# brendan-duncan/unity_webgpu_pathtracer

Hardware: AMD Instinct MI355X
Metric: Mrays/s at 1920x1080, 8 spp (higher is better)
Workload: dtype f32; 1 GPU; sponza: Sponza-class atrium (~250k tris, 24 textured Disney materials, 2 rect lights + sky), 1920x1080, 8 spp/pass, depth 4, progressive passes (CurrentSample = 8k); tris=250752, schedule=1, passes_in_flight=12, passes_per_launch_sequence=1

## Files before the change

### __graft_entry__.py

```python
import os
import subprocess
import sys

ROOT = os.path.dirname(os.path.abspath(__file__))
if ROOT not in sys.path:
    sys.path.insert(0, ROOT)


def build() -> None:
    subprocess.check_call(["make", "-C", os.path.join(ROOT, "unity_webgpu_pathtracer_amd", "csrc")])
    subprocess.check_call(["make", "-C", os.path.join(ROOT, "unity_webgpu_pathtracer_amd", "csrc"), "stress"])
    subprocess.check_call(["make", "-C", os.path.join(ROOT, "host")])
    subprocess.check_call(["make", "-C", os.path.join(ROOT, "oracle")])
    subprocess.check_call(["make", "-C", os.path.join(ROOT, "oracle"), "ref"])
    from unity_webgpu_pathtracer_amd import plugin
    plugin.load_library()


def smoke() -> None:
    import numpy as np
    from oracle import pyoracle
    from unity_webgpu_pathtracer_amd import scenes
    from unity_webgpu_pathtracer_amd.pathtracer import PathTracer

    for s, w, h in ((scenes.material_zoo(), 96, 64), (scenes.cornell_box(), 64, 64)):
        pt = PathTracer(s, device=0, width=w, height=h, samplesPerPass=2)
        p = pt.params(seed=0x12345678)
        pt.render_pass(p)
        gpu = pt.readback()
        b = pyoracle.buffers_from_bvhscene(pt._bvhScene)
        ref, _ = pyoracle.render(b, p)
        linf = float(np.abs(gpu - ref).max())
        print(f"[smoke] {s.name} {w}x{h} 2spp, schedule {pt.schedule()}: Linf vs oracle = {linf:.3e}, rays = {pt.stats().rays}")
        assert linf < 1e-4, linf
        pt.close()


if __name__ == "__main__":
    build()
    if len(sys.argv) > 1 and sys.argv[1] == "smoke":
        smoke()
```

### include/ptmi_plugin.h

```cpp
#ifndef PTMI_PLUGIN_H
#define PTMI_PLUGIN_H

#include <stdint.h>
#include "ptmi_layouts.h"

#ifdef __cplusplus
extern "C" {
#endif

#if defined(_WIN32)
#define PT_API __declspec(dllexport)
#else
#define PT_API __attribute__((visibility("default")))
#endif


PT_API int   BuildBVH(const PTFloat4* vertices, int triangleCount);
PT_API void  DestroyBVH(int index);
PT_API int   IsBVHReady(int index);
PT_API void* GetBVHPtr(int index);
PT_API void* GetBVH(int index);
PT_API int   GetCWBVHNodesSize(int index);
PT_API int   GetCWBVHTrisSize(int index);
PT_API int   GetCWBVHData(int index, PTFloat4** bvhNodes, PTFloat4** bvhTris);
// ... 88 lines not shown
} PTTimings;

#define PT_OK                 0
#define PT_ERR_INVALID_ARG   -1
#define PT_ERR_NO_DEVICE     -2
#define PT_ERR_HIP           -3
#define PT_ERR_NO_SCENE      -4
#define PT_ERR_UNSUPPORTED   -5

PT_API int PTCreate(int deviceIndex, PTContext** outCtx);
PT_API int PTDestroy(PTContext* ctx);

PT_API int PTSetScene(PTContext* ctx, const PTSceneDesc* scene);

PT_API int PTSetTileOwnership(PTContext* ctx, int rank, int worldSize);

PT_API int PTGetOwnedTileSlots(PTContext* ctx, const PTFrameParams* params, uint64_t* outFloat4Slots);
PT_API int PTPackOwnedTiles(PTContext* ctx, const PTFrameParams* params, const void* dFrame, void* dPacked);
PT_API int PTUnpackTiles(PTContext* ctx, const PTFrameParams* params, int rank, int worldSize, const void* dPacked, void* dFrame);

typedef struct PTGroup PTGroup;
PT_API int PTCreateMulti(const int* deviceIndices, int deviceCount, PTGroup** outGroup);
PT_API int PTGroupDestroy(PTGroup* group);
PT_API int PTGroupSize(PTGroup* group);
PT_API PTContext* PTGroupGetContext(PTGroup* group, int index);
PT_API int PTGroupSetScene(PTGroup* group, const PTSceneDesc* scene);
PT_API int PTGroupRenderPass(PTGroup* group, const PTFrameParams* params);
PT_API int PTGroupRenderPassBatch(PTGroup* group, const PTFrameParams* params, int count);
PT_API int PTGroupFlipFrames(PTGroup* group);
PT_API int PTGroupResetFrames(PTGroup* group);
PT_API int PTGroupSynchronize(PTGroup* group);
PT_API int PTGroupReadback(PTGroup* group, float* dstRGBA, uint64_t dstFloats);
PT_API void* PTGroupGetAssembledFrame(PTGroup* group);
PT_API int PTGroupGetStats(PTGroup* group, PTStats* out);
PT_API int PTGroupResetStats(PTGroup* group);

PT_API int PTRenderPass(PTContext* ctx, const PTFrameParams* params);
PT_API int PTFlipFrames(PTContext* ctx);
PT_API int PTResetFrames(PTContext* ctx);

PT_API int PTRenderPassTo(PTContext* ctx, const PTFrameParams* params, void* dOutput, const void* dAccumulated);

PT_API int PTRenderPassBatchTo(PTContext* ctx, const PTFrameParams* params, int count, void* dOutput, const void* dAccumulated);
PT_API int PTRenderPassBatch(PTContext* ctx, const PTFrameParams* params, int count);

PT_API int PTSynchronize(PTContext* ctx);
PT_API int PTReadback(PTContext* ctx, float* dstRGBA, uint64_t dstFloats);
PT_API void* PTGetFramePointer(PTContext* ctx, int which);
typedef struct PTPresentParams {
    uint32_t OutputWidth, OutputHeight;
    int32_t  Mode;
    int32_t  sRGB;
    float    Exposure, Brightness, Contrast, Saturation, Vignette;
} PTPresentParams;
PT_API int PTPresent(PTContext* ctx, const PTPresentParams* params, const void* dSrc, void* dDst);
PT_API int PTPresentToHost(PTContext* ctx, const PTPresentParams* params, float* dstRGBA, uint64_t dstFloats);

#define PT_MESH_HAS_32_BIT_INDICES 0x1u
#define PT_MESH_HAS_NORMALS        0x2u
#define PT_MESH_HAS_TANGENTS       0x4u
#define PT_MESH_HAS_UVS            0x8u
typedef struct PTMeshDesc {
    const void* vertexBuffer;  uint64_t vertexBufferBytes;
    const void* indexBuffer;   uint64_t indexBufferBytes;
    uint32_t VertexStride, PositionOffset, NormalOffset, TangentOffset, UVOffset;
    uint32_t MaterialIndex;
    uint32_t TriangleCount, OutputTriangleStart;
    float    LocalToWorld[16], WorldToLocal[16];
    uint32_t flags;            uint32_t _pad;
} PTMeshDesc;
PT_API int PTProcessMeshes(PTContext* ctx, const PTMeshDesc* meshes, uint32_t meshCount, uint32_t totalTriangles,
                           float* outVertexPositions, void* outTriangleAttributes);

typedef struct PTTextureDesc {
    const float* texels;  uint32_t width, height;  int32_t hasAlpha;  uint32_t _pad;
} PTTextureDesc;
PT_API int PTCopyTextureData(PTContext* ctx, const PTTextureDesc* textures, uint32_t count, uint32_t* outTextureData, uint64_t outUints);

PT_API void* PTGetStream(PTContext* ctx);

PT_API int PTSetStatsLevel(PTContext* ctx, int level);
PT_API int PTGetStats(PTContext* ctx, PTStats* out);
PT_API int PTResetStats(PTContext* ctx);

PT_API int PTSetProfiling(PTContext* ctx, int enabled);
PT_API int PTGetTimings(PTContext* ctx, PTTimings* out);
PT_API int PTResetTimings(PTContext* ctx);

PT_API int PTSetSchedule(PTContext* ctx, int schedule);
PT_API int PTGetSchedule(PTContext* ctx);
PT_API int PTSetWavefrontIterations(PTContext* ctx, int iterations);

PT_API int PTSetPassesInFlight(PTContext* ctx, int passes);
PT_API int PTGetPassesInFlight(PTContext* ctx);
PT_API int PTSetSubFrames(PTContext* ctx, int subFrames);

typedef struct PTRay {
    float    origin[3];
    float    direction[3];
    float    tmax;
    uint32_t reserved;
} PTRay;

typedef struct PTRayHit {
    float    t;
    float    u, v;
    uint32_t prim;
} PTRayHit;

typedef struct PTRaySurface {
    float    position[3]; float    t;
    float    normal[3];   int32_t  materialIndex;
    float    uv[2];       uint32_t instance;
                          uint32_t prim;
} PTRaySurface;

#ifdef __cplusplus
static_assert(sizeof(PTRay) == 32, "PTRay is 32 bytes");
static_assert(sizeof(PTRayHit) == 16, "PTRayHit is 16 bytes");
static_assert(sizeof(PTRaySurface) == 48, "PTRaySurface is 48 bytes");
#else
_Static_assert(sizeof(PTRay) == 32, "PTRay is 32 bytes");
_Static_assert(sizeof(PTRayHit) == 16, "PTRayHit is 16 bytes");
_Static_assert(sizeof(PTRaySurface) == 48, "PTRaySurface is 48 bytes");
#endif

#define PT_QUERY_CLOSEST  0u
#define PT_QUERY_ANY_HIT  1u
#define PT_QUERY_SURFACE  2u

PT_API int PTTraceRays(PTContext* ctx, const PTRay* dRays, uint64_t count, uint32_t flags,
                       PTRayHit* dHits, PTRaySurface* dSurface );
PT_API int PTTraceRaysHost(PTContext* ctx, const PTRay* rays, uint64_t count, uint32_t flags,
                           PTRayHit* hits, PTRaySurface* surface);

#define PT_DENOISE_DEMODULATE_ALBEDO 0x1u

typedef struct PTDenoiseParams {
    uint32_t structSize;
    int32_t  iterations;
    float    sigmaLuminance;
    float    sigmaNormal;
    float    sigmaDepth;
    uint32_t flags;
} PTDenoiseParams;

#ifdef __cplusplus
static_assert(sizeof(PTDenoiseParams) == 24, "PTDenoiseParams is 24 bytes");
#else
_Static_assert(sizeof(PTDenoiseParams) == 24, "PTDenoiseParams is 24 bytes");
#endif

PT_API int PTRenderGuides(PTContext* ctx, const PTFrameParams* params, int samplesPerPixel);
PT_API int PTDenoise(PTContext* ctx, const PTDenoiseParams* params, const void* dSrc, void* dDst);
PT_API int PTDenoiseToHost(PTContext* ctx, const PTDenoiseParams* params, float* dstRGBA, uint64_t dstFloats);
PT_API void* PTGetGuidePointer(PTContext* ctx, int which);

PT_API int PTUpdateInstances(PTContext* ctx, const PTBlasInstance* instances, uint32_t count);
PT_API int PTUpdateInstancesDevice(PTContext* ctx, const PTBlasInstance* dInstances, uint32_t count);
PT_API int PTUpdateLights(PTContext* ctx, const void* lights, uint32_t count);
PT_API int PTUpdateMaterials(PTContext* ctx, const void* materials, uint32_t count);
PT_API int PTReadTLAS(PTContext* ctx, void* dstNodes, uint64_t dstNodeBytes, uint32_t* dstIndices, uint64_t dstIndexCount,
                      uint32_t* outNodeCount);

typedef struct PTNoiseParams {
    uint32_t structSize;
// ... 483 lines not shown
```

### unity_webgpu_pathtracer_amd/abi.py

```python
import ctypes as C

import numpy as np

FLOAT4 = np.dtype([("x", "<f4"), ("y", "<f4"), ("z", "<f4"), ("w", "<f4")])

CWBVH_NODE = np.dtype([
    ("lo", "<f4", 3), ("ex", "u1"), ("ey", "u1"), ("ez", "u1"), ("imask", "u1"),
    ("childBaseIndex", "<u4"), ("triBaseIndex", "<u4"), ("meta", "u1", 8),
    ("qlox", "u1", 8), ("qloy", "u1", 8), ("qloz", "u1", 8),
    ("qhix", "u1", 8), ("qhiy", "u1", 8), ("qhiz", "u1", 8),
])
assert CWBVH_NODE.itemsize == 80

TRI_ATTR = np.dtype([
    ("normal0", "<f4", 3), ("pad0", "<f4"), ("normal1", "<f4", 3), ("pad1", "<f4"),
    ("normal2", "<f4", 3), ("pad2", "<f4"), ("tangent0", "<f4", 3), ("pad3", "<f4"),
    ("tangent1", "<f4", 3), ("pad4", "<f4"), ("tangent2", "<f4", 3), ("pad5", "<f4"),
    ("uv0", "<f4", 2), ("uv1", "<f4", 2), ("uv2", "<f4", 2), ("materialIndex", "<u4"), ("pad6", "<f4"),
])
assert TRI_ATTR.itemsize == 128

MATERIAL_FLOATS = 32
LIGHT_FLOATS = 16

# ... 22 lines not shown
PT_FEATURE_HAS_ENVIRONMENT_TEXTURE = 0x8

PT_OK = 0
PT_ERR_INVALID_ARG = -1
PT_ERR_NO_DEVICE = -2
PT_ERR_HIP = -3
PT_ERR_NO_SCENE = -4
PT_ERR_UNSUPPORTED = -5


class _Sized(C.Structure):
    def __init__(self, *args, **kw):
        super().__init__(*args, **kw)
        self.structSize = C.sizeof(type(self))


class PTSceneDesc(_Sized):
    _fields_ = [
        ("structSize", C.c_uint32), ("_pad3", C.c_uint32),
        ("bvhNodes", C.c_void_p), ("bvhNodesBytes", C.c_uint64),
        ("bvhTris", C.c_void_p), ("bvhTrisBytes", C.c_uint64),
        ("triAttrs", C.c_void_p), ("triAttrsBytes", C.c_uint64),
        ("materials", C.c_void_p), ("materialCount", C.c_uint32), ("_pad0", C.c_uint32),
        ("lights", C.c_void_p), ("lightCount", C.c_uint32), ("_pad1", C.c_uint32),
        ("textureData", C.c_void_p), ("textureDataUints", C.c_uint64),
        ("features", C.c_uint32), ("_pad2", C.c_uint32),
        ("tlasData", C.c_void_p), ("tlasDataFloats", C.c_uint64),
        ("tlasIndexOffset", C.c_uint32), ("instanceCount", C.c_uint32),
        ("gpuInstances", C.c_void_p),
        ("envTexture", C.c_void_p), ("envWidth", C.c_uint32), ("envHeight", C.c_uint32),
    ]


class PTFrameParams(_Sized):
    _fields_ = [
        ("structSize", C.c_uint32), ("_pad0", C.c_uint32),
        ("CamInvProj", C.c_float * 16),
        ("CamToWorld", C.c_float * 16),
        ("RngSeedRoot", C.c_uint32),
        ("MaxRayBounces", C.c_uint32),
        ("SamplesPerPass", C.c_int32),
        ("OutputWidth", C.c_uint32),
        ("OutputHeight", C.c_uint32),
        ("CurrentSample", C.c_uint32),
        ("EnvironmentMode", C.c_int32),
        ("EnvironmentIntensity", C.c_float),
        ("EnvironmentColor", C.c_float * 4),
        ("EnvironmentMapRotation", C.c_float),
        ("FocalLength", C.c_float),
        ("Aperture", C.c_float),
        ("UseFireflyFilter", C.c_int32),
        ("MaxFireflyLuminance", C.c_float),
        ("UseRussianRoulette", C.c_int32),
        ("DispatchGroupsX", C.c_uint32),
        ("DispatchGroupsY", C.c_uint32),
    ]

    def copy(self):
        other = PTFrameParams()
        C.memmove(C.byref(other), C.byref(self), C.sizeof(PTFrameParams))
        return other


class PTStats(C.Structure):
    _fields_ = [(n, C.c_uint64) for n in (
        "paths", "closestHitRays", "shadowRays", "nodeVisits", "triTests", "attrFetches",
        "materialFetches", "lightFetches", "texelFetches", "texDescriptorFetches",
        "pixelsWritten", "pixelsRead", "maxStackDepth", "stackOverflows", "tlasNodeVisits", "instanceVisits")]

    def as_dict(self):
        return {n: int(getattr(self, n)) for n, _ in self._fields_}

    @property
    def rays(self):
        return int(self.closestHitRays + self.shadowRays)

    def algorithmic_bytes(self):
        return int(80 * self.nodeVisits + 48 * self.triTests + 128 * self.attrFetches
                   + 128 * self.materialFetches + 64 * self.lightFetches + 4 * self.texelFetches
                   + 16 * self.texDescriptorFetches + 16 * (self.pixelsWritten + self.pixelsRead)
                   + 64 * self.tlasNodeVisits + 144 * self.instanceVisits)


class PTPresentParams(C.Structure):
    _fields_ = [("OutputWidth", C.c_uint32), ("OutputHeight", C.c_uint32), ("Mode", C.c_int32), ("sRGB", C.c_int32),
                ("Exposure", C.c_float), ("Brightness", C.c_float), ("Contrast", C.c_float), ("Saturation", C.c_float),
                ("Vignette", C.c_float)]


TONEMAP_NONE, TONEMAP_ACES, TONEMAP_FILMIC, TONEMAP_REINHARD, TONEMAP_LOTTES = range(5)


PT_MESH_HAS_32_BIT_INDICES, PT_MESH_HAS_NORMALS, PT_MESH_HAS_TANGENTS, PT_MESH_HAS_UVS = 0x1, 0x2, 0x4, 0x8


class PTMeshDesc(C.Structure):
    _fields_ = [("vertexBuffer", C.c_void_p), ("vertexBufferBytes", C.c_uint64),
                ("indexBuffer", C.c_void_p), ("indexBufferBytes", C.c_uint64),
                ("VertexStride", C.c_uint32), ("PositionOffset", C.c_uint32), ("NormalOffset", C.c_uint32),
                ("TangentOffset", C.c_uint32), ("UVOffset", C.c_uint32), ("MaterialIndex", C.c_uint32),
                ("TriangleCount", C.c_uint32), ("OutputTriangleStart", C.c_uint32),
                ("LocalToWorld", C.c_float * 16), ("WorldToLocal", C.c_float * 16),
                ("flags", C.c_uint32), ("_pad", C.c_uint32)]


class PTTextureDesc(C.Structure):
    _fields_ = [("texels", C.c_void_p), ("width", C.c_uint32), ("height", C.c_uint32), ("hasAlpha", C.c_int32), ("_pad", C.c_uint32)]


class PTTimings(C.Structure):
    _fields_ = [("passes", C.c_uint64), ("kernelMsTotal", C.c_double),
                ("kernelMsLast", C.c_double), ("kernelLaunches", C.c_uint64)]


PT_FAR_PLANE = 100000.0
PT_QUERY_CLOSEST = 0
PT_QUERY_ANY_HIT = 1
PT_QUERY_SURFACE = 2
PT_MISS = 0xFFFFFFFF


class PTRay(C.Structure):
    _fields_ = [("origin", C.c_float * 3), ("direction", C.c_float * 3), ("tmax", C.c_float), ("reserved", C.c_uint32)]


class PTRayHit(C.Structure):
    _fields_ = [("t", C.c_float), ("u", C.c_float), ("v", C.c_float), ("prim", C.c_uint32)]


class PTRaySurface(C.Structure):
    _fields_ = [("position", C.c_float * 3), ("t", C.c_float), ("normal", C.c_float * 3), ("materialIndex", C.c_int32),
                ("uv", C.c_float * 2), ("instance", C.c_uint32), ("prim", C.c_uint32)]


assert C.sizeof(PTRay) == 32 and C.sizeof(PTRayHit) == 16 and C.sizeof(PTRaySurface) == 48


PT_DENOISE_DEMODULATE_ALBEDO = 0x1


class PTDenoiseParams(C.Structure):
    _fields_ = [("structSize", C.c_uint32), ("iterations", C.c_int32), ("sigmaLuminance", C.c_float),
                ("sigmaNormal", C.c_float), ("sigmaDepth", C.c_float), ("flags", C.c_uint32)]


assert C.sizeof(PTDenoiseParams) == 24


def denoise_params(iterations: int = 5, sigma_luminance: float = 4.0, sigma_normal: float = 128.0, sigma_depth: float = 1.0,
                   demodulate: bool = True) -> PTDenoiseParams:
    return PTDenoiseParams(C.sizeof(PTDenoiseParams), iterations, sigma_luminance, sigma_normal, sigma_depth,
                           PT_DENOISE_DEMODULATE_ALBEDO if demodulate else 0)


class PTNoiseParams(C.Structure):
    _fields_ = [("structSize", C.c_uint32), ("relFloor", C.c_float), ("threshold", C.c_float), ("percentile", C.c_float)]


class PTNoiseStats(C.Structure):
    _fields_ = [("structSize", C.c_uint32), ("observations", C.c_uint32), ("samples", C.c_uint64), ("pixels", C.c_uint64),
                ("pixelsBelow", C.c_uint64), ("meanError", C.c_float), ("maxError", C.c_float), ("percentileError", C.c_float),
                ("_pad", C.c_uint32), ("histogram", C.c_uint32 * 256)]


assert C.sizeof(PTNoiseParams) == 16 and C.sizeof(PTNoiseStats) == 1072

# ... 277 lines not shown
```

### unity_webgpu_pathtracer_amd/csrc/plugin_exports.cpp

```cpp
#include <chrono>
#include <cstddef>
#include <deque>
#include <string>
#include <algorithm>
#include "bvh_builder.h"
#include "bvh_refit.h"
#include "bvh_quality.h"
#include "skin_rule.h"
#include "morph_rule.h"
#include "chart_rule.h"
#include "sh_rule.h"
#include "volume_rule.h"
#include "placement_rule.h"
#include "lmfilter_rule.h"
#include "adaptive_gather_rule.h"
#include "reflection_rule.h"
#include "ptmi_plugin.h"

namespace {
std::deque<ptbvh::Cwbvh*> g_bvhs;
std::deque<ptbvh::Tlas*> g_tlases;

template <class T> int add_slot(std::deque<T*>& table, T* obj)
{
    for (size_t i = 0; i < table.size(); ++i)
        if (table[i] == nullptr) { table[i] = obj; return (int)i; }
    table.push_back(obj);
    return (int)table.size() - 1;
}
template <class T> T* get_slot(std::deque<T*>& table, int index)
{
    return (index >= 0 && index < (int)table.size()) ? table[index] : nullptr;
}
template <class T> void free_slot(std::deque<T*>& table, int index)
{
    if (index >= 0 && index < (int)table.size() && table[index]) { delete table[index]; table[index] = nullptr; }
}
}

extern "C" {

PT_API int BuildBVH(const PTFloat4* vertices, int triangleCount)
{
    if (!vertices || triangleCount <= 0) return -1;
    ptbvh::Cwbvh* bvh = new ptbvh::Cwbvh();
    const auto t0 = std::chrono::steady_clock::now();
    if (!bvh->build(vertices, (uint32_t)triangleCount)) { delete bvh; return -1; }
    bvh->buildMs = std::chrono::duration<double, std::milli>(std::chrono::steady_clock::now() - t0).count();
    return add_slot(g_bvhs, bvh);
}

namespace { std::string g_buildError; }
PT_API int PTBuildBVHDevice(int deviceIndex, const PTFloat4* vertices, int triangleCount)
{
    if (!vertices || triangleCount <= 0) { g_buildError = "vertices == NULL or triangleCount <= 0"; return -1; }
    ptbvh::Cwbvh* bvh = new ptbvh::Cwbvh();
    if (!ptbvh::build_cwbvh_device(deviceIndex, vertices, (uint32_t)triangleCount, *bvh, &bvh->buildMs, g_buildError)) { delete bvh; return -1; }
    g_buildError.clear();
    return add_slot(g_bvhs, bvh);
}
PT_API const char* PTGetBVHBuildError(void) { return g_buildError.c_str(); }
PT_API double PTGetBVHBuildMs(int index)
{
    ptbvh::Cwbvh* b = get_slot(g_bvhs, index);
    return b ? b->buildMs : -1.0;
}
PT_API int PTRefitBVH(int index, const PTFloat4* vertices, int triangleCount)
{
    ptbvh::Cwbvh* b = get_slot(g_bvhs, index);
    if (!b) { g_buildError = "no such BVH handle"; return 0; }
    if (!vertices || triangleCount <= 0 || (uint32_t)triangleCount != b->triCount) { g_buildError = "vertices == NULL or triangleCount is not the handle's"; return 0; }
    if (!ptbvh::refit_cwbvh(b->nodeData.data(), b->usedBlocks / 5u, b->triData.data(), (uint64_t)b->triCount * 3u, 0, 0, vertices, b->triCount, g_buildError)) return 0;
    g_buildError.clear();
    return 1;
}
PT_API int PTRefitBVHArrays(PTFloat4* bvhNodes, uint64_t nodeBytes, PTFloat4* bvhTris, uint64_t triBytes, const PTFloat4* vertices, int triangleCount)
{
    if (!bvhNodes || !bvhTris || !vertices || triangleCount <= 0 || nodeBytes < 80 || nodeBytes % 80 || triBytes != (uint64_t)triangleCount * 48u) {
        g_buildError = "NULL array, nodeBytes not a multiple of 80 or triBytes != triangleCount * 48";
        return 0;
    }
    if (!ptbvh::refit_cwbvh(bvhNodes, nodeBytes / 80u, bvhTris, triBytes / 16u, 0, 0, vertices, (uint32_t)triangleCount, g_buildError)) return 0;
    g_buildError.clear();
    return 1;
}
PT_API int PTMeasureBVHArrays(const PTFloat4* bvhNodes, uint64_t nodeBytes, const PTFloat4* bvhTris, uint64_t triBytes, int triangleCount, PTGeometryQuality* out)
{
    if (!bvhNodes || !bvhTris || !out || triangleCount <= 0 || nodeBytes < 80 || nodeBytes % 80 || triBytes != (uint64_t)triangleCount * 48u) {
        g_buildError = "NULL array or result, nodeBytes not a multiple of 80 or triBytes != triangleCount * 48";
        return 0;
    }
    if (out->structSize < sizeof(PTGeometryQuality) || out->structSize > 4096u) {
        g_buildError = "PTGeometryQuality.structSize is not set (must be sizeof(PTGeometryQuality) of the host's header)";
        return 0;
    }
    ptbvh::Quality q;
    if (!ptbvh::measure_cwbvh(bvhNodes, nodeBytes / 80u, bvhTris, triBytes / 16u, (uint32_t)triangleCount, q, g_buildError)) return 0;
    out->nodeCapacity = q.nodeCapacity; out->nodeCount = q.nodeCount; out->triangleCount = q.triangleCount; out->levels = q.levels;
    out->reserved = 0;
// ... 96 lines not shown
    g_buildError.clear();
    return 1;
}
PT_API int PTProbeDepthProjectHost(const PTProbe* probes, uint64_t count, uint32_t firstSample, uint32_t samples, const float* distances,
                                   float maxDistance, PTProbeDepthMap* out)
{
    if (!ptvol::depth_project_host(probes, count, firstSample, samples, distances, maxDistance, out, g_buildError)) return 0;
    g_buildError.clear();
    return 1;
}
PT_API int PTProbeGridIrradianceHost(const PTProbeGrid* grid, const PTProbeCoeffs* sh, const PTProbeDepthMap* depth, const PTReceiver* queries,
                                     uint64_t count, PTIrradiance* out)
{
    if (!ptvol::grid_irradiance_host(grid, sh, depth, queries, count, out, g_buildError)) return 0;
    g_buildError.clear();
    return 1;
}
PT_API int PTProbePlaceStepHost(const PTProbe* probes, uint64_t count, uint32_t firstSample, uint32_t samples, const PTProbePlaceParams* params,
                                const PTRayHit* hits, const PTRaySurface* surfaces, int move, PTProbePlacement* inout, PTProbePlaceStats* stats)
{
    if (!ptplace::place_step_host(probes, count, firstSample, samples, params, hits, surfaces, move, inout, stats, g_buildError)) return 0;
    g_buildError.clear();
    return 1;
}
PT_API int PTProbeGridIrradiancePlacedHost(const PTProbeGrid* grid, const PTProbeCoeffs* sh, const PTProbeDepthMap* depth, const PTProbePlacement* placement,
                                           const PTReceiver* queries, uint64_t count, PTIrradiance* out)
{
    if (!ptplace::grid_irradiance_placed_host(grid, sh, depth, placement, queries, count, out, g_buildError)) return 0;
    g_buildError.clear();
    return 1;
}
PT_API int PTDenoiseLightmapHost(const PTLightmapDenoiseParams* params, const uint32_t* texels, const PTReceiver* recv, const PTIrradiance* irr, uint64_t count,
                                 uint32_t width, uint32_t height, PTIrradiance* out)
{
    if (!ptlmf::denoise_host(params, texels, recv, irr, count, width, height, out, g_buildError)) return 0;
    g_buildError.clear();
    return 1;
}
PT_API int PTSelectReceiversHost(const PTAdaptiveGather* adaptive, uint32_t n, const uint32_t* active, uint64_t activeCount, const PTIrradiance* acc,
                                 const PTReceiver* recv, uint64_t entryCount, uint32_t* outActive, PTReceiver* outRecv, uint64_t* survivors, uint64_t* stopped)
{
    if (!ptag::select_host(adaptive, n, active, activeCount, acc, recv, entryCount, outActive, outRecv, survivors, stopped, g_buildError)) return 0;
    g_buildError.clear();
    return 1;
}
PT_API int PTFoldIrradianceHost(const uint32_t* active, uint64_t activeCount, const PTIrradiance* fresh, uint32_t m, uint32_t n, uint64_t entryCount,
                                PTIrradiance* acc, uint32_t* counts)
{
    if (!ptag::fold_host(active, activeCount, fresh, m, n, entryCount, acc, counts, g_buildError)) return 0;
    g_buildError.clear();
    return 1;
}
PT_API int PTEqualiseIrradianceHost(const PTIrradiance* irr, const uint32_t* counts, uint64_t count, uint32_t samplesEq, PTIrradiance* out)
{
    if (!ptag::equalise_host(irr, counts, count, samplesEq, out, g_buildError)) return 0;
    g_buildError.clear();
    return 1;
}
PT_API int PTReflectionDirectionsHost(const PTProbe* probes, uint64_t count, uint32_t res, uint32_t firstSample, uint32_t samples, PTRadianceRay* rays)
{
    if (!ptrefl::directions_host(probes, count, res, firstSample, samples, rays, g_buildError)) return 0;
    g_buildError.clear();
    return 1;
}
PT_API int PTReflectionFoldHost(const PTRadiance* radiance, uint64_t count, uint32_t res, uint32_t samples, PTReflectionTexel* out)
{
    if (!ptrefl::fold_host(radiance, count, res, samples, out, g_buildError)) return 0;
    g_buildError.clear();
    return 1;
}
PT_API int PTReflectionPrefilterHost(const PTReflectionTexel* base, uint64_t count, uint32_t res, uint32_t levels, PTReflectionTexel* outMaps)
{
    if (!ptrefl::prefilter_host(base, count, res, levels, outMaps, g_buildError)) return 0;
    g_buildError.clear();
    return 1;
}
PT_API int PTReflectionLookupHost(const PTReflectionTexel* maps, uint64_t probeCount, uint32_t res, uint32_t levels, const PTProbe* probes,
                                  const PTReflectionBox* boxes, const PTReflectionQuery* queries, uint64_t count, PTReflectionTexel* out)
{
    if (!ptrefl::lookup_host(maps, probeCount, res, levels, probes, boxes, queries, count, out, g_buildError)) return 0;
    g_buildError.clear();
    return 1;
}
PT_API void DestroyBVH(int index) { free_slot(g_bvhs, index); }
PT_API int IsBVHReady(int index) { return get_slot(g_bvhs, index) != nullptr; }
PT_API void* GetBVH(int index) { return get_slot(g_bvhs, index); }
PT_API void* GetBVHPtr(int index) { return get_slot(g_bvhs, index); }
PT_API int GetCWBVHNodesSize(int index)
{
    ptbvh::Cwbvh* b = get_slot(g_bvhs, index);
    return b ? (int)(b->usedBlocks * 16u) : 0;
}
PT_API int GetCWBVHTrisSize(int index)
{
    ptbvh::Cwbvh* b = get_slot(g_bvhs, index);
    return b ? (int)(b->triCount * 3u * 16u) : 0;
}
PT_API int GetCWBVHData(int index, PTFloat4** bvhNodes, PTFloat4** bvhTris)
{
    ptbvh::Cwbvh* b = get_slot(g_bvhs, index);
    if (!b || !bvhNodes || !bvhTris || b->nodeData.empty() || b->triData.empty()) return 0;
    *bvhNodes = b->nodeData.data();
    *bvhTris = b->triData.data();
    return 1;
}

PT_API int BuildTLAS(const PTBlasInstance* instances, int instanceCount)
{
    if (!instances || instanceCount <= 0) return -1;
    ptbvh::Tlas* t = new ptbvh::Tlas();
    if (!t->build(instances, (uint32_t)instanceCount)) { delete t; return -1; }
    return add_slot(g_tlases, t);
}
PT_API void DestroyTLAS(int index) { free_slot(g_tlases, index); }
PT_API int IsTLASReady(int index) { return get_slot(g_tlases, index) != nullptr; }
PT_API int GetTLASNodesSize(int index)
{
    ptbvh::Tlas* t = get_slot(g_tlases, index);
    return t ? (int)(t->usedNodes * 64u) : 0;
}
PT_API int GetTLASData(int index, PTFloat4** tlasNodes, uint32_t** tlasIndices)
{
    ptbvh::Tlas* t = get_slot(g_tlases, index);
    if (!t || !tlasNodes || !tlasIndices || t->nodes.empty()) return 0;
    *tlasNodes = (PTFloat4*)t->nodes.data();
    *tlasIndices = t->indices.data();
    return 1;
}

}
```

### unity_webgpu_pathtracer_amd/csrc/pt_api_context.hip

```cpp
#include "pt_context.h"

#include <dlfcn.h>

#include <cstdlib>
#include <algorithm>
#include <array>

thread_local std::string g_lastError;

namespace {

uint32_t hw_queue_limit()
{
    const char* e = getenv("GPU_MAX_HW_QUEUES");
    const long q = e ? strtol(e, nullptr, 10) : 4;
    return q < 1 ? 1u : (q > 1024 ? 1024u : (uint32_t)q);
}

bool create_masked(Stream& s)
{
    int device = 0, cus = 0;
    if (hipGetDevice(&device) != hipSuccess || hipDeviceGetAttribute(&cus, hipDeviceAttributeMultiprocessorCount, device) != hipSuccess || cus <= 0) {
        (void)hipGetLastError();
        return false;
// ... 279 lines not shown
    if (envOn) {
        const size_t n = (size_t)s->envWidth * s->envHeight;
        cdf.resize(n);
        for (size_t i = 0; i < n; ++i) {
            const float* px = s->envTexture + 4 * i;
            cdfSum += 0.299f * px[0] + 0.587f * px[1] + 0.114f * px[2];
            cdf[i] = cdfSum;
        }
        if ((rc = upload(c, c->envTex, s->envTexture, n * 16))) return rc;
        if ((rc = upload(c, c->envCdf, cdf.data(), n * 4))) return rc;
    }
    if (lights) {
        if ((rc = c->lightConst.reserve((size_t)s->lightCount * 64))) return rc;
    }
    HIP_TRY(hipStreamSynchronize(c->stream));
    c->scene.nodes = (const uint4*)c->nodes.ptr;
    c->scene.tris = (const float4*)c->tris.ptr;
    c->scene.attrs = (const float4*)c->attrs.ptr;
    c->scene.materials = (const float4*)c->materials.ptr;
    c->scene.lights = lights ? (const float4*)c->lights.ptr : nullptr;
    c->scene.tex = textures ? (const uint32_t*)c->tex.ptr : nullptr;
    c->scene.lightCount = lights ? (int32_t)s->lightCount : 0;
    c->scene.materialCount = s->materialCount;
    c->scene.hasLights = lights ? 1u : 0u;
    c->scene.hasTextures = textures ? 1u : 0u;
    c->scene.tlas = tlasOn ? (const float*)c->tlas.ptr : nullptr;
    c->scene.instances = tlasOn ? (const float4*)c->instances.ptr : nullptr;
    c->scene.instByLeaf = tlasOn ? (const float4*)c->instByLeaf.ptr : nullptr;
    c->scene.tlasBfs = tlasOn ? (const float*)c->tlasBfs.ptr : nullptr;
    c->scene.tlasNodeCount = tlasOn ? (uint32_t)(bfs.size() / 16) : 0u;
    c->scene.tlasIndexOffset = tlasOn ? s->tlasIndexOffset : 0u;
    c->scene.hasTlas = tlasOn ? 1u : 0u;
    c->scene.envTex = envOn ? (const float4*)c->envTex.ptr : nullptr;
    c->scene.envCdf = envOn ? (const float*)c->envCdf.ptr : nullptr;
    c->scene.envW = envOn ? (int32_t)s->envWidth : 0;
    c->scene.envH = envOn ? (int32_t)s->envHeight : 0;
    c->scene.envCdfSum = cdfSum;
    c->scene.hasEnvTex = envOn ? 1u : 0u;
    c->scene.lightConst = lights ? (const float4*)c->lightConst.ptr : nullptr;
    c->update.instanceCount = tlasOn ? s->instanceCount : 0u;
    c->update.sceneLightCount = lights ? s->lightCount : 0u;
    c->update.origTlasNodes = tlasOn ? s->tlasIndexOffset / 16u : 0u;
    std::vector<uint32_t>& valid = c->update.validTextures;
    valid.clear();
    if (textures) {
        const float* mats = (const float*)s->materials;
        for (uint32_t m = 0; m < s->materialCount; ++m)
            for (int k : kTextureSlots) {
                uint64_t t = 0;
                if (texture_slot(mats[(size_t)m * 32 + k], s->textureData, s->textureDataUints, t) == 0) valid.push_back((uint32_t)t);
            }
        std::sort(valid.begin(), valid.end());
        valid.erase(std::unique(valid.begin(), valid.end()), valid.end());
    }
    if (lights) {
        HIP_TRY(pt_launch_derive_lights(c->scene, (float4*)c->lightConst.ptr, c->stream));
        HIP_TRY(hipStreamSynchronize(c->stream));
    }
    c->hasScene = true;
    return PT_OK;
}

extern "C" {

PT_API int PTCreate(int deviceIndex, PTContext** outCtx)
{
    if (!outCtx) return fail(PT_ERR_INVALID_ARG, "outCtx == NULL");
    *outCtx = nullptr;
    int count = 0;
    hipError_t e = hipGetDeviceCount(&count);
    if (e != hipSuccess || count <= 0)
        return fail(PT_ERR_NO_DEVICE, std::string("no HIP device available (") + (e != hipSuccess ? hipGetErrorString(e) : "device count 0") +
                                          "); this library has no CPU fallback");
    if (deviceIndex < 0 || deviceIndex >= count) return fail(PT_ERR_INVALID_ARG, "deviceIndex out of range");
    HIP_TRY(hipSetDevice(deviceIndex));
    PTContext* c = new PTContext();
    c->device = deviceIndex;
    hipError_t se = hipStreamCreateWithFlags(&c->stream.h, hipStreamNonBlocking);
    if (se != hipSuccess) { delete c; return fail(PT_ERR_HIP, std::string("hipStreamCreate: ") + hipGetErrorString(se)); }
    if (hw_queue_limit() < 16u) {
        if (int rc = create_set_stream(0u, c->sets[0].stream, &c->ownQueues)) { delete c; return rc; }
    }
    c->numSets = default_passes_in_flight(c->ownQueues);
    se = hipMalloc(&c->dStats.ptr, 16 * sizeof(unsigned long long));
    if (se != hipSuccess) { delete c; return fail(PT_ERR_HIP, std::string("hipMalloc: ") + hipGetErrorString(se)); }
    hipMemsetAsync(c->dStats.ptr, 0, 16 * sizeof(unsigned long long), c->stream);
    *outCtx = c;
    return PT_OK;
}

PT_API int PTDestroy(PTContext* c)
{
    if (!c) return PT_OK;
    hipSetDevice(c->device);
    hipStreamSynchronize(c->stream);
    if (c->update.stream) hipStreamSynchronize(c->update.stream);
    for (auto& set : c->sets) if (set.stream) hipStreamSynchronize(set.stream);
    delete c;
    return PT_OK;
}

PT_API int PTSetScene(PTContext* c, const PTSceneDesc* hostScene) { return set_scene(c, hostScene, true); }

PT_API int PTSetTileOwnership(PTContext* c, int rank, int worldSize)
{
    if (!c || worldSize < 1 || rank < 0 || rank >= worldSize) return fail(PT_ERR_INVALID_ARG, "bad rank/worldSize");
    c->rank = rank;
    c->world = worldSize;
    return PT_OK;
}

PT_API int PTSynchronize(PTContext* c)
{
    if (!c) return fail(PT_ERR_INVALID_ARG, "ctx == NULL");
    HIP_TRY(hipSetDevice(c->device));
    HIP_TRY(hipStreamSynchronize(c->stream));
    return PT_OK;
}

PT_API void* PTGetStream(PTContext* c) { return c ? (void*)c->stream : nullptr; }

PT_API int PTSetStatsLevel(PTContext* c, int level)
{
    if (!c) return fail(PT_ERR_INVALID_ARG, "ctx == NULL");
    c->statsLevel = level > 0 ? 1 : 0;
    return PT_OK;
}

PT_API int PTGetStats(PTContext* c, PTStats* out)
{
    if (!c || !out) return fail(PT_ERR_INVALID_ARG, "ctx/out == NULL");
    HIP_TRY(hipSetDevice(c->device));
    unsigned long long h[16];
    HIP_TRY(hipMemcpyAsync(h, c->dStats.ptr, sizeof(h), hipMemcpyDeviceToHost, c->stream));
    HIP_TRY(hipStreamSynchronize(c->stream));
    static_assert(sizeof(PTStats) == 16 * 8, "PTStats is 16 counters");
    memcpy(out, h, sizeof(PTStats));
    return PT_OK;
}

PT_API int PTResetStats(PTContext* c)
{
    if (!c) return fail(PT_ERR_INVALID_ARG, "ctx == NULL");
    HIP_TRY(hipSetDevice(c->device));
    HIP_TRY(hipMemsetAsync(c->dStats.ptr, 0, 16 * sizeof(unsigned long long), c->stream));
    return PT_OK;
}

PT_API int PTSetProfiling(PTContext* c, int enabled)
{
    if (!c) return fail(PT_ERR_INVALID_ARG, "ctx == NULL");
    c->profiling = enabled != 0;
    return PT_OK;
}

PT_API int PTGetTimings(PTContext* c, PTTimings* out)
{
    if (!c || !out) return fail(PT_ERR_INVALID_ARG, "ctx/out == NULL");
    HIP_TRY(hipSetDevice(c->device));
    int rc = drain_events(c);
    if (rc) return rc;
    *out = c->timings;
    return PT_OK;
}

PT_API int PTResetTimings(PTContext* c)
{
    if (!c) return fail(PT_ERR_INVALID_ARG, "ctx == NULL");
    int rc = drain_events(c);
    if (rc) return rc;
    c->timings = PTTimings{};
    return PT_OK;
}

PT_API int PTGetSchedule(PTContext* c)
{
    if (!c) return fail(PT_ERR_INVALID_ARG, "ctx == NULL");
    return effective_schedule(c);
}

PT_API int PTSetSchedule(PTContext* c, int schedule)
{
    if (!c) return fail(PT_ERR_INVALID_ARG, "ctx == NULL");
    if (schedule < -1 || schedule > 4)
        return fail(PT_ERR_UNSUPPORTED, "unknown schedule (0 = megakernel, 1 = wavefront + refill trace, 2 = wavefront, one ray per lane, 3 = wavefront + persistent dynamic-chunk trace, 4 = fused persistent wavefront)");
    c->schedule = schedule;
    return PT_OK;
}

PT_API int PTSetPassesInFlight(PTContext* c, int passes)
{
    if (!c || passes < 0 || passes > PT_WF_SETS) return fail(PT_ERR_INVALID_ARG, "ctx == NULL or passes outside 0.." + std::to_string(PT_WF_SETS));
    HIP_TRY(hipSetDevice(c->device));
    for (auto& set : c->sets) if (set.stream) HIP_TRY(hipStreamSynchronize(set.stream));
    c->numSets = passes == 0 ? default_passes_in_flight(c->ownQueues) : (uint32_t)passes;
    c->nextSet = 0u;
    for (uint32_t k = c->numSets; k < (uint32_t)PT_WF_SETS; ++k) {
        c->sets[k].arena.release();
        c->sets[k].wf = PTWfBuffers{};
    }
    return PT_OK;
}

PT_API int PTSetSubFrames(PTContext* c, int subFrames)
{
    if (!c || subFrames < 1 || subFrames > PT_WF_SETS) return fail(PT_ERR_INVALID_ARG, "ctx == NULL or subFrames outside 1.." + std::to_string(PT_WF_SETS));
    c->subFrames = (uint32_t)subFrames;
    return PT_OK;
}

PT_API int PTGetPassesInFlight(PTContext* c) { return c ? (int)c->numSets : fail(PT_ERR_INVALID_ARG, "ctx == NULL"); }

PT_API int PTSetWavefrontIterations(PTContext* c, int iterations)
{
    if (!c || iterations < 0) return fail(PT_ERR_INVALID_ARG, "ctx == NULL or iterations < 0");
    c->wfIterations = (uint32_t)iterations;
    return PT_OK;
}

PT_API const char* PTGetLastError(void) { return g_lastError.c_str(); }
PT_API int PTGetVersion(void) { return (0 << 16) | 2; }

}
// ... 1 lines not shown
```

### unity_webgpu_pathtracer_amd/csrc/pt_api_render.hip

```cpp
#include "pt_context.h"

int ensure_frames(PTContext* c, uint32_t w, uint32_t h)
{
    if (c->frames.w == w && c->frames.h == h) return PT_OK;
    int rc = c->frames.resize(w, h, {sizeof(float4), sizeof(float4)}, nullptr);
    if (rc) return rc;
    for (int i = 0; i < 2; i++) HIP_TRY(hipMemsetAsync(c->frames.f4(i), 0, c->frames.buf[i].used, c->stream));
    c->cur = 0;
    return PT_OK;
}

int ensure_wavefront(PTContext* c, PTContext::WfSet& set, uint32_t numSlots, uint32_t maxIterations)
{
    int rc;
    if ((rc = create_set_stream((uint32_t)(&set - c->sets), set.stream)) || (rc = create(set.callEv)) || (rc = create(set.done))) return rc;
    const bool needTlas = c->scene.hasTlas != 0u;
    if (set.wf.flags && set.wf.numSlots == numSlots && set.wf.maxIterations >= maxIterations && (!needTlas || set.wf.tlasSpill)) return PT_OK;
    if (c->residentWaves == 0u) {
        hipDeviceProp_t prop;
        HIP_TRY(hipGetDeviceProperties(&prop, c->device));
        c->residentWaves = (uint32_t)prop.multiProcessorCount * 4u * 8u;
    }
    if ((rc = set.arena.reserve(pt_wf_arena_bytes(numSlots, c->residentWaves, needTlas, maxIterations), set.stream))) {
        set.wf = PTWfBuffers{};
        return rc;
    }
    set.wf = pt_wf_arena_carve(set.arena.ptr, numSlots, c->residentWaves, needTlas, maxIterations);
    HIP_TRY(hipMemsetAsync(set.wf.statRows, 0, (size_t)set.wf.numStatRows * 16 * 8, set.stream));
    return PT_OK;
}

int wavefront_limits(const PTFrameParams& p, uint32_t& maxIterations)
{
    const uint32_t spp = p.SamplesPerPass > 1 ? (uint32_t)p.SamplesPerPass : 1u;
    const uint32_t bounces = p.MaxRayBounces > 1u ? p.MaxRayBounces : 1u;
    if (spp > 4095u || bounces > 8191u) return fail(PT_ERR_UNSUPPORTED, "wavefront schedules pack SamplesPerPass <= 4095 and MaxRayBounces <= 8191");
    const uint64_t maxIt = (uint64_t)spp * (bounces + 2u) + 4u;
    maxIterations = (uint32_t)(maxIt > 65536u ? 65536u : maxIt);
    return PT_OK;
}

PTContext::WfSet& next_wavefront_set(PTContext* c, uint32_t* index)
{
    if (c->nextSet >= c->numSets) c->nextSet = 0u;
    const uint32_t k = c->nextSet;
    c->nextSet = (k + 1u) % c->numSets;
    if (index) *index = k;
    return c->sets[k];
}

int enqueue_wavefront(PTContext* c, PTContext::WfSet& set, PTWfLaunch& L, hipEvent_t profStart, hipEvent_t profStop, uint32_t& launches)
{
    L.scene = &c->scene;
    L.buffers = &set.wf;
    L.counters = (unsigned long long*)c->dStats.ptr;
    L.fullStats = c->statsLevel > 0;
    L.stream = set.stream;
    L.schedule = effective_schedule(c);
    L.iterationsOverride = c->wfIterations;
    if (c->update.pending) HIP_TRY(hipStreamWaitEvent(set.stream, c->update.done, 0));
    if (profStart) HIP_TRY(hipEventRecord(profStart, set.stream));
    uint32_t n = 0;
    HIP_TRY(pt_launch_wavefront(L, &n));
    launches += n;
    if (profStop) HIP_TRY(hipEventRecord(profStop, set.stream));
    HIP_TRY(hipEventRecord(set.done, set.stream));
    return PT_OK;
}

int enqueue_list_chunks(PTContext* c, const PTFrameParams& p, uint64_t count, uint64_t perChunk, uint32_t slotsPerEntry, const char* rangeName,
                        ListChunkFill fill, void* fillArg)
{
    RoctxRange range(rangeName);
    int rc;
    uint32_t maxIterations;
    if ((rc = wavefront_limits(p, maxIterations))) return rc;
    if (count == 0) return PT_OK;
    HIP_TRY(hipSetDevice(c->device));
    uint32_t used = 0u;
    static_assert(PT_WF_SETS <= 32, "one bit per state set");
    for (uint64_t first = 0; first < count; first += perChunk) {
        const uint32_t n = (uint32_t)(count - first < perChunk ? count - first : perChunk);
        EventPair ep;
        if (c->profiling && (rc = take_event_pair(c, ep))) return rc;
        uint32_t k;
        PTContext::WfSet& set = next_wavefront_set(c, &k);
        used |= 1u << k;
        const uint32_t numSlots = (n * slotsPerEntry + 255u) & ~255u;
        if ((rc = ensure_wavefront(c, set, numSlots, maxIterations))) return rc;
        set.wf.slotsPerPass = numSlots;
        PTWfLaunch L = {};
        L.params = &p;
        fill(fillArg, first, n, L);
        HIP_TRY(hipEventRecord(set.callEv, c->stream));
        HIP_TRY(hipStreamWaitEvent(set.stream, set.callEv, 0));
        uint32_t launches = 0;
        if ((rc = enqueue_wavefront(c, set, L, c->profiling ? ep.start.h : nullptr, c->profiling ? ep.stop.h : nullptr, launches))) return rc;
        if (c->profiling) {
            ep.launches = launches;
            c->pending.push_back(std::move(ep));
        }
    }
    for (uint32_t k = 0; k < c->numSets; ++k)
        if (used & (1u << k)) HIP_TRY(hipStreamWaitEvent(c->stream, c->sets[k].done, 0));
    return PT_OK;
}

namespace {

int render_to(PTContext* c, const PTFrameParams& params, float4* dOut, const float4* dAcc, const PTBatch* hostBatch = nullptr)
{
    RoctxRange range("PT pass (enqueue)");
    const PTFrameParams* p = &params;
    int rc;
    PTBatch batch = {};
    if (hostBatch) batch = *hostBatch;
    else { batch.count = 1u; batch.seedRoot[0] = p->RngSeedRoot; batch.currentSample[0] = p->CurrentSample; }
    if (!c->hasScene) return fail(PT_ERR_NO_SCENE, "PTSetScene has not been called");
    if (!dOut) return fail(PT_ERR_INVALID_ARG, "output buffer == NULL");
    if (p->CurrentSample > 0 && !dAcc) return fail(PT_ERR_INVALID_ARG, "CurrentSample > 0 needs an accumulated frame");
    HIP_TRY(hipSetDevice(c->device));

    const PTTileMap tm = pt_make_tile_map(*p, c->rank, c->world);

    EventPair ep;
    if (c->profiling && (rc = take_event_pair(c, ep))) return rc;
    uint32_t launches = 0;
    const int schedule = effective_schedule(c);
    switch (schedule) {
    case 1:
    case 2:
    case 3:
    case 4: {
        uint32_t maxIterations;
        if ((rc = wavefront_limits(*p, maxIterations))) return rc;
        uint32_t S = c->subFrames < 1u ? 1u : c->subFrames;
        if (S > c->numSets) S = c->numSets;
        const bool zeroOnce = c->world > 1 && S > 1u;
// ... 194 lines not shown
```

### unity_webgpu_pathtracer_amd/csrc/pt_launch.h

```cpp
#pragma once
#include <hip/hip_runtime.h>
#include "pt_device.h"

struct PTTileMap {
    uint32_t rank, world;
    uint32_t blocksX, blocksY;
    uint32_t coverW, coverH;
};

__host__ __device__ inline uint32_t pt_num_slots(const PTTileMap& tm)
{
    const uint32_t bpr = (tm.blocksX + tm.world - 1u) / tm.world;
    return bpr * tm.blocksY * 256u;
}
__host__ __device__ inline bool pt_slot_to_pixel(const PTTileMap& tm, uint32_t slot, uint32_t& px, uint32_t& py)
{
    const uint32_t bpr = (tm.blocksX + tm.world - 1u) / tm.world;
    const uint32_t block = slot >> 8, tid = slot & 255u;
    const uint32_t by = block / bpr, k = block % bpr;
    const uint32_t first = (uint32_t)(((int)tm.rank - (int)(by % tm.world) + (int)tm.world) % (int)tm.world);
    const uint32_t bx = first + k * tm.world;
    const uint32_t wave = tid >> 6, lane = tid & 63u;
    px = bx * 16u + (wave & 1u) * 8u + (lane & 7u);
    py = by * 16u + (wave >> 1) * 8u + (lane >> 3);
// ... 25 lines not shown
                                  float4* dTriangleAttributes, hipStream_t stream);
hipError_t pt_launch_copy_texture(const float4* dTexture, uint32_t width, uint32_t height, uint32_t dataOffset, uint32_t descriptorOffset,
                                  int hasAlpha, uint32_t* dTextureData, hipStream_t stream);
hipError_t pt_launch_present(const PTPresentParams& Q, const float4* src, float4* dst, hipStream_t stream);

#define PT_QUERY_KERNELS 12
inline int pt_query_kernel_index(bool tlas, uint32_t mode, bool stats) { return ((tlas ? 3 : 0) + (int)mode) * 2 + (stats ? 1 : 0); }
hipError_t pt_query_grid_caps(int device, uint32_t caps[PT_QUERY_KERNELS]);
size_t pt_query_slab_bytes_per_wave();
hipError_t pt_launch_query(const DScene& S, const float4* rays, uint32_t count, uint32_t mode, bool stats, float4* hits,
                           float4* surface, uint2* slab, uint32_t gridCap, unsigned long long* gstats, hipStream_t stream);

hipError_t pt_guide_grid_caps(int device, uint32_t caps[2]);
size_t pt_guide_slab_bytes_per_wave();
hipError_t pt_launch_guides(const DScene& S, const PTFrameParams& P, uint32_t n, float4* albedo, float4* normalDepth, uint2* slab,
                            uint32_t gridCap, hipStream_t stream);
struct PTDenoiseArgs {
    uint32_t width, height;
    float sigmaL, sigmaN, sigmaZ;
    uint32_t flags;
};
struct PTDenoiseVariance {
    const float4* plane0;
    const float4* plane1;
    float invDof;
    const float* blockInvDof = nullptr;
};
hipError_t pt_launch_denoise(const PTDenoiseArgs& A, int iterations, const float4* src, float4* dst, const float4* albedo,
                             const float4* normalDepth, float4* state0, float4* state1, float2* gradz,
                             const PTDenoiseVariance* variance, hipStream_t stream);

hipError_t pt_launch_moments_accumulate(uint32_t pixels, float f, const float4* out, const float4* acc, float4* plane0,
                                        float4* plane1, hipStream_t stream);
hipError_t pt_launch_moments_accumulate_blocks(uint32_t entries, const uint2* table, uint32_t width, uint32_t height, const float4* out,
                                               const float4* acc, float4* plane0, float4* plane1, hipStream_t stream);
enum : uint32_t { PT_NOISE_MAX = 256, PT_NOISE_BELOW, PT_NOISE_SUM, PT_NOISE_WORDS };
struct PTNoiseArgs {
    uint32_t width, height;
    uint32_t rank, world;
    float invDof, relFloor, threshold;
};
hipError_t pt_launch_noise(const PTNoiseArgs& A, const float4* frame, const float4* plane0, uint32_t* stats, float* blockSums,
                           float* tiles, hipStream_t stream, const float* blockInvDof = nullptr);

enum : uint32_t { PT_F4_RAY0 = 0, PT_F4_RAY1 = 2, PT_F4_RAY2 = 4, PT_F4_RAD = 6, PT_F4_THR, PT_F4_COLOR, PT_F4_ENVC, PT_F4_LIGHTC,
                  PT_F4_PTHR, PT_F4_HIT, PT_F4_HIT2, PT_F4_PIXSUM, PT_F4_COUNT };
#ifndef PT_WF_LDS_STACK
#define PT_WF_LDS_STACK 8
#endif
#ifndef PT_WF_TLAS_WG_WAVES
#define PT_WF_TLAS_WG_WAVES 1u
#endif
#ifndef PT_WF_TLAS_CACHE_NODES
#define PT_WF_TLAS_CACHE_NODES 400u
#endif
#ifndef PT_WF_TLAS_CHUNK
#define PT_WF_TLAS_CHUNK 64u
#endif
#ifndef PT_WF_TLAS_BLAS_LDS_STACK
#define PT_WF_TLAS_BLAS_LDS_STACK (PT_WF_LDS_STACK < 4 ? PT_WF_LDS_STACK : 4)
#endif
#define PT_WF_SPILL_ROW_ENTRIES (PT_BVH_STACK_SIZE - (PT_WF_TLAS_BLAS_LDS_STACK < PT_WF_LDS_STACK ? PT_WF_TLAS_BLAS_LDS_STACK : PT_WF_LDS_STACK))
struct PTWfBuffers {
    uint32_t* flags;
    uint32_t* rng;
    float4* ray[3];
    float4 *rad, *thr, *color;
    float4 *envC, *lightC, *pthr;
    float4* hit;
    float4* hit2;
    float4* pixsum;
    float4* f4base;
    uint32_t f4stride;
    uint8_t* occl;
    uint2* stackSpill;
    uint32_t* tlasSpill;
    uint4* susp;
    uint32_t* suspCount;
    uint32_t* chunkHeads;
    unsigned long long* statRows;
    uint32_t numSlots, numStatRows, maxIterations;
    uint32_t slotsPerPass;
    uint32_t residentWaves;
};

size_t pt_wf_arena_bytes(uint32_t numSlots, uint32_t residentWaves, bool needTlas, uint32_t maxIterations);
PTWfBuffers pt_wf_arena_carve(void* base, uint32_t numSlots, uint32_t residentWaves, bool needTlas, uint32_t maxIterations);

#ifndef PT_WF_WIDE_DIV
#define PT_WF_WIDE_DIV 4u
#endif
inline bool pt_wf_wide_ranges(uint32_t numSlots, uint32_t residentWaves) { return (numSlots / 128u) >= residentWaves / PT_WF_WIDE_DIV; }
inline uint32_t pt_wf_max_trace_waves(uint32_t numSlots, uint32_t residentWaves)
{
    const uint32_t narrow = (numSlots + 63u) / 64u;
    if (!pt_wf_wide_ranges(numSlots, residentWaves)) return narrow;
    const uint32_t wide = (numSlots + 127u) / 128u, persist = residentWaves < narrow ? residentWaves : narrow;
    return wide > persist ? wide : persist;
}

#define PT_MAX_BATCH 8
struct PTBatch {
    uint32_t count;
    uint32_t seedRoot[PT_MAX_BATCH];
    uint32_t currentSample[PT_MAX_BATCH];
};
__host__ __device__ inline void pt_batch_pick(const PTBatch& b, uint32_t j, uint32_t& seedRoot, uint32_t& currentSample)
{
    seedRoot = b.seedRoot[0]; currentSample = b.currentSample[0];
#pragma unroll
    for (uint32_t k = 1; k < PT_MAX_BATCH; ++k) if (j == k) { seedRoot = b.seedRoot[k]; currentSample = b.currentSample[k]; }
}

struct PTListMap {
    uint32_t frameBlocksX;
    uint32_t coverW, coverH;
    const uint2* table;
};
__host__ __device__ inline bool pt_list_slot_to_pixel(uint32_t frameBlocksX, uint32_t coverW, uint32_t coverH, uint32_t blockId, uint32_t tid,
                                                      uint32_t& px, uint32_t& py)
{
    const uint32_t by = blockId / frameBlocksX, bx = blockId - by * frameBlocksX;
    const uint32_t wave = tid >> 6, lane = tid & 63u;
    px = bx * 16u + (wave & 1u) * 8u + (lane & 7u);
    py = by * 16u + (wave >> 1) * 8u + (lane >> 3);
    return px < coverW && py < coverH;
}

struct PTRayMap {
    const PTRadianceRay* rays;
    uint32_t count;
};
#define PT_RADIANCE_CHUNK (1u << 21)
hipError_t pt_launch_camera_rays(const PTFrameParams& P, const uint32_t* indices, uint32_t count, PTRadianceRay* rays, hipStream_t stream);

struct PTGatherMap {
    const PTReceiver* recv;
    uint32_t entries, samples;
    uint32_t firstSample;
};
hipError_t pt_launch_gather_init(const DScene& S, const PTFrameParams& P, const PTGatherMap& gm, const PTWfBuffers& B, bool fullStats, hipStream_t stream);
hipError_t pt_launch_gather_resolve(const PTGatherMap& gm, const PTWfBuffers& B, PTIrradiance* out, hipStream_t stream);
hipError_t pt_launch_gather_rays(const DScene& S, const PTFrameParams& P, const PTGatherMap& gm, PTRadianceRay* rays, hipStream_t stream);

struct PTProbeMap {
    const PTProbe* probes;
    uint32_t entries, samples;
    uint32_t firstSample;
    uint32_t lightCount;
    const float4* deltaRays;
    const float4* deltaLi;
    const float4* deltaHits;
};
hipError_t pt_launch_probe_init(const PTProbeMap& pm, const PTWfBuffers& B, hipStream_t stream);
hipError_t pt_launch_probe_resolve(const PTProbeMap& pm, const PTWfBuffers& B, PTProbeCoeffs* out, hipStream_t stream);
hipError_t pt_launch_probe_rays(const PTProbeMap& pm, PTRadianceRay* rays, hipStream_t stream);
hipError_t pt_launch_probe_delta_rays(const DScene& S, const PTProbe* probes, uint32_t entries, float4* rays, float4* li, hipStream_t stream);
hipError_t pt_launch_probe_irradiance(const PTProbeCoeffs* sh, uint64_t probeCount, const PTProbeQuery* queries, uint32_t count, PTIrradiance* out,
                                      hipStream_t stream);
hipError_t pt_launch_probe_depth_rays(const PTProbe* probes, uint32_t entries, uint32_t samples, uint32_t firstSample, float maxDistance, float4* rays,
                                      hipStream_t stream);
hipError_t pt_launch_probe_depth_resolve(const PTProbe* probes, uint32_t entries, uint32_t samples, uint32_t firstSample, float maxDistance,
                                         const float4* hits, PTProbeDepthMap* out, hipStream_t stream);
hipError_t pt_launch_probe_grid_irradiance(const PTProbeGrid& grid, const PTProbeCoeffs* sh, const PTProbeDepthMap* depth, const PTReceiver* queries,
                                           uint32_t count, PTIrradiance* out, hipStream_t stream);
hipError_t pt_launch_probe_place_rays(const PTProbe* probes, uint32_t entries, uint32_t samples, uint32_t firstSample, const PTProbePlaceParams& params,
                                      const PTProbePlacement* placement, float4* rays, hipStream_t stream);
hipError_t pt_launch_probe_place_step(const PTProbe* probes, uint32_t entries, uint32_t samples, uint32_t firstSample, const PTProbePlaceParams& params,
                                      const float4* hits, const float4* surfaces, bool move, PTProbePlacement* placement, PTProbePlaceStats* stats,
                                      hipStream_t stream);
hipError_t pt_launch_probe_grid_irradiance_placed(const PTProbeGrid& grid, const PTProbeCoeffs* sh, const PTProbeDepthMap* depth, const PTProbePlacement* placement,
                                                  const PTReceiver* queries, uint32_t count, PTIrradiance* out, hipStream_t stream);
hipError_t pt_launch_refl_rays(const PTProbe* probes, uint64_t firstTexel, uint32_t texels, uint32_t res, uint32_t firstSample, uint32_t samples,
                               PTRadianceRay* rays, hipStream_t stream);
hipError_t pt_launch_refl_fold(const PTRadiance* radiance, uint32_t texels, uint32_t samples, PTReflectionTexel* out, hipStream_t stream);
hipError_t pt_launch_refl_prefilter(const PTReflectionTexel* base, uint32_t probes, uint32_t res, uint32_t levels, PTReflectionTexel* out, hipStream_t stream);
hipError_t pt_launch_refl_lookup(const PTReflectionTexel* maps, uint64_t probeCount, uint32_t res, uint32_t levels, const PTProbe* probes,
                                 const PTReflectionBox* boxes, const PTReflectionQuery* queries, uint32_t count, PTReflectionTexel* out, hipStream_t stream);
#ifndef PT_WF_FUSED_GROUPS
#define PT_WF_FUSED_GROUPS 2u
#endif
#ifndef PT_WF_SUSPEND
#define PT_WF_SUSPEND 16u
#endif
#ifndef PT_WF_SETS
#define PT_WF_SETS 12
#endif

enum PTWfMapKind : uint32_t { PT_WF_MAP_TILES, PT_WF_MAP_LIST, PT_WF_MAP_RAYS, PT_WF_MAP_GATHER, PT_WF_MAP_PROBE };
struct PTWfLaunch {
    const DScene* scene;
    const PTFrameParams* params;
    PTBatch batch;
    PTWfMapKind mapKind;
    union {
        PTTileMap tiles;
        PTListMap list;
        PTRayMap rays;
        PTGatherMap gather;
        PTProbeMap probe;
    };
    const float4* accumulated;
    void* output;
    const PTWfBuffers* buffers;
    unsigned long long* counters;
    bool fullStats;
    hipStream_t stream;
    hipEvent_t orderAfter;
    bool zeroOutputFirst;
    int schedule;
    uint32_t iterationsOverride;
};
hipError_t pt_launch_wavefront(const PTWfLaunch& L, uint32_t* launchesOut);
```

### unity_webgpu_pathtracer_amd/csrc/pt_wavefront.hip

```cpp
#include "pt_device.h"
#include "pt_launch.h"
#include "pt_wf_state.h"
#include <type_traits>

namespace {

#define PT_WF_CHUNK 64u

PT_DEV float4* f4_array(const PTWfBuffers& B, uint32_t k) { return B.f4base + (size_t)k * B.f4stride; }
PT_DEV void fetch_ray(const PTWfBuffers& B, uint32_t slot, uint32_t kind, v3& o, v3& d)
{
    const float4* rec = f4_array(B, 2u * kind) + 2u * (size_t)slot;
    o = xyz(rec[0]);
    d = xyz(rec[1]);
}


PT_DEV uint32_t pixel_slot_of(const PTWfBuffers& B, uint32_t slot, uint32_t& pass)
{
    pass = 0u;
    if (slot >= B.slotsPerPass) { pass = slot / B.slotsPerPass; slot -= pass * B.slotsPerPass; }
    return slot;
}

PT_DEV bool wf_pixel(const PTTileMap& tm, const PTWfBuffers& B, uint32_t slot, uint32_t wgSlot, uint32_t& px, uint32_t& py, uint32_t& pass, uint32_t& base)
{
    base = 0u;
    return pt_slot_to_pixel(tm, pixel_slot_of(B, slot, pass), px, py);
}
PT_DEV bool wf_pixel(const PTListMap& lm, const PTWfBuffers& B, uint32_t slot, uint32_t wgSlot, uint32_t& px, uint32_t& py, uint32_t& pass, uint32_t& base)
{
    pass = wgSlot / B.slotsPerPass;
    const uint2 entry = lm.table[(wgSlot - pass * B.slotsPerPass) >> 8];
    base = entry.y;
    return pt_list_slot_to_pixel(lm.frameBlocksX, lm.coverW, lm.coverH, entry.x, slot & 255u, px, py);
}
template <class MAP> constexpr bool kListMap = std::is_same<MAP, PTListMap>::value;

PT_DEV bool wf_pixel(const PTRayMap& rm, const PTWfBuffers& B, uint32_t slot, uint32_t wgSlot, uint32_t& px, uint32_t& py, uint32_t& pass, uint32_t& base)
{
    px = 0u; py = 0u; pass = 0u; base = 0u;
    return slot < rm.count;
}
template <class MAP> constexpr bool kRayMap = std::is_same<MAP, PTRayMap>::value;
struct RaySample {
    const PTRadianceRay* rays; uint32_t slot;
    PT_DEV void operator()(const PTFrameParams&, uint32_t, uint32_t, PathRegs& r, Counters& cn) const { start_ray(r, cn); }
    PT_DEV void start_ray(PathRegs& r, Counters& cn) const
    {
        const float4* e = (const float4*)(rays + slot);
        const float4 a = e[0], b = e[1];
        cn.paths++;
        r.scatterPdf = 0.0f;
        r.maxRoughness = 0.0f;
        r.ro = mk3(a.x, a.y, a.z);
        r.rd = mk3(a.w, b.x, b.y);
        r.state = PS_TRACE;
    }
};
PT_DEV void ray_path_init(const PTRayMap& rm, uint32_t slot, PathRegs& r, Counters& cn)
{
    r.rng = rm.rays[slot].rng;
    r.sampleIdx = 0u;
    r.color = mk3(0.0f);
    r.env.valid = 0u; r.light.valid = 0u;
    r.env.dir = mk3(0.0f); r.light.dir = mk3(0.0f);
    r.env.contribution = mk3(0.0f); r.light.contribution = mk3(0.0f);
    r.neeOrigin = mk3(0.0f); r.pendThroughput = mk3(0.0f);
    r.hasPending = false; r.green = false;
    path_reset_sample(r);
    RaySample{rm.rays, slot}.start_ray(r, cn);
}

template <class MAP = PTTileMap>
__global__ __launch_bounds__(256) void pt_wf_init(PTFrameParams P, PTBatch batch, MAP tm, PTWfBuffers B)
{
    const uint32_t slot = blockIdx.x * 256u + threadIdx.x;
    if (blockIdx.x == 0u && threadIdx.x < PT_WF_SHARDS) B.chunkHeads[threadIdx.x * 32u] = 0u;
    if (slot >= B.numSlots) return;
    uint32_t px, py, pass, base;
    Counters cn = {};
    if (!wf_pixel(tm, B, slot, blockIdx.x * 256u, px, py, pass, base)) B.flags[slot] = PS_DONE;
    else {
        PathRegs r;
        if constexpr (kRayMap<MAP>) ray_path_init(tm, slot, r, cn);
        else {
            uint32_t seedRoot, currentSample;
            pt_batch_pick(batch, pass, seedRoot, currentSample);
            if (kListMap<MAP>) currentSample = base + pass * (P.SamplesPerPass > 1 ? (uint32_t)P.SamplesPerPass : 1u);
            path_init(P, seedRoot, currentSample, px, py, py * P.OutputWidth + px, r, cn);
        }
        store_path(B, slot, r, false);
    }
    flush_counters<false>(cn, B.statRows, blockIdx.x * 4u + (threadIdx.x >> 6), threadIdx.x & 63u);
}

#ifndef PT_WF_TRACE_MIN_WAVES
#define PT_WF_TRACE_MIN_WAVES 8
#endif

template <bool STATS, bool TLAS>
__global__ __launch_bounds__(256, 4) void pt_wf_trace(DScene S, PTWfBuffers B, uint32_t iteration)
{
    __shared__ uint2 s_stack[PT_LDS_STACK][256];
    const uint32_t nb = B.numSlots >> 8;
    const uint32_t vb = blockIdx.x;
    const uint32_t kind = vb / nb;
    const uint32_t slot = (vb % nb) * 256u + threadIdx.x;
    const uint32_t f = B.flags[slot];
    bool valid;
    if (kind == 0u) valid = fl_state(f) == PS_TRACE;
    else if (kind == 1u) valid = fl_pending(f) && fl_env(f) != 0u;
    else valid = fl_pending(f) && fl_light(f) != 0u;
    Counters cn = {};
    if (valid) {
        v3 o, d;
        fetch_ray(B, slot, kind, o, d);
        TravStack st;
        st.lds = PT_LDS_U2(&s_stack[0][threadIdx.x]);
        st.stride = 256u;
        HitRecord h;
        h.h.t = PT_FAR_PLANE; h.h.u = 0.0f; h.h.v = 0.0f; h.h.triIndex = 0u;
        h.pos = mk3(0.0f); h.inst = 0u;
        bool occluded;
        if (TLAS) occluded = traverse_tlas<STATS>(S, o, d, kind != 0u, h, st, cn);
        else { traverse_cwbvh<STATS>(S, o, d, kind != 0u, h.h, st, cn); occluded = h.h.t < PT_FAR_PLANE; }
        if (kind == 0u) {
            B.hit[slot] = make_float4(h.h.t, h.h.u, h.h.v, pt_asfloat(h.h.triIndex));
            if (TLAS) B.hit2[slot] = make_float4(h.pos.x, h.pos.y, h.pos.z, pt_asfloat(h.inst));
            cn.closestRays++;
        } else { B.occl[(size_t)(kind - 1u) * B.numSlots + slot] = occluded ? 1 : 0; cn.shadowRays++; }
    }
    flush_counters<STATS>(cn, B.statRows, (B.numSlots >> 6) + vb * 4u + (threadIdx.x >> 6), threadIdx.x & 63u);
}

#ifndef PT_WF_RANGE
#define PT_WF_RANGE 128u
#endif
#define PT_WF_STAT_ROW_SETS 4u
static_assert(PT_WF_RANGE >= 64u && (PT_WF_RANGE & (PT_WF_RANGE - 1u)) == 0u && PT_WF_STAT_ROW_SETS >= 3u,
              "one counter row per trace wave: the main trace launch uses rows numSlots/64 + wave, the tail launch rows 2 x numSlots/64 + wave");
#ifndef PT_WF_REFILL
#define PT_WF_REFILL 16u
#endif
#ifndef PT_WF_TRI_PARK
#define PT_WF_TRI_PARK 4u
#endif

typedef volatile __attribute__((address_space(3))) uint32_t* pt_lds_u32;
typedef volatile __attribute__((address_space(3))) uint16_t* pt_lds_u16;
PT_DEV uint32_t rank_below(unsigned long long m)
{
    return __builtin_amdgcn_mbcnt_hi((uint32_t)(m >> 32), __builtin_amdgcn_mbcnt_lo((uint32_t)m, 0u));
}

PT_DEV void store_miss(const PTWfBuffers& B, uint32_t slot)
{
    float far = PT_FAR_PLANE;
    asm volatile("" : "+v"(far), "+v"(slot));
    f4_array(B, PT_F4_HIT)[slot] = make_float4(far, 0.0f, 0.0f, 0.0f);
}
PT_DEV void store_hit(const PTWfBuffers& B, uint32_t slot, const TraceHit& hit)
// ... 428 lines not shown
    if ((threadIdx.x & 63u) == 0u) {
        for (uint32_t t = 0; t < PT_WF_SHARDS; ++t) {
            const uint32_t sh = (shard + t) & (PT_WF_SHARDS - 1u);
            const uint32_t inShard = (numChunks + PT_WF_SHARDS - 1u - sh) / PT_WF_SHARDS;
            if (inShard == 0u) continue;
            const uint32_t k = atomicAdd(&heads[sh * 32u], 1u);
            if (k < inShard) { result = k * PT_WF_SHARDS + sh; break; }
        }
    }
    result = __shfl(result, 0, 64);
    chunk = result;
    return result != 0xFFFFFFFFu;
}

template <bool STATS>
__global__ __launch_bounds__(64, PT_WF_TRACE_MIN_WAVES) void pt_wf_trace_persist(DScene S, PTWfBuffers B, uint32_t iteration)
{
    __shared__ uint2 s_stack[PT_WF_LDS_STACK][64];
    __shared__ uint32_t s_xchg[64];
    const uint32_t lane = threadIdx.x;
    const uint32_t numChunks = (B.numSlots + PT_WF_CHUNK - 1u) / PT_WF_CHUNK;
    const uint32_t shard = blockIdx.x & (PT_WF_SHARDS - 1u);
    const uint32_t nItems = 3u * PT_WF_CHUNK;
    pt_lds_u32 xchg = (pt_lds_u32)&s_xchg[0];

    Counters cn = {};
    TravStackT<PT_WF_LDS_STACK, true> st;
    st.lds = PT_LDS_U2(&s_stack[0][lane]);
    st.stride = 64u;
    st.gbase = B.stackSpill;
    __shared__ uint32_t s_gw;
    if (lane == 0u) s_gw = blockIdx.x;
    st.gwave = PT_LDS_WORD(s_gw);
    RayState rs;
    rs.sp = 0u; rs.anyHit = false; rs.overflow = false;
    bool have = false;
    uint32_t mySlot = 0u, myKind = 0u;
    uint32_t cursor = nItems, slotBase = 0u;
    bool more = true;

    while (true) {
        uint32_t nIdle = (uint32_t)__popcll(__ballot(!have));
        while (nIdle >= PT_WF_REFILL || nIdle == 64u) {
            if (cursor >= nItems) {
                uint32_t chunk;
                if (!more || !next_chunk(B.chunkHeads, numChunks, shard, chunk)) { more = false; break; }
                slotBase = chunk * PT_WF_CHUNK;
                cursor = 0u;
            }
            const uint32_t item = cursor + lane;
            const uint32_t kind = item / PT_WF_CHUNK;
            const uint32_t slot = slotBase + (item & (PT_WF_CHUNK - 1u));
            bool valid = item < nItems && slot < B.numSlots;
            if (valid) valid = ray_exists(B.flags[slot], kind);
            const Compaction c = compact_candidates(xchg, !have, nIdle, valid, item);
            if (!have && c.rankI < c.take) {
                const uint32_t it = xchg[c.rankI];
                myKind = it / PT_WF_CHUNK;
                mySlot = slotBase + (it & (PT_WF_CHUNK - 1u));
                have = start_ray(B, mySlot, myKind, rs, cn);
            }
            __builtin_amdgcn_wave_barrier();
            cursor += c.consumed;
            nIdle = (uint32_t)__popcll(__ballot(!have));
        }
        if (nIdle == 64u) break;
        const uint32_t stopAt = more ? PT_WF_REFILL : 64u;
        do {
            if (have) {
                const float tBefore = rs.hit.t;
                const bool fin = ray_step<STATS>(S, rs, st, cn);
                if (myKind == 0u && rs.hit.t < tBefore) f4_array(B, PT_F4_HIT)[mySlot] = make_float4(rs.hit.t, rs.hit.u, rs.hit.v, pt_asfloat(rs.hit.triIndex));
                if (fin) {
                    store_result(B, mySlot, myKind, rs.hit.t < PT_FAR_PLANE, rs.hit, true);
                    have = false;
                }
            }
            nIdle = (uint32_t)__popcll(__ballot(!have));
        } while (nIdle < stopAt);
    }
    flush_counters<STATS>(cn, B.statRows, (B.numSlots >> 6) + blockIdx.x, lane);
}

#ifndef PT_WF_SHADE_MIN_WAVES
#define PT_WF_SHADE_MIN_WAVES 3
#endif

PT_DEV void load_path(const PTWfBuffers& B, uint32_t slot, uint32_t f, PathRegs& r)
{
    r.state = fl_state(f);
    r.hasPending = fl_pending(f);
    r.env.valid = fl_env(f);
    r.light.valid = fl_light(f);
    r.green = (f >> 6) & 1u;
    r.sampleIdx = (f >> 7) & 0xFFFu;
    r.depth = f >> 19;
    r.rng = B.rng[slot];
    float4 q;
    q = B.ray[0][2u * slot]; r.ro = xyz(q); r.scatterPdf = q.w;
    q = B.ray[0][2u * slot + 1u]; r.rd = xyz(q); r.maxRoughness = q.w;
    r.radiance = xyz(B.rad[slot]);
    r.throughput = xyz(B.thr[slot]);
    r.color = xyz(B.color[slot]);
    r.env.dir = mk3(0.0f); r.light.dir = mk3(0.0f); r.neeOrigin = mk3(0.0f);
    r.env.contribution = mk3(0.0f); r.light.contribution = mk3(0.0f); r.pendThroughput = mk3(0.0f);
    if (r.hasPending) {
        r.env.contribution = xyz(B.envC[slot]);
        r.light.contribution = xyz(B.lightC[slot]);
        r.pendThroughput = xyz(B.pthr[slot]);
    }
}

template <bool STATS, bool PIXSUM = false, class MAP = PTTileMap>
PT_DEV bool shade_slot(const DScene& S, const PTFrameParams& P, const MAP& tm, const PTWfBuffers& B, uint32_t slot, uint32_t pixelSlot,
                       uint32_t f, Counters& cn, uint32_t wgSlot = 0u)
{
    uint32_t px, py, pass, base;
    wf_pixel(tm, B, pixelSlot, wgSlot, px, py, pass, base);
    uint32_t rng = B.rng[slot];
    float4 qro = B.ray[0][2u * slot], qrd = B.ray[0][2u * slot + 1u], qrad = B.rad[slot], qthr = B.thr[slot], qcol = B.color[slot];
    float4 qenvC = B.envC[slot], qlightC = B.lightC[slot], qpthr = B.pthr[slot], qhit = B.hit[slot];
    uint32_t o0 = B.occl[slot], o1 = B.occl[(size_t)B.numSlots + slot];
    float4 qhit2 = make_float4(0.0f, 0.0f, 0.0f, 0.0f);
    if (S.hasTlas) qhit2 = B.hit2[slot];
    asm volatile("" : "+v"(rng), "+v"(qro.x), "+v"(qrd.x), "+v"(qrad.x), "+v"(qthr.x), "+v"(qcol.x), "+v"(qenvC.x), "+v"(qlightC.x), "+v"(qpthr.x),
                      "+v"(qhit.x), "+v"(o0), "+v"(o1), "+v"(qhit2.x));
    PathRegs r;
    r.state = fl_state(f);
    r.hasPending = fl_pending(f);
    r.env.valid = fl_env(f);
    r.light.valid = fl_light(f);
    r.green = (f >> 6) & 1u;
    r.sampleIdx = (f >> 7) & 0xFFFu;
    r.depth = f >> 19;
    r.rng = rng;
    r.ro = xyz(qro); r.scatterPdf = qro.w;
    r.rd = xyz(qrd); r.maxRoughness = qrd.w;
    r.radiance = xyz(qrad);
    r.throughput = xyz(qthr);
    r.color = xyz(qcol);
    r.env.dir = mk3(0.0f); r.light.dir = mk3(0.0f); r.neeOrigin = mk3(0.0f);
    r.env.contribution = r.hasPending ? xyz(qenvC) : mk3(0.0f);
    r.light.contribution = r.hasPending ? xyz(qlightC) : mk3(0.0f);
    r.pendThroughput = r.hasPending ? xyz(qpthr) : mk3(0.0f);
    const bool occEnv = r.hasPending && o0 != 0u, occLight = r.hasPending && o1 != 0u;
    HitRecord ch;
    ch.h.t = PT_FAR_PLANE; ch.h.u = 0.0f; ch.h.v = 0.0f; ch.h.triIndex = 0u;
    ch.pos = mk3(0.0f); ch.inst = 0u;
    if (r.state == PS_TRACE) {
        ch.h.t = qhit.x; ch.h.u = qhit.y; ch.h.v = qhit.z; ch.h.triIndex = pt_asuint(qhit.w);
        if (S.hasTlas) { ch.pos = xyz(qhit2); ch.inst = pt_asuint(qhit2.w); }
    }
    struct Sink {
        const PTWfBuffers& B; uint32_t slot;
        PT_DEV void operator()(PathRegs& q) const {
            uint32_t s2 = slot;
            asm volatile("" : "+v"(s2));
            B.ray[1][2u * s2] = f4(q.neeOrigin, 0.0f);
            B.ray[1][2u * s2 + 1u] = f4(q.env.dir, 0.0f);
            B.ray[2][2u * s2] = f4(q.neeOrigin, 0.0f);
            B.ray[2][2u * s2 + 1u] = f4(q.light.dir, 0.0f);
            B.envC[s2] = f4(q.env.contribution, 0.0f);
            B.lightC[s2] = f4(q.light.contribution, 0.0f);
            B.pthr[s2] = f4(q.pendThroughput, 0.0f);
        }
    };
    if constexpr (kRayMap<MAP>)
        path_step<STATS, false, Sink, RaySample, true>(S, P, r, ch, occEnv, occLight, 0u, 0u, 0u, nullptr, nullptr, cn, Sink{B, slot}, RaySample{tm.rays, pixelSlot});
    else
        path_step<STATS, false, Sink, CameraSample, true>(S, P, r, ch, occEnv, occLight, px, py, py * P.OutputWidth + px, nullptr, nullptr, cn, Sink{B, slot});
    uint32_t storeSlot = slot;
    asm volatile("" : "+v"(storeSlot));
    store_path(B, storeSlot, r, false);
    if (PIXSUM && r.state == PS_DONE) {
        uint32_t ps = pixelSlot;
        asm volatile("" : "+v"(ps));
        B.pixsum[ps] = f4(r.color, 0.0f);
    }
    return r.state != PS_DONE;
}

#ifndef PT_WF_SHADE_BLOCK
#define PT_WF_SHADE_BLOCK 64u
#endif
template <bool STATS, class MAP = PTTileMap>
__global__ __launch_bounds__(PT_WF_SHADE_BLOCK, PT_WF_SHADE_MIN_WAVES) void pt_wf_shade(DScene S, PTFrameParams P, MAP tm, PTWfBuffers B,
                                                                         uint32_t iteration)
{
    const uint32_t vb = blockIdx.x;
    const uint32_t slot = vb * PT_WF_SHADE_BLOCK + threadIdx.x;
    if (vb == 0u && threadIdx.x < PT_WF_SHARDS) B.chunkHeads[threadIdx.x * 32u] = 0u;
    const uint32_t f = B.flags[slot];
    Counters cn = {};
    if (fl_state(f) != PS_DONE) shade_slot<STATS, false, MAP>(S, P, tm, B, slot, slot, f, cn, vb * PT_WF_SHADE_BLOCK);
    flush_counters<STATS>(cn, B.statRows, vb * (PT_WF_SHADE_BLOCK / 64u) + (threadIdx.x >> 6), threadIdx.x & 63u);
}

#ifndef PT_WF_FUSED_WAVES
#define PT_WF_FUSED_WAVES 4
#endif

#define PT_WF_NO_PIXEL 0xFFFFFFFFu

template <bool STATS>
PT_DEV void counters_to_lds(const Counters& cn, pt_lds_u32 tot, uint32_t lane)
{
    uint32_t vals[PT_NUM_COUNTERS];
    counters_to_array(cn, vals);
#pragma unroll
    for (int i = 0; i < PT_NUM_COUNTERS; ++i) {
        if (!STATS && (i >= 3 && i <= 9)) continue;
        if (!STATS && i >= 12) continue;
        if (i == 12) {
            const uint32_t m = wave_max_u32(vals[i]);
            if (lane == 0u && m > tot[i]) tot[i] = m;
        } else {
            const uint32_t v = wave_sum_u32(vals[i]);
            if (lane == 0u && v) tot[i] += v;
        }
    }
}

template <bool STATS>
__global__ __launch_bounds__(64, PT_WF_FUSED_WAVES) void pt_wf_fused(DScene S, PTFrameParams P, PTBatch batch, PTTileMap tm, PTWfBuffers B)
{
    constexpr uint32_t K = PT_WF_FUSED_GROUPS;
    constexpr uint32_t kSusp = PT_WF_SUSPEND ? PT_WF_SUSPEND : 1u;
    static_assert((K & (K - 1u)) == 0u && K >= 1u && K <= 16u, "context groups per wave: a power of two");
    __shared__ uint2 s_stack[PT_WF_LDS_STACK][64];
    __shared__ uint32_t s_xchg[64];
    __shared__ uint32_t s_pix[K][64];
    __shared__ uint32_t s_pend[2][K][2];
    __shared__ uint4 s_susp[kSusp][PT_WF_SUSP_ROWS];
    __shared__ uint32_t s_cnt[PT_NUM_COUNTERS];
    __shared__ uint32_t s_gw;
    const uint32_t lane = threadIdx.x;
    const uint32_t ctxBase = blockIdx.x * (K * 64u);
    pt_lds_u32 xchg = (pt_lds_u32)&s_xchg[0];
    pt_lds_u32 pix = (pt_lds_u32)&s_pix[0][0];
    pt_lds_u32 cnt = (pt_lds_u32)&s_cnt[0];
#pragma unroll
    for (uint32_t k = 0; k < K; ++k) {
        s_pix[k][lane] = PT_WF_NO_PIXEL;
        B.flags[ctxBase + k * 64u + lane] = PS_DONE;
    }
    if (lane < PT_NUM_COUNTERS) s_cnt[lane] = 0u;
    if (lane < 4u * K) (&s_pend[0][0][0])[lane] = 0u;
    if (lane == 0u) s_gw = blockIdx.x;
    __builtin_amdgcn_wave_barrier();
    uint32_t nSusp = 0u, pb = 0u;
    bool more = true;

    while (true) {
        bool any = false;
#pragma unroll 1
        for (uint32_t k = 0; k < K; ++k) {
            const uint32_t ctx = ctxBase + k * 64u + lane;
            uint32_t mine = pix[k * 64u + lane];
            const unsigned long long E = __ballot(mine == PT_WF_NO_PIXEL);
            if (more && E != 0ull) {
                const uint32_t n = (uint32_t)__popcll(E);
                uint32_t base = 0u;
                if (lane == 0u) base = atomicAdd(&B.chunkHeads[0], n);
                base = (uint32_t)__builtin_amdgcn_readfirstlane((int)base);
                if (base + n >= B.numSlots) more = false;
                Counters cn = {};
                if (mine == PT_WF_NO_PIXEL) {
// ... 49 lines not shown

            while (true) {
                uint32_t nIdle = (uint32_t)__popcll(__ballot(!have));
                while (cursor < nItems && (nIdle >= PT_WF_REFILL || nIdle == 64u)) {
                    const uint32_t item = cursor + lane;
                    const uint32_t kind = item / (64u * K);
                    const uint32_t local = item & (64u * K - 1u);
                    bool valid = item < nItems;
                    if (valid) {
                        const uint32_t pw = s_pend[po][local >> 6][(local >> 5) & 1u];
                        valid = !((pw >> (local & 31u)) & 1u) && ray_exists(B.flags[ctxBase + local], kind);
                    }
                    const Compaction c = compact_candidates(xchg, !have, nIdle, valid, (kind << 30) | local);
                    if (!have && c.rankI < c.take) {
                        myRef = xchg[c.rankI];
                        have = start_ray(B, ctxBase + (myRef & 0x3FFFFFFFu), myRef >> 30, rs, cn);
                    }
                    __builtin_amdgcn_wave_barrier();
                    if (c.take > 0u) startedNew = true;
                    cursor += c.consumed;
                    nIdle = (uint32_t)__popcll(__ballot(!have));
                }
                if (nIdle == 64u) break;
                const bool exhausted = cursor >= nItems;
                const bool mayPark = PT_WF_SUSPEND > 0u && exhausted && startedNew;
                const uint32_t stopAt = !exhausted ? PT_WF_REFILL : (mayPark ? 64u - PT_WF_SUSPEND : 64u);
                while (nIdle < stopAt) {
                    if (wave_step<STATS>(S, have, rs, st, cn)) {
                        store_result(B, ctxBase + (myRef & 0x3FFFFFFFu), myRef >> 30, rs.hit.t < PT_FAR_PLANE, rs.hit, false);
                        have = false;
                    }
                    nIdle = (uint32_t)__popcll(__ballot(!have));
                }
                if (mayPark && nIdle < 64u) {
                    have = finish_slab_rays<STATS>(S, B, have, ctxBase + (myRef & 0x3FFFFFFFu), myRef >> 30, rs, st, cn);
                    const unsigned long long act = __ballot(have);
                    if (have) {
                        const uint32_t kind = myRef >> 30, local = myRef & 0x3FFFFFFFu;
                        if (kind == 0u && rs.hit.t < PT_FAR_PLANE) store_hit(B, ctxBase + local, rs.hit);
                        suspend_ray(s_susp[rank_below(act)], myRef, rs, st);
                        atomicOr(&s_pend[pn][local >> 6][(local >> 5) & 1u], 1u << (local & 31u));
                        have = false;
                    }
                    nSusp = (uint32_t)__popcll(act);
                    break;
                }
            }
            pb = pn;
            counters_to_lds<STATS>(cn, cnt, lane);
        }
        __builtin_amdgcn_fence(__ATOMIC_RELEASE, "workgroup");
        __builtin_amdgcn_fence(__ATOMIC_ACQUIRE, "workgroup");
        __builtin_amdgcn_wave_barrier();

#pragma unroll 1
        for (uint32_t k = 0; k < K; ++k) {
            const uint32_t ctx = ctxBase + k * 64u + lane;
            const uint32_t mine = pix[k * 64u + lane];
            const uint32_t pw = s_pend[pb][k][lane >> 5];
            const bool parked = (pw >> (lane & 31u)) & 1u;
            Counters cn = {};
            if (mine != PT_WF_NO_PIXEL && !parked) {
                const uint32_t f = B.flags[ctx];
                if (!shade_slot<STATS, true>(S, P, tm, B, ctx, mine, f, cn)) pix[k * 64u + lane] = PT_WF_NO_PIXEL;
            }
            counters_to_lds<STATS>(cn, cnt, lane);
        }
        __builtin_amdgcn_fence(__ATOMIC_RELEASE, "workgroup");
        __builtin_amdgcn_fence(__ATOMIC_ACQUIRE, "workgroup");
        __builtin_amdgcn_wave_barrier();
    }
    __builtin_amdgcn_wave_barrier();
    if (lane < PT_NUM_COUNTERS) {
        unsigned long long* p = B.statRows + (size_t)blockIdx.x * 16u + lane;
        const unsigned long long v = cnt[lane];
        if (lane == 12u) { if (v > *p) *p = v; } else if (v) *p += v;
    }
}

template <bool STATS, bool TLAS, class MAP = PTTileMap>
__global__ __launch_bounds__(256, 2) void pt_wf_cleanup(DScene S, PTFrameParams P, MAP tm, PTWfBuffers B)
{
    __shared__ uint2 s_stack[PT_LDS_STACK][256];
    Counters cn = {};
    for (uint32_t blk = blockIdx.x; blk < (B.numSlots >> 8); blk += gridDim.x) {
    const uint32_t slot = blk * 256u + threadIdx.x;
    const uint32_t f = B.flags[slot];
    if (__any(fl_state(f) != PS_DONE)) {
        if (fl_state(f) != PS_DONE) {
            uint32_t px, py, pass, base;
            wf_pixel(tm, B, slot, blk * 256u, px, py, pass, base);
            PathRegs r;
            load_path(B, slot, f, r);
            if (r.hasPending) {
                r.neeOrigin = xyz(B.ray[1][2u * slot]);
                r.env.dir = xyz(B.ray[1][2u * slot + 1u]);
                r.light.dir = xyz(B.ray[2][2u * slot + 1u]);
            }
            TravStack st;
            st.lds = PT_LDS_U2(&s_stack[0][threadIdx.x]);
            st.stride = 256u;
            while (r.state != PS_DONE) {
                HitRecord ch;
                ch.h.t = PT_FAR_PLANE; ch.h.u = 0.0f; ch.h.v = 0.0f; ch.h.triIndex = 0u;
                ch.pos = mk3(0.0f); ch.inst = 0u;
                bool occEnv = false, occLight = false;
                if (r.hasPending && r.env.valid != 0u) {
                    HitRecord h = ch;
                    if (TLAS) occEnv = traverse_tlas<STATS>(S, r.neeOrigin, r.env.dir, true, h, st, cn);
                    else { traverse_cwbvh<STATS>(S, r.neeOrigin, r.env.dir, true, h.h, st, cn); occEnv = h.h.t < PT_FAR_PLANE; }
                    cn.shadowRays++;
                }
                if (r.hasPending && r.light.valid != 0u) {
                    HitRecord h = ch;
                    if (TLAS) occLight = traverse_tlas<STATS>(S, r.neeOrigin, r.light.dir, true, h, st, cn);
                    else { traverse_cwbvh<STATS>(S, r.neeOrigin, r.light.dir, true, h.h, st, cn); occLight = h.h.t < PT_FAR_PLANE; }
                    cn.shadowRays++;
                }
                if (r.state == PS_TRACE) {
                    if (TLAS) traverse_tlas<STATS>(S, r.ro, r.rd, false, ch, st, cn);
                    else traverse_cwbvh<STATS>(S, r.ro, r.rd, false, ch.h, st, cn);
                    cn.closestRays++;
                }
                if constexpr (kRayMap<MAP>)
                    path_step<STATS, false, NoNeeSink, RaySample, true>(S, P, r, ch, occEnv, occLight, 0u, 0u, 0u, nullptr, nullptr, cn, NoNeeSink(), RaySample{tm.rays, slot});
                else
                    path_step<STATS, false, NoNeeSink, CameraSample, true>(S, P, r, ch, occEnv, occLight, px, py, py * P.OutputWidth + px, nullptr, nullptr, cn);
            }
            B.flags[slot] = pack_flags(r);
            B.color[slot] = f4(r.color, 0.0f);
            if constexpr (kRayMap<MAP>) B.rng[slot] = r.rng;
        }
    }
    }
    flush_counters<STATS>(cn, B.statRows, blockIdx.x * 4u + (threadIdx.x >> 6), threadIdx.x & 63u);
}

template <class MAP = PTTileMap>
__global__ __launch_bounds__(256) void pt_wf_resolve(PTFrameParams P, PTBatch batch, MAP tm, PTWfBuffers B, const float4* __restrict__ sums,
                                                     const float4* __restrict__ accumulated, float4* __restrict__ output)
{
    const uint32_t slot = blockIdx.x * 256u + threadIdx.x;
    uint32_t px, py, pass, base;
    Counters cn = {};
    if (slot < B.slotsPerPass && wf_pixel(tm, B, slot, blockIdx.x * 256u, px, py, pass, base)) {
        const uint32_t pixelIndex = py * P.OutputWidth + px;
        const uint32_t numSamples = P.SamplesPerPass > 1 ? (uint32_t)P.SamplesPerPass : 1u;
        const float fSamples = (float)numSamples;
        v3 acc = mk3(0.0f);
        for (uint32_t j = 0; j < batch.count; ++j) {
            uint32_t seedRoot, currentSample;
            pt_batch_pick(batch, j, seedRoot, currentSample);
            if (kListMap<MAP>) currentSample = base + j * numSamples;
            const v3 color = xyz(sums[(size_t)j * B.slotsPerPass + slot]);
            if (currentSample > 0u) {
                if (j == 0u) {
                    const float4 a = accumulated[pixelIndex];
                    acc = mk3(a.x, a.y, a.z);
                }
                cn.pixelsRead++;
                const float cs = (float)currentSample;
                acc = (color + acc * cs) / (cs + fSamples);
            } else {
                acc = color / fSamples;
            }
            cn.pixelsWritten++;
        }
        output[pixelIndex] = make_float4(acc.x, acc.y, acc.z, 1.0f);
    }
    flush_counters<false>(cn, B.statRows, blockIdx.x * 4u + (threadIdx.x >> 6), threadIdx.x & 63u);
}

__global__ __launch_bounds__(256) void pt_wf_resolve_rays(PTFrameParams P, PTRayMap rm, PTWfBuffers B, PTRadiance* __restrict__ out)
{
    const uint32_t slot = blockIdx.x * 256u + threadIdx.x;
    if (slot >= rm.count) return;
    const uint32_t numSamples = P.SamplesPerPass > 1 ? (uint32_t)P.SamplesPerPass : 1u;
    const float fSamples = (float)numSamples;
    const v3 acc = xyz(B.color[slot]) / fSamples;
    ((float4*)out)[slot] = make_float4(acc.x, acc.y, acc.z, pt_asfloat(B.rng[slot]));
}

__global__ __launch_bounds__(256) void pt_wf_fold_rows(unsigned long long* rows, uint32_t numRows, unsigned long long* gstats)
{
    unsigned long long acc[PT_NUM_COUNTERS] = {};
    for (uint32_t r = blockIdx.x * 256u + threadIdx.x; r < numRows; r += gridDim.x * 256u) {
        unsigned long long* p = rows + (size_t)r * 16u;
#pragma unroll
        for (int i = 0; i < PT_NUM_COUNTERS; ++i) {
            unsigned long long v = p[i];
            if (i == 12) acc[i] = v > acc[i] ? v : acc[i]; else acc[i] += v;
            p[i] = 0ull;
        }
    }
    const uint32_t lane = threadIdx.x & 63u;
#pragma unroll
    for (int i = 0; i < PT_NUM_COUNTERS; ++i) {
        unsigned long long v = acc[i];
        for (int off = 32; off > 0; off >>= 1) {
            unsigned long long o = __shfl_xor(v, off, 64);
            if (i == 12) v = o > v ? o : v; else v += o;
        }
        if (lane == 0 && v) { if (i == 12) atomicMax(&gstats[i], v); else atomicAdd(&gstats[i], v); }
    }
}

size_t pt_wf_arena_layout(char* base, uint32_t numSlots, uint32_t residentWaves, bool needTlas, uint32_t maxIterations, PTWfBuffers& B)
{
    const size_t n = numSlots;
    const uint32_t numRows = PT_WF_STAT_ROW_SETS * (numSlots >> 6);
    auto align = [](size_t x) { return (x + 255) & ~(size_t)255; };
    const size_t traceWaves = pt_wf_max_trace_waves(numSlots, residentWaves);
    const size_t spillBytes = traceWaves * 64u * (size_t)(needTlas ? PT_WF_SPILL_ROW_ENTRIES : PT_BVH_STACK_SIZE - PT_WF_LDS_STACK) * sizeof(uint2);
    const size_t suspBytes = traceWaves * (size_t)(PT_WF_SUSPEND ? PT_WF_SUSPEND : 1u) * PT_WF_SUSP_RECORD_ROWS * sizeof(uint4);
    const size_t tlasSpillBytes = needTlas ? traceWaves * 64u * (size_t)PT_BVH_STACK_SIZE * sizeof(uint32_t) : 0;
    size_t total = 0;
    auto carve = [&](size_t bytes) { char* q = base ? base + total : nullptr; total += align(bytes); return q; };
    B.flags = (uint32_t*)carve(n * 4);
    B.rng = (uint32_t*)carve(n * 4);
    float4* dummy = nullptr;
    float4** arrs[PT_F4_COUNT] = {&B.ray[0], &dummy, &B.ray[1], &dummy, &B.ray[2], &dummy, &B.rad, &B.thr, &B.color, &B.envC, &B.lightC, &B.pthr, &B.hit, &B.hit2, &B.pixsum};
    for (auto a : arrs) *a = (float4*)carve(n * 16);
    B.f4base = B.ray[0];
    B.f4stride = (uint32_t)(align(n * 16) / 16);
    B.occl = (uint8_t*)carve(n * 2);
    B.statRows = (unsigned long long*)carve((size_t)numRows * 16 * 8);
    B.chunkHeads = (uint32_t*)carve(PT_WF_SHARDS * 32 * 4);
    B.stackSpill = (uint2*)carve(spillBytes);
    B.susp = (uint4*)carve(suspBytes);
    B.suspCount = (uint32_t*)carve(traceWaves * 4);
    B.tlasSpill = needTlas ? (uint32_t*)carve(tlasSpillBytes) : nullptr;
    B.residentWaves = residentWaves;
    B.numSlots = numSlots;
    B.numStatRows = numRows;
    B.maxIterations = maxIterations;
    return total;
}

}

namespace {

enum class Trace { Refill, RefillTlas, Lane, Persist, Fused };
Trace pick_trace(int schedule, bool tlas)
{
    if (tlas) return schedule == 1 || schedule == 4 ? Trace::RefillTlas : Trace::Lane;
    return schedule == 1 ? Trace::Refill : schedule == 2 ? Trace::Lane : schedule == 3 ? Trace::Persist : Trace::Fused;
}

template <class F> void with_flag(bool flag, F&& f) { if (flag) f(std::true_type{}); else f(std::false_type{}); }
#define PT_FLAG(x) (decltype(x)::value)

template <class MAP, bool UNIT_A>
hipError_t launch_sequence(const PTWfLaunch& L, const MAP& tm, uint32_t* launchesOut)
{
    constexpr bool kList = kListMap<MAP>, kRays = kRayMap<MAP>;
    const DScene& S = *L.scene;
    const PTFrameParams& P = *L.params;
    const PTBatch& batch = L.batch;
    const PTWfBuffers& B = *L.buffers;
    const bool fullStats = L.fullStats;
    const hipStream_t stream = L.stream;
    float4* const output = (float4*)L.output;
    const uint32_t nb = B.numSlots >> 8, nbPass = B.slotsPerPass >> 8;
    uint32_t launches = 0;
    hipError_t e;
    const bool tlas = S.hasTlas != 0u;
    const Trace trace = pick_trace(L.schedule, tlas);
    if (UNIT_A != (trace == Trace::Refill)) return hipErrorInvalidValue;
    if (trace == Trace::Fused) {
        if constexpr (!UNIT_A && !kList && !kRays) {
            if ((e = hipMemsetAsync(B.chunkHeads, 0, sizeof(uint32_t), stream)) != hipSuccess) return e;
            const uint32_t maxWaves = B.numSlots / (64u * PT_WF_FUSED_GROUPS);
            uint32_t waves = B.residentWaves / 8u * (uint32_t)PT_WF_FUSED_WAVES;
            if (waves > maxWaves) waves = maxWaves;
            if (waves == 0u) waves = 1u;
            with_flag(fullStats, [&](auto stats) {
                hipLaunchKernelGGL(pt_wf_fused<PT_FLAG(stats)>, dim3(waves), dim3(64), 0, stream, S, P, batch, tm, B);
            });
            if ((e = hipGetLastError()) != hipSuccess) return e;
            if (L.orderAfter && (e = hipStreamWaitEvent(stream, L.orderAfter, 0)) != hipSuccess) return e;
            if (L.zeroOutputFirst &&
                (e = hipMemsetAsync(output, 0, (size_t)P.OutputWidth * P.OutputHeight * sizeof(float4), stream)) != hipSuccess) return e;
            hipLaunchKernelGGL(pt_wf_resolve<PTTileMap>, dim3(nbPass), dim3(256), 0, stream, P, batch, tm, B, (const float4*)B.pixsum, L.accumulated, output);
            hipLaunchKernelGGL(pt_wf_fold_rows, dim3(256), dim3(256), 0, stream, B.statRows, B.numStatRows, L.counters);
            if (launchesOut) *launchesOut = 3u;
            return hipGetLastError();
        } else {
            return hipErrorNotSupported;
        }
    }
    const bool gather = kRays && L.mapKind == PT_WF_MAP_GATHER;
    const bool probe = kRays && L.mapKind == PT_WF_MAP_PROBE;
    if (gather) { if ((e = pt_launch_gather_init(S, P, L.gather, B, fullStats, stream)) != hipSuccess) return e; }
    else if (probe) { if ((e = pt_launch_probe_init(L.probe, B, stream)) != hipSuccess) return e; }
    else hipLaunchKernelGGL(pt_wf_init<MAP>, dim3(nb), dim3(256), 0, stream, P, batch, tm, B);
    launches++;
    const uint32_t spp = P.SamplesPerPass > 1 ? (uint32_t)P.SamplesPerPass : 1u;
    const uint32_t bounces = P.MaxRayBounces > 1u ? P.MaxRayBounces : 1u;
    uint32_t iterations = L.iterationsOverride ? L.iterationsOverride : spp * (bounces + 2u) + 4u;
    if (iterations > B.maxIterations) iterations = B.maxIterations;
    for (uint32_t it = 0; it < iterations; ++it) {
        if constexpr (UNIT_A) {
            const bool wide = PT_WF_RANGE >= 128u && pt_wf_wide_ranges(B.numSlots, B.residentWaves);
            const uint32_t blocks = wide ? (B.numSlots + 127u) / 128u : (B.numSlots + 63u) / 64u;
            auto refill = [&](auto tail, uint32_t grid) {
                with_flag(fullStats, [&](auto stats) { with_flag(wide, [&](auto w) {
                    hipLaunchKernelGGL((pt_wf_trace_refill<PT_FLAG(stats), PT_FLAG(tail), PT_FLAG(w) ? 128u : 64u>), dim3(grid), dim3(64), 0, stream, S, B, it);
                }); });
                launches++;
            };
            refill(std::false_type{}, blocks);
            if (PT_WF_SUSPEND > 0u) refill(std::true_type{}, (blocks + PT_WF_TAIL_GROUP - 1u) / PT_WF_TAIL_GROUP);
        } else {
            if (trace == Trace::Persist) {
                const uint32_t numChunks = (B.numSlots + PT_WF_CHUNK - 1u) / PT_WF_CHUNK;
                uint32_t waves = B.residentWaves;
                if (waves > numChunks) waves = numChunks;
                with_flag(fullStats, [&](auto stats) {
                    hipLaunchKernelGGL(pt_wf_trace_persist<PT_FLAG(stats)>, dim3(waves), dim3(64), 0, stream, S, B, it);
                });
            } else if (trace == Trace::RefillTlas) {
                const uint32_t refillBlocks = (B.numSlots + PT_WF_RANGE - 1u) / PT_WF_RANGE;
                const bool shared = PT_WF_TLAS_WG_WAVES > 1u && S.tlasNodeCount <= 0xFFFFu;
                with_flag(fullStats, [&](auto stats) { with_flag(shared, [&](auto sh) {
                    constexpr uint32_t WAVES = PT_FLAG(sh) ? PT_WF_TLAS_WG_WAVES : 1u;
                    hipLaunchKernelGGL((pt_wf_trace_refill_tlas<PT_FLAG(stats), WAVES>), dim3((refillBlocks + WAVES - 1u) / WAVES), dim3(64u * WAVES), 0, stream, S, B, it);
                }); });
            } else {
                with_flag(fullStats, [&](auto stats) { with_flag(tlas, [&](auto tl) {
                    hipLaunchKernelGGL((pt_wf_trace<PT_FLAG(stats), PT_FLAG(tl)>), dim3(nb * 3u), dim3(256), 0, stream, S, B, it);
                }); });
            }
            launches++;
        }
        with_flag(fullStats, [&](auto stats) {
            hipLaunchKernelGGL((pt_wf_shade<PT_FLAG(stats), MAP>), dim3(B.numSlots / PT_WF_SHADE_BLOCK), dim3(PT_WF_SHADE_BLOCK), 0, stream, S, P, tm, B, it);
        });
        launches++;
    }
    const uint32_t cleanupBlocks = nb < 1024u ? nb : 1024u;
    with_flag(fullStats, [&](auto stats) { with_flag(!UNIT_A && tlas, [&](auto tl) {
        constexpr bool TLAS = !UNIT_A && PT_FLAG(tl);
        hipLaunchKernelGGL((pt_wf_cleanup<PT_FLAG(stats), TLAS, MAP>), dim3(cleanupBlocks), dim3(256), 0, stream, S, P, tm, B);
    }); });
    if (L.orderAfter && (e = hipStreamWaitEvent(stream, L.orderAfter, 0)) != hipSuccess) return e;
    if (L.zeroOutputFirst &&
        (e = hipMemsetAsync(output, 0, (size_t)P.OutputWidth * P.OutputHeight * sizeof(float4), stream)) != hipSuccess) return e;
    if constexpr (kRays) {
        if (gather) { if ((e = pt_launch_gather_resolve(L.gather, B, (PTIrradiance*)L.output, stream)) != hipSuccess) return e; }
        else if (probe) { if ((e = pt_launch_probe_resolve(L.probe, B, (PTProbeCoeffs*)L.output, stream)) != hipSuccess) return e; }
        else hipLaunchKernelGGL(pt_wf_resolve_rays, dim3(nbPass), dim3(256), 0, stream, P, tm, B, (PTRadiance*)L.output);
    } else if constexpr (kList) {
        if (L.accumulated &&
            (e = hipMemcpyAsync(output, L.accumulated, (size_t)P.OutputWidth * P.OutputHeight * sizeof(float4), hipMemcpyDeviceToDevice, stream)) != hipSuccess) return e;
    }
    if constexpr (!kRays)
        hipLaunchKernelGGL(pt_wf_resolve<MAP>, dim3(nbPass), dim3(256), 0, stream, P, batch, tm, B, (const float4*)B.color, L.accumulated, output);
    hipLaunchKernelGGL(pt_wf_fold_rows, dim3(256), dim3(256), 0, stream, B.statRows, B.numStatRows, L.counters);
    launches += 3;
    if (launchesOut) *launchesOut = launches;
    return hipGetLastError();
}
#undef PT_FLAG

template <bool UNIT_A>
hipError_t launch_mapped(const PTWfLaunch& L, uint32_t* launchesOut)
{
    PTWfLaunch M = L;
    switch (L.mapKind) {
    case PT_WF_MAP_TILES:
        return launch_sequence<PTTileMap, UNIT_A>(M, M.tiles, launchesOut);
    case PT_WF_MAP_LIST:
        M.zeroOutputFirst = false;
        return launch_sequence<PTListMap, UNIT_A>(M, M.list, launchesOut);
    case PT_WF_MAP_RAYS:
        M.batch = PTBatch{};
        M.batch.count = 1u;
        M.accumulated = nullptr;
        M.orderAfter = nullptr;
        M.zeroOutputFirst = false;
        return launch_sequence<PTRayMap, UNIT_A>(M, M.rays, launchesOut);
    case PT_WF_MAP_GATHER:
    case PT_WF_MAP_PROBE: {
        const PTRayMap slots = {nullptr, L.mapKind == PT_WF_MAP_PROBE ? L.probe.entries * L.probe.samples : L.gather.entries * L.gather.samples};
        PTFrameParams P1 = *L.params;
        P1.SamplesPerPass = 1;
        M.params = &P1;
        M.batch = PTBatch{};
        M.batch.count = 1u;
        M.accumulated = nullptr;
        M.orderAfter = nullptr;
        M.zeroOutputFirst = false;
        return launch_sequence<PTRayMap, UNIT_A>(M, slots, launchesOut);
    }
    }
    return hipErrorInvalidValue;
}
}

#ifdef PT_WF_TU_B
size_t pt_wf_arena_bytes(uint32_t numSlots, uint32_t residentWaves, bool needTlas, uint32_t maxIterations)
{
    PTWfBuffers B = {};
    return pt_wf_arena_layout(nullptr, numSlots, residentWaves, needTlas, maxIterations, B);
}
PTWfBuffers pt_wf_arena_carve(void* base, uint32_t numSlots, uint32_t residentWaves, bool needTlas, uint32_t maxIterations)
{
    PTWfBuffers B = {};
    pt_wf_arena_layout((char*)base, numSlots, residentWaves, needTlas, maxIterations, B);
    return B;
}
hipError_t pt_wf_launch_unit_a(const PTWfLaunch& L, uint32_t* launchesOut);
hipError_t pt_launch_wavefront(const PTWfLaunch& L, uint32_t* launchesOut)
{
    if (L.schedule < 1 || L.schedule > 4) return hipErrorInvalidValue;
    if (L.schedule == 4 && L.mapKind != PT_WF_MAP_TILES) return hipErrorNotSupported;
    if (L.schedule == 1 && L.scene->hasTlas == 0u) return pt_wf_launch_unit_a(L, launchesOut);
    return launch_mapped<false>(L, launchesOut);
}
#else
hipError_t pt_wf_launch_unit_a(const PTWfLaunch& L, uint32_t* launchesOut) { return launch_mapped<true>(L, launchesOut); }
#endif
```

### unity_webgpu_pathtracer_amd/pathtracer.py

```python
import contextlib
import ctypes as C

import numpy as np

from . import abi, plugin
from .scenes import Scene, frame_params


class BVHScene:

    def __init__(self, scene: Scene, build_device: int = None, node_capacity=None):
        self.scene = scene
        self.build_device = build_device
        self.node_capacity = node_capacity
        self.build_ms = {}
        self.tlas_data = None
        self.tlas_index_offset = 0
        self.gpu_instances = None
        if scene.use_tlas:
            self._build_two_level(scene)
        else:
            self.bvh_nodes, self.bvh_tris = plugin.build_cwbvh(scene.vertices, device=build_device, timing=self.build_ms)
            self.bvh_nodes = self._padded(self.bvh_nodes, 0)
            self.blas_spans = [(0, self.bvh_nodes.nbytes // 80, 0, self.bvh_tris.nbytes // 48)]
# ... 141 lines not shown
        self.ctx = ctx
        self.device = device
        self._bvhScene = BVHScene(scene, build_device=build_device, node_capacity=node_capacity)
        self._builtCost = {}
        self._bvhScene.PrepareShader(self.ctx)
        if world_size > 1:
            plugin.check(self.lib.PTSetTileOwnership(self.ctx, rank, world_size))
        self.rank, self.world_size = rank, world_size
        if schedule is not None:
            self.set_schedule(schedule)

    def Reset(self):
        self._currentSample = 0
        plugin.check(self.lib.PTResetFrames(self.ctx))

    def params(self, seed: int) -> abi.PTFrameParams:
        groups = (0, 0)
        if self.reference_dispatch:
            groups = (self.width // 8, self.height // 8)
        return frame_params(self.scene, self.width, self.height, spp=self.samplesPerPass,
                            current_sample=self._currentSample, seed=seed, max_bounces=self.maxRayBounces,
                            russian_roulette=self.useRussianRoulette, firefly=self.fireflyFilter,
                            max_firefly_luminance=self.maxFireflyLuminance, dispatch_groups=groups)

    def OnRenderImage(self, seed: int):
        if self._currentSample < self.maxSamples:
            p = self.params(seed)
            plugin.check(self.lib.PTRenderPass(self.ctx, C.byref(p)))
            if self.track_noise:
                plugin.check(self.lib.PTAccumulateMoments(self.ctx, C.byref(p), 1))
        if self._currentSample < self.maxSamples:
            self._currentSample += max(1, self.samplesPerPass)
        if self._currentSample < self.maxSamples:
            plugin.check(self.lib.PTFlipFrames(self.ctx))
            self._flipped = True
        else:
            self._flipped = False

    def render_pass(self, p: abi.PTFrameParams):
        plugin.check(self.lib.PTRenderPass(self.ctx, C.byref(p)))

    def render_pass_to(self, p: abi.PTFrameParams, d_output: int, d_accumulated: int = 0):
        plugin.check(self.lib.PTRenderPassTo(self.ctx, C.byref(p), C.c_void_p(d_output), C.c_void_p(d_accumulated or None)))

    def render_batch_to(self, params, d_output: int, d_accumulated: int = 0):
        arr = (abi.PTFrameParams * len(params))(*params)
        plugin.check(self.lib.PTRenderPassBatchTo(self.ctx, arr, len(params), C.c_void_p(d_output), C.c_void_p(d_accumulated or None)))

    def flip(self):
        plugin.check(self.lib.PTFlipFrames(self.ctx))

    def synchronize(self):
        plugin.check(self.lib.PTSynchronize(self.ctx))

    def readback(self, last_output: bool = True) -> np.ndarray:
        out = np.empty((self.height, self.width, 4), dtype=np.float32)
        flipped = last_output and getattr(self, "_flipped", False)
        if flipped:
            plugin.check(self.lib.PTFlipFrames(self.ctx))
        try:
            plugin.check(self.lib.PTReadback(self.ctx, out.ctypes.data_as(C.c_void_p), out.size))
        finally:
            if flipped:
                plugin.check(self.lib.PTFlipFrames(self.ctx))
        return out

    def frame_pointer(self, which: int = -1) -> int:
        return self.lib.PTGetFramePointer(self.ctx, which)

    def stream(self) -> int:
        return self.lib.PTGetStream(self.ctx)

    def set_stats_level(self, level: int):
        plugin.check(self.lib.PTSetStatsLevel(self.ctx, level))

    def stats(self) -> abi.PTStats:
        st = abi.PTStats()
        plugin.check(self.lib.PTGetStats(self.ctx, C.byref(st)))
        return st

    def reset_stats(self):
        plugin.check(self.lib.PTResetStats(self.ctx))

    def set_profiling(self, on: bool):
        plugin.check(self.lib.PTSetProfiling(self.ctx, 1 if on else 0))

    def timings(self) -> abi.PTTimings:
        t = abi.PTTimings()
        plugin.check(self.lib.PTGetTimings(self.ctx, C.byref(t)))
        return t

    def reset_timings(self):
        plugin.check(self.lib.PTResetTimings(self.ctx))

    def present_params(self) -> abi.PTPresentParams:
        q = abi.PTPresentParams()
        q.OutputWidth, q.OutputHeight = self.width, self.height
        q.Mode, q.sRGB = int(self.tonemapMode), 1 if self.sRGB else 0
        q.Exposure, q.Brightness, q.Contrast, q.Saturation, q.Vignette = (self.exposure, self.brightness, self.contrast,
                                                                          self.saturation, self.vignette)
        return q

    def present(self, q: abi.PTPresentParams = None) -> np.ndarray:
        q = q or self.present_params()
        out = np.empty((q.OutputHeight, q.OutputWidth, 4), dtype=np.float32)
        plugin.check(self.lib.PTPresentToHost(self.ctx, C.byref(q), out.ctypes.data_as(C.c_void_p), out.size))
        return out

    def present_to(self, q: abi.PTPresentParams, d_src: int, d_dst: int):
        plugin.check(self.lib.PTPresent(self.ctx, C.byref(q), C.c_void_p(d_src) if d_src else None, C.c_void_p(d_dst)))

    def set_schedule(self, schedule: int):
        plugin.check(self.lib.PTSetSchedule(self.ctx, schedule))

    def schedule(self) -> int:
        rc = self.lib.PTGetSchedule(self.ctx)
        if rc < 0:
            plugin.check(rc)
        return rc

    def set_wavefront_iterations(self, n: int):
        plugin.check(self.lib.PTSetWavefrontIterations(self.ctx, n))

    def set_passes_in_flight(self, n: int):
        plugin.check(self.lib.PTSetPassesInFlight(self.ctx, n))

    def set_sub_frames(self, n: int):
        plugin.check(self.lib.PTSetSubFrames(self.ctx, n))

    def passes_in_flight(self) -> int:
        return self.lib.PTGetPassesInFlight(self.ctx)

    @contextlib.contextmanager
    def _ordered(self, dev):
        import torch
        cur = torch.cuda.current_stream(dev)
        ext = torch.cuda.ExternalStream(self.stream(), device=dev)
        ext.wait_stream(cur)
        yield
        cur.wait_stream(ext)

    @staticmethod
    def _seed_bits(seeds, n, dev):
        import torch
        if seeds is None:
            return torch.arange(n, dtype=torch.int32, device=dev)
        sd = torch.as_tensor(seeds, device=dev).reshape(n).to(torch.int64).bitwise_and(0xFFFFFFFF)
        return torch.where(sd >= 2 ** 31, sd - 2 ** 32, sd).to(torch.int32)

    def _sample_rays(self, fn, rows, p, first_sample, spp):
        import torch
        as_numpy = isinstance(rows, np.ndarray)
        dev = torch.device(f"cuda:{self.device}")
        d_rows = torch.from_numpy(rows).to(dev) if as_numpy else rows
        n = rows.shape[0]
        rays = torch.empty((n * max(spp, 0), 8), dtype=torch.float32, device=dev)
        with self._ordered(dev):
            plugin.check(fn(self.ctx, C.byref(p), d_rows.data_ptr(), n, first_sample & 0xFFFFFFFF, spp, rays.data_ptr()))
        return rays.cpu().numpy() if as_numpy else rays

    def trace_rays(self, rays, any_hit: bool = False, surface: bool = False):
        if any_hit and surface:
            raise ValueError("surface records need closest-hit queries")
        flags = (abi.PT_QUERY_ANY_HIT if any_hit else abi.PT_QUERY_CLOSEST) | (abi.PT_QUERY_SURFACE if surface else 0)
        if isinstance(rays, np.ndarray):
            r = np.ascontiguousarray(rays, dtype=np.float32)
# ... 983 lines not shown
```

### unity_webgpu_pathtracer_amd/plugin.py

```python
import ctypes as C
import os
import subprocess

import numpy as np

from . import abi

_HERE = os.path.dirname(os.path.abspath(__file__))
LIB_NAME = "libunity-webgpu-pathtracer-plugin.so"
LIB_PATH = os.environ.get("PT_PLUGIN") or os.path.join(_HERE, "lib", LIB_NAME)

vp, i32, u32p = C.c_void_p, C.c_int, C.POINTER(C.c_uint32)
sig = {
    "BuildBVH": (i32, [vp, i32]), "DestroyBVH": (None, [i32]), "IsBVHReady": (i32, [i32]),
    "GetBVHPtr": (vp, [i32]), "GetBVH": (vp, [i32]),
    "GetCWBVHNodesSize": (i32, [i32]), "GetCWBVHTrisSize": (i32, [i32]),
    "GetCWBVHData": (i32, [i32, C.POINTER(vp), C.POINTER(vp)]),
    "PTBuildBVHDevice": (i32, [i32, vp, i32]), "PTGetBVHBuildError": (C.c_char_p, []), "PTGetBVHBuildMs": (C.c_double, [i32]),
    "PTRefitBVH": (i32, [i32, vp, i32]), "PTRefitBVHArrays": (i32, [vp, C.c_uint64, vp, C.c_uint64, vp, i32]),
    "BuildTLAS": (i32, [vp, i32]), "DestroyTLAS": (None, [i32]), "IsTLASReady": (i32, [i32]),
    "GetTLASNodesSize": (i32, [i32]), "GetTLASData": (i32, [i32, C.POINTER(vp), C.POINTER(vp)]),
    "PTCreate": (i32, [i32, C.POINTER(vp)]), "PTDestroy": (i32, [vp]),
    "PTSetScene": (i32, [vp, C.POINTER(abi.PTSceneDesc)]),
    "PTSetTileOwnership": (i32, [vp, i32, i32]),
    "PTRenderPass": (i32, [vp, C.POINTER(abi.PTFrameParams)]),
    "PTFlipFrames": (i32, [vp]), "PTResetFrames": (i32, [vp]),
    "PTRenderPassTo": (i32, [vp, C.POINTER(abi.PTFrameParams), vp, vp]),
    "PTRenderPassBatchTo": (i32, [vp, C.POINTER(abi.PTFrameParams), i32, vp, vp]),
    "PTRenderPassBatch": (i32, [vp, C.POINTER(abi.PTFrameParams), i32]),
    "PTGroupRenderPassBatch": (i32, [vp, C.POINTER(abi.PTFrameParams), i32]),
    "PTSynchronize": (i32, [vp]), "PTReadback": (i32, [vp, vp, C.c_uint64]),
    "PTGetFramePointer": (vp, [vp, i32]), "PTGetStream": (vp, [vp]),
    "PTSetStatsLevel": (i32, [vp, i32]), "PTGetStats": (i32, [vp, C.POINTER(abi.PTStats)]), "PTResetStats": (i32, [vp]),
    "PTSetProfiling": (i32, [vp, i32]), "PTGetTimings": (i32, [vp, C.POINTER(abi.PTTimings)]), "PTResetTimings": (i32, [vp]),
    "PTProcessMeshes": (i32, [vp, C.POINTER(abi.PTMeshDesc), C.c_uint32, C.c_uint32, vp, vp]),
    "PTCopyTextureData": (i32, [vp, C.POINTER(abi.PTTextureDesc), C.c_uint32, vp, C.c_uint64]),
    "PTPresent": (i32, [vp, C.POINTER(abi.PTPresentParams), vp, vp]),
    "PTPresentToHost": (i32, [vp, C.POINTER(abi.PTPresentParams), vp, C.c_uint64]),
    "PTSetSchedule": (i32, [vp, i32]), "PTGetSchedule": (i32, [vp]), "PTSetWavefrontIterations": (i32, [vp, i32]),
    "PTSetPassesInFlight": (i32, [vp, i32]), "PTGetPassesInFlight": (i32, [vp]), "PTSetSubFrames": (i32, [vp, i32]),
    "PTGetOwnedTileSlots": (i32, [vp, C.POINTER(abi.PTFrameParams), C.POINTER(C.c_uint64)]),
    "PTPackOwnedTiles": (i32, [vp, C.POINTER(abi.PTFrameParams), vp, vp]),
    "PTUnpackTiles": (i32, [vp, C.POINTER(abi.PTFrameParams), i32, i32, vp, vp]),
    "PTCreateMulti": (i32, [C.POINTER(i32), i32, C.POINTER(vp)]), "PTGroupDestroy": (i32, [vp]), "PTGroupSize": (i32, [vp]),
    "PTGroupGetContext": (vp, [vp, i32]), "PTGroupSetScene": (i32, [vp, C.POINTER(abi.PTSceneDesc)]),
    "PTGroupRenderPass": (i32, [vp, C.POINTER(abi.PTFrameParams)]), "PTGroupFlipFrames": (i32, [vp]), "PTGroupResetFrames": (i32, [vp]),
    "PTGroupSynchronize": (i32, [vp]), "PTGroupReadback": (i32, [vp, vp, C.c_uint64]), "PTGroupGetAssembledFrame": (vp, [vp]),
    "PTGroupGetStats": (i32, [vp, C.POINTER(abi.PTStats)]), "PTGroupResetStats": (i32, [vp]),
    "PTTraceRays": (i32, [vp, vp, C.c_uint64, C.c_uint32, vp, vp]),
    "PTTraceRaysHost": (i32, [vp, vp, C.c_uint64, C.c_uint32, vp, vp]),
    "PTRenderGuides": (i32, [vp, C.POINTER(abi.PTFrameParams), i32]),
    "PTDenoise": (i32, [vp, C.POINTER(abi.PTDenoiseParams), vp, vp]),
    "PTDenoiseToHost": (i32, [vp, C.POINTER(abi.PTDenoiseParams), vp, C.c_uint64]),
    "PTGetGuidePointer": (vp, [vp, i32]),
    "PTUpdateInstances": (i32, [vp, vp, C.c_uint32]), "PTUpdateInstancesDevice": (i32, [vp, vp, C.c_uint32]),
    "PTUpdateLights": (i32, [vp, vp, C.c_uint32]), "PTUpdateMaterials": (i32, [vp, vp, C.c_uint32]),
    "PTReadTLAS": (i32, [vp, vp, C.c_uint64, vp, C.c_uint64, u32p]),
    "PTAccumulateMoments": (i32, [vp, C.POINTER(abi.PTFrameParams), i32]),
    "PTAccumulateMomentsTo": (i32, [vp, C.POINTER(abi.PTFrameParams), i32, vp, vp]),
    "PTGetMomentsInfo": (i32, [vp, u32p, C.POINTER(C.c_uint64), u32p, u32p]),
    "PTGetMomentsPointer": (vp, [vp, i32]),
    "PTMeasureNoise": (i32, [vp, C.POINTER(abi.PTNoiseParams), vp, C.POINTER(abi.PTNoiseStats)]),
    "PTGetNoiseTilePointer": (vp, [vp]),
    "PTDenoiseMoments": (i32, [vp, C.POINTER(abi.PTDenoiseParams), vp, vp]),
    "PTDenoiseMomentsToHost": (i32, [vp, C.POINTER(abi.PTDenoiseParams), vp, C.c_uint64]),
    "PTAdaptiveBegin": (i32, [vp, C.POINTER(abi.PTFrameParams), C.c_uint32]), "PTAdaptiveEnd": (i32, [vp]),
    "PTSetActiveBlocks": (i32, [vp, u32p, C.c_uint32, u32p]),
    "PTSelectActiveBlocks": (i32, [vp, C.POINTER(abi.PTAdaptiveSelect), u32p]),
    "PTGetActiveBlocks": (i32, [vp, u32p, C.c_uint32, u32p]), "PTGetBlockSamples": (i32, [vp, u32p, C.c_uint64]),
    "PTRenderPassActive": (i32, [vp, C.POINTER(abi.PTFrameParams), i32]),
    "PTRenderPassActiveTo": (i32, [vp, C.POINTER(abi.PTFrameParams), i32, vp, vp]),
    "PTAccumulateMomentsActive": (i32, [vp, C.POINTER(abi.PTFrameParams), i32]),
    "PTAccumulateMomentsActiveTo": (i32, [vp, C.POINTER(abi.PTFrameParams), i32, vp, vp]),
    "PTCameraRays": (i32, [vp, C.POINTER(abi.PTFrameParams), vp, C.c_uint64, vp]),
    "PTTraceRadiance": (i32, [vp, C.POINTER(abi.PTFrameParams), vp, C.c_uint64, vp]),
    "PTTraceRadianceHost": (i32, [vp, C.POINTER(abi.PTFrameParams), vp, C.c_uint64, vp]),
    "PTUpdateGeometry": (i32, [vp, C.c_int32, C.c_int32, C.c_int32, vp, i32, vp]),
    "PTUpdateGeometryDevice": (i32, [vp, C.c_int32, C.c_int32, C.c_int32, vp, i32, vp]),
    "PTReadGeometry": (i32, [vp, vp, C.c_uint64, vp, C.c_uint64, vp, C.c_uint64]),
    "PTRebuildGeometry": (i32, [vp, C.c_int32, C.c_int32, C.c_int32, vp, i32, vp]),
    "PTRebuildGeometryDevice": (i32, [vp, C.c_int32, C.c_int32, C.c_int32, vp, i32, vp]),
    "PTMeasureGeometry": (i32, [vp, C.c_int32, C.c_int32, C.c_int32, C.POINTER(abi.PTGeometryQuality)]),
    "PTMeasureBVHArrays": (i32, [vp, C.c_uint64, vp, C.c_uint64, i32, C.POINTER(abi.PTGeometryQuality)]),
    "PTSetSkin": (i32, [vp, C.c_int32, C.c_int32, C.c_int32, i32, C.POINTER(abi.PTSkinDesc)]),
    "PTSkinGeometry": (i32, [vp, C.c_int32, C.c_int32, C.c_int32, vp, C.c_uint32, C.c_uint32, C.POINTER(C.c_float)]),
    "PTSkinGeometryDevice": (i32, [vp, C.c_int32, C.c_int32, C.c_int32, vp, C.c_uint32, C.c_uint32, C.POINTER(C.c_float)]),
    "PTSkinVerticesHost": (i32, [C.POINTER(abi.PTSkinDesc), i32, vp, vp, vp, C.POINTER(C.c_float)]),
    "PTSetMorph": (i32, [vp, C.c_int32, C.c_int32, C.c_int32, i32, C.POINTER(abi.PTMorphDesc)]),
    "PTMorphGeometry": (i32, [vp, C.c_int32, C.c_int32, C.c_int32, vp, C.c_uint32, vp, C.c_uint32, C.c_uint32, C.POINTER(C.c_float)]),
    "PTMorphGeometryDevice": (i32, [vp, C.c_int32, C.c_int32, C.c_int32, vp, C.c_uint32, vp, C.c_uint32, C.c_uint32, C.POINTER(C.c_float)]),
    "PTMorphVerticesHost": (i32, [C.POINTER(abi.PTMorphDesc), C.POINTER(abi.PTSkinDesc), i32, vp, vp, vp, vp, C.POINTER(C.c_float)]),
    "PTMorphLayoutHost": (C.c_uint64, [vp, vp, C.c_uint32, vp, vp, vp]),
    "PTGatherIrradiance": (i32, [vp, C.POINTER(abi.PTFrameParams), vp, C.c_uint64, C.c_uint32, C.c_uint32, vp]),
    "PTGatherIrradianceHost": (i32, [vp, C.POINTER(abi.PTFrameParams), vp, C.c_uint64, C.c_uint32, C.c_uint32, vp]),
    "PTGatherRays": (i32, [vp, C.POINTER(abi.PTFrameParams), vp, C.c_uint64, C.c_uint32, C.c_uint32, vp]),
    "PTRasterizeChart": (i32, [vp, C.POINTER(abi.PTChartDesc), vp, vp, vp, C.c_uint64, C.POINTER(C.c_uint64)]),
    "PTRasterizeChartHost": (i32, [C.POINTER(abi.PTChartDesc), vp, vp, vp, vp, vp, vp, vp, C.c_uint64, C.POINTER(C.c_uint64)]),
    "PTResolveLightmap": (i32, [vp, vp, vp, C.c_uint64, C.c_uint32, C.c_uint32, C.c_uint32, vp]),
    "PTResolveLightmapHost": (i32, [vp, vp, C.c_uint64, C.c_uint32, C.c_uint32, C.c_uint32, vp]),
    "PTProbeSH": (i32, [vp, C.POINTER(abi.PTFrameParams), vp, C.c_uint64, C.c_uint32, C.c_uint32, C.c_uint32, vp]),
    "PTProbeSHHost": (i32, [vp, C.POINTER(abi.PTFrameParams), vp, C.c_uint64, C.c_uint32, C.c_uint32, C.c_uint32, vp]),
    "PTProbeRays": (i32, [vp, C.POINTER(abi.PTFrameParams), vp, C.c_uint64, C.c_uint32, C.c_uint32, vp]),
    "PTProbeIrradiance": (i32, [vp, vp, C.c_uint64, vp, C.c_uint64, vp]),
    "PTProbeDirectionsHost": (i32, [vp, C.c_uint64, C.c_uint32, C.c_uint32, vp]),
    "PTProbeProjectHost": (i32, [vp, vp, C.c_uint64, C.c_uint32, vp]),
    "PTProbeIrradianceHost": (i32, [vp, C.c_uint64, vp, C.c_uint64, vp]),
    "PTProbeDepth": (i32, [vp, vp, C.c_uint64, C.c_uint32, C.c_uint32, C.c_float, vp]),
    "PTProbeDepthHost": (i32, [vp, vp, C.c_uint64, C.c_uint32, C.c_uint32, C.c_float, vp]),
    "PTProbeGridIrradiance": (i32, [vp, C.POINTER(abi.PTProbeGrid), vp, vp, vp, C.c_uint64, vp]),
    "PTProbeDepthProjectHost": (i32, [vp, C.c_uint64, C.c_uint32, C.c_uint32, vp, C.c_float, vp]),
    "PTProbeGridIrradianceHost": (i32, [C.POINTER(abi.PTProbeGrid), vp, vp, vp, C.c_uint64, vp]),
    "PTDenoiseLightmap": (i32, [vp, C.POINTER(abi.PTLightmapDenoiseParams), vp, vp, vp, C.c_uint64, C.c_uint32, C.c_uint32, vp]),
    "PTDenoiseLightmapHost": (i32, [C.POINTER(abi.PTLightmapDenoiseParams), vp, vp, vp, C.c_uint64, C.c_uint32, C.c_uint32, vp]),
    "PTProbePlace": (i32, [vp, vp, C.c_uint64, C.c_uint32, C.c_uint32, C.POINTER(abi.PTProbePlaceParams), C.c_uint32, vp, vp]),
    "PTProbePlaceHost": (i32, [vp, vp, C.c_uint64, C.c_uint32, C.c_uint32, C.POINTER(abi.PTProbePlaceParams), C.c_uint32, vp, vp]),
    "PTProbeGridIrradiancePlaced": (i32, [vp, C.POINTER(abi.PTProbeGrid), vp, vp, vp, vp, C.c_uint64, vp]),
# ... 647 lines not shown
```

Before: 5689 Mrays/s.

## Compact live wavefront path slots mid-sequence to shrink later kernel grids

Adds a stream-compaction pass for the wavefront path tracer. At selected iterations it counts live slots per block, scans them, and copies live path state (ray, radiance, throughput, rng, pixel index) into a temp arena and back, packed densely at the front. It also adds shade and cleanup variants that read the pixel via an indirection array. The aim is to cut idle lanes and reduce grid extent once many paths have terminated. The cost is four extra small kernels and about 204 bytes of state copied per live slot at each repack, plus the indirection loads.

```diff
diff --git a/__graft_entry__.py b/__graft_entry__.py
--- a/__graft_entry__.py
+++ b/__graft_entry__.py
@@ -10,6 +10,7 @@
 def build() -> None:
     subprocess.check_call(["make", "-C", os.path.join(ROOT, "unity_webgpu_pathtracer_amd", "csrc")])
     subprocess.check_call(["make", "-C", os.path.join(ROOT, "unity_webgpu_pathtracer_amd", "csrc"), "stress"])
+    subprocess.check_call(["make", "-C", os.path.join(ROOT, "unity_webgpu_pathtracer_amd", "csrc"), "stress-repack"])
     subprocess.check_call(["make", "-C", os.path.join(ROOT, "host")])
     subprocess.check_call(["make", "-C", os.path.join(ROOT, "oracle")])
     subprocess.check_call(["make", "-C", os.path.join(ROOT, "oracle"), "ref"])
diff --git a/include/ptmi_plugin.h b/include/ptmi_plugin.h
--- a/include/ptmi_plugin.h
+++ b/include/ptmi_plugin.h
@@ -194,6 +194,15 @@
 PT_API int PTSetStatsLevel(PTContext* ctx, int level);
 PT_API int PTGetStats(PTContext* ctx, PTStats* out);
 PT_API int PTResetStats(PTContext* ctx);
+typedef struct PTRepackStats {
+    uint64_t sequences;
+    uint64_t candidates;
+    uint64_t repacks;
+    uint64_t slotsMoved;
+} PTRepackStats;
+PT_API int PTGetRepackStats(PTContext* ctx, PTRepackStats* out);
+PT_API int PTRepackPlanHost(const uint32_t* flags, uint32_t numSlots, uint32_t capacity, uint32_t fillNum, uint32_t fillDen,
+                            uint32_t* outPlan, uint32_t* outDest);
 
 PT_API int PTSetProfiling(PTContext* ctx, int enabled);
 PT_API int PTGetTimings(PTContext* ctx, PTTimings* out);
diff --git a/unity_webgpu_pathtracer_amd/abi.py b/unity_webgpu_pathtracer_amd/abi.py
--- a/unity_webgpu_pathtracer_amd/abi.py
+++ b/unity_webgpu_pathtracer_amd/abi.py
@@ -128,6 +128,13 @@
                    + 64 * self.tlasNodeVisits + 144 * self.instanceVisits)
 
 
+class PTRepackStats(C.Structure):
+    _fields_ = [(n, C.c_uint64) for n in ("sequences", "candidates", "repacks", "slotsMoved")]
+
+    def as_dict(self):
+        return {n: int(getattr(self, n)) for n, _ in self._fields_}
+
+
 class PTPresentParams(C.Structure):
     _fields_ = [("OutputWidth", C.c_uint32), ("OutputHeight", C.c_uint32), ("Mode", C.c_int32), ("sRGB", C.c_int32),
                 ("Exposure", C.c_float), ("Brightness", C.c_float), ("Contrast", C.c_float), ("Saturation", C.c_float),
diff --git a/unity_webgpu_pathtracer_amd/csrc/plugin_exports.cpp b/unity_webgpu_pathtracer_amd/csrc/plugin_exports.cpp
--- a/unity_webgpu_pathtracer_amd/csrc/plugin_exports.cpp
+++ b/unity_webgpu_pathtracer_amd/csrc/plugin_exports.cpp
@@ -15,6 +15,7 @@
 #include "lmfilter_rule.h"
 #include "adaptive_gather_rule.h"
 #include "reflection_rule.h"
+#include "repack_rule.h"
 #include "ptmi_plugin.h"
 
 namespace {
@@ -277,6 +278,17 @@
     g_buildError.clear();
     return 1;
 }
+PT_API int PTRepackPlanHost(const uint32_t* flags, uint32_t numSlots, uint32_t capacity, uint32_t fillNum, uint32_t fillDen, uint32_t* outPlan, uint32_t* outDest)
+{
+    ptrepack::Plan plan;
+    if (!flags || !outPlan || !ptrepack::plan_host(flags, numSlots, capacity, fillNum, fillDen, plan, outDest, nullptr)) {
+        g_buildError = "NULL flags or plan, numSlots not a multiple of 256, or fillDen == 0";
+        return 0;
+    }
+    outPlan[0] = plan.go; outPlan[1] = plan.live; outPlan[2] = plan.extent;
+    g_buildError.clear();
+    return 1;
+}
 PT_API void DestroyBVH(int index) { free_slot(g_bvhs, index); }
 PT_API int IsBVHReady(int index) { return get_slot(g_bvhs, index) != nullptr; }
 PT_API void* GetBVH(int index) { return get_slot(g_bvhs, index); }
diff --git a/unity_webgpu_pathtracer_amd/csrc/pt_api_context.hip b/unity_webgpu_pathtracer_amd/csrc/pt_api_context.hip
--- a/unity_webgpu_pathtracer_amd/csrc/pt_api_context.hip
+++ b/unity_webgpu_pathtracer_amd/csrc/pt_api_context.hip
@@ -385,9 +385,9 @@
         if (int rc = create_set_stream(0u, c->sets[0].stream, &c->ownQueues)) { delete c; return rc; }
     }
     c->numSets = default_passes_in_flight(c->ownQueues);
-    se = hipMalloc(&c->dStats.ptr, 16 * sizeof(unsigned long long));
+    se = hipMalloc(&c->dStats.ptr, (16 + 4) * sizeof(unsigned long long));
     if (se != hipSuccess) { delete c; return fail(PT_ERR_HIP, std::string("hipMalloc: ") + hipGetErrorString(se)); }
-    hipMemsetAsync(c->dStats.ptr, 0, 16 * sizeof(unsigned long long), c->stream);
+    hipMemsetAsync(c->dStats.ptr, 0, (16 + 4) * sizeof(unsigned long long), c->stream);
     *outCtx = c;
     return PT_OK;
 }
@@ -442,6 +442,18 @@
     return PT_OK;
 }
 
+PT_API int PTGetRepackStats(PTContext* c, PTRepackStats* out)
+{
+    if (!c || !out) return fail(PT_ERR_INVALID_ARG, "ctx/out == NULL");
+    HIP_TRY(hipSetDevice(c->device));
+    unsigned long long h[4];
+    HIP_TRY(hipMemcpyAsync(h, (unsigned long long*)c->dStats.ptr + 16, sizeof(h), hipMemcpyDeviceToHost, c->stream));
+    HIP_TRY(hipStreamSynchronize(c->stream));
+    static_assert(sizeof(PTRepackStats) == 4 * 8, "PTRepackStats is 4 counters");
+    memcpy(out, h, sizeof(PTRepackStats));
+    return PT_OK;
+}
+
 PT_API int PTResetStats(PTContext* c)
 {
     if (!c) return fail(PT_ERR_INVALID_ARG, "ctx == NULL");
diff --git a/unity_webgpu_pathtracer_amd/csrc/pt_api_render.hip b/unity_webgpu_pathtracer_amd/csrc/pt_api_render.hip
--- a/unity_webgpu_pathtracer_amd/csrc/pt_api_render.hip
+++ b/unity_webgpu_pathtracer_amd/csrc/pt_api_render.hip
@@ -54,6 +54,7 @@
     L.scene = &c->scene;
     L.buffers = &set.wf;
     L.counters = (unsigned long long*)c->dStats.ptr;
+    L.repackStats = L.counters + 16;
     L.fullStats = c->statsLevel > 0;
     L.stream = set.stream;
     L.schedule = effective_schedule(c);
diff --git a/unity_webgpu_pathtracer_amd/csrc/pt_launch.h b/unity_webgpu_pathtracer_amd/csrc/pt_launch.h
--- a/unity_webgpu_pathtracer_amd/csrc/pt_launch.h
+++ b/unity_webgpu_pathtracer_amd/csrc/pt_launch.h
@@ -131,7 +131,13 @@
     uint32_t numSlots, numStatRows, maxIterations;
     uint32_t slotsPerPass;
     uint32_t residentWaves;
-};
+    uint32_t* pixelOf;
+    uint32_t* rpPrefix;
+    uint32_t* rpCtl;
+    char* rpTemp;
+    uint32_t rpCapacity;
+};
+#define PT_WF_REPACK_SLOT_BYTES 204u
 
 size_t pt_wf_arena_bytes(uint32_t numSlots, uint32_t residentWaves, bool needTlas, uint32_t maxIterations);
 PTWfBuffers pt_wf_arena_carve(void* base, uint32_t numSlots, uint32_t residentWaves, bool needTlas, uint32_t maxIterations);
@@ -232,6 +238,49 @@
 #ifndef PT_WF_SUSPEND
 #define PT_WF_SUSPEND 16u
 #endif
+#ifndef PT_WF_REPACK_MIN_ITERATIONS
+#define PT_WF_REPACK_MIN_ITERATIONS 12u
+#endif
+#ifndef PT_WF_REPACK_FIRST_SPP
+#define PT_WF_REPACK_FIRST_SPP 2u
+#endif
+#ifndef PT_WF_REPACK_FIRST_ADD
+#define PT_WF_REPACK_FIRST_ADD 0u
+#endif
+#ifndef PT_WF_REPACK_STRIDE
+#define PT_WF_REPACK_STRIDE 2u
+#endif
+#ifndef PT_WF_REPACK_MAX_CANDIDATES
+#define PT_WF_REPACK_MAX_CANDIDATES 5u
+#endif
+#ifndef PT_WF_REPACK_MIN_LEFT
+#define PT_WF_REPACK_MIN_LEFT 4u
+#endif
+#ifndef PT_WF_REPACK_FILL_NUM
+#define PT_WF_REPACK_FILL_NUM 3u
+#endif
+#ifndef PT_WF_REPACK_FILL_DEN
+#define PT_WF_REPACK_FILL_DEN 4u
+#endif
+inline bool pt_wf_repack_slots(uint32_t numSlots, uint32_t residentWaves)
+{
+#ifdef PT_WF_REPACK_MIN_SLOTS
+    return numSlots >= PT_WF_REPACK_MIN_SLOTS;
+#else
+    return pt_wf_wide_ranges(numSlots, residentWaves);
+#endif
+}
+inline bool pt_wf_repack_candidate(uint32_t it, uint32_t iterations, uint32_t spp)
+{
+    const uint32_t first = PT_WF_REPACK_FIRST_SPP * spp + PT_WF_REPACK_FIRST_ADD;
+    if (it < first || it + PT_WF_REPACK_MIN_LEFT >= iterations) return false;
+    return (it - first) % PT_WF_REPACK_STRIDE == 0u && (it - first) / PT_WF_REPACK_STRIDE < PT_WF_REPACK_MAX_CANDIDATES;
+}
+hipError_t pt_launch_repack(const PTWfBuffers& B, uint32_t fillNum, uint32_t fillDen, bool firstOfSequence, unsigned long long* stats, hipStream_t stream);
+hipError_t pt_launch_repack_shade(const DScene& S, const PTFrameParams& P, const PTTileMap& tm, const PTWfBuffers& B, bool fullStats, uint32_t iteration,
+                                  hipStream_t stream);
+hipError_t pt_launch_repack_cleanup(const DScene& S, const PTFrameParams& P, const PTTileMap& tm, const PTWfBuffers& B, bool fullStats, uint32_t blocks,
+                                    hipStream_t stream);
 #ifndef PT_WF_SETS
 #define PT_WF_SETS 12
 #endif
@@ -259,5 +308,6 @@
     bool zeroOutputFirst;
     int schedule;
     uint32_t iterationsOverride;
+    unsigned long long* repackStats;
 };
 hipError_t pt_launch_wavefront(const PTWfLaunch& L, uint32_t* launchesOut);
diff --git a/unity_webgpu_pathtracer_amd/csrc/pt_repack.hip b/unity_webgpu_pathtracer_amd/csrc/pt_repack.hip
--- /dev/null
+++ b/unity_webgpu_pathtracer_amd/csrc/pt_repack.hip
@@ -0,0 +1,176 @@
+#include "pt_device.h"
+#include "pt_launch.h"
+#include "pt_wf_state.h"
+#include "pt_wf_shade.h"
+#include "repack_rule.h"
+
+namespace {
+
+PT_DEV uint32_t rank_below(unsigned long long m)
+{
+    return __builtin_amdgcn_mbcnt_hi((uint32_t)(m >> 32), __builtin_amdgcn_mbcnt_lo((uint32_t)m, 0u));
+}
+
+static_assert(PT_REPACK_STATE_DONE == PS_DONE && PT_REPACK_BLOCK == 256u, "repack_rule.h restates the state code and the block");
+
+PT_DEV uint32_t* rp_u32(const PTWfBuffers& B, uint32_t k) { return (uint32_t*)((float4*)B.rpTemp + (size_t)PT_F4_HIT * B.rpCapacity) + (size_t)k * B.rpCapacity; }
+static_assert(PT_F4_HIT == 12u && PT_F4_HIT * 16u + 3u * 4u == PT_WF_REPACK_SLOT_BYTES, "the moved state is the twelve float4 planes before PT_F4_HIT and three words");
+
+PT_DEV uint32_t rp_rank_in_block(bool live, uint32_t* s_wave, uint32_t& blockLive)
+{
+    const unsigned long long m = __ballot(live);
+    const uint32_t w = threadIdx.x >> 6;
+    if ((threadIdx.x & 63u) == 0u) s_wave[w] = (uint32_t)__popcll(m);
+    __syncthreads();
+    uint32_t before = 0u;
+    for (uint32_t i = 0; i < 4u; ++i) if (i < w) before += s_wave[i];
+    blockLive = s_wave[0] + s_wave[1] + s_wave[2] + s_wave[3];
+    return before + rank_below(m);
+}
+
+__global__ __launch_bounds__(256) void pt_wf_repack_count(PTWfBuffers B)
+{
+    __shared__ uint32_t s_wave[4];
+    const uint32_t slot = blockIdx.x * 256u + threadIdx.x;
+    uint32_t blockLive;
+    rp_rank_in_block(ptrepack::slot_live(B.flags[slot]), s_wave, blockLive);
+    if (threadIdx.x == 0u) B.rpPrefix[blockIdx.x] = blockLive;
+}
+
+__global__ __launch_bounds__(1024) void pt_wf_repack_scan(PTWfBuffers B, uint32_t fillNum, uint32_t fillDen, uint32_t firstOfSequence, unsigned long long* stats)
+{
+    __shared__ uint32_t s_sum[16], s_hi[16];
+    const uint32_t nb = B.numSlots >> 8, t = threadIdx.x, lane = t & 63u, w = t >> 6;
+    const uint32_t per = (nb + 1023u) / 1024u;
+    const uint32_t b0 = t * per, b1 = b0 + per < nb ? b0 + per : nb;
+    uint32_t sum = 0u, hi = 0u;
+    for (uint32_t b = b0; b < b1; ++b) { const uint32_t c = B.rpPrefix[b]; sum += c; if (c) hi = b + 1u; }
+    uint32_t incl = sum;
+#pragma unroll
+    for (uint32_t off = 1u; off < 64u; off <<= 1) { const uint32_t o = (uint32_t)__shfl_up((int)incl, off, 64); if (lane >= off) incl += o; }
+    uint32_t whi = hi;
+#pragma unroll
+    for (uint32_t off = 32u; off > 0u; off >>= 1) { const uint32_t o = (uint32_t)__shfl_xor((int)whi, (int)off, 64); whi = o > whi ? o : whi; }
+    if (lane == 63u) s_sum[w] = incl;
+    if (lane == 0u) s_hi[w] = whi;
+    __syncthreads();
+    uint32_t before = 0u, L = 0u, top = 0u;
+    for (uint32_t i = 0; i < 16u; ++i) { if (i < w) before += s_sum[i]; L += s_sum[i]; top = s_hi[i] > top ? s_hi[i] : top; }
+    uint32_t running = before + incl - sum;
+    for (uint32_t b = b0; b < b1; ++b) { const uint32_t c = B.rpPrefix[b]; B.rpPrefix[b] = running; running += c; }
+    if (t == 0u) {
+        const uint32_t E = ptrepack::extent_of(top != 0u, top - 1u);
+        const bool go = ptrepack::decide(L, E, B.rpCapacity, fillNum, fillDen);
+        B.rpCtl[ptrepack::PT_REPACK_GO] = go ? 1u : 0u;
+        B.rpCtl[ptrepack::PT_REPACK_LIVE] = L;
+        B.rpCtl[ptrepack::PT_REPACK_EXTENT] = E;
+        if (stats) {
+            if (firstOfSequence) atomicAdd(stats + ptrepack::PT_REPACK_STAT_SEQUENCES, 1ull);
+            atomicAdd(stats + ptrepack::PT_REPACK_STAT_CANDIDATES, 1ull);
+            if (go) { atomicAdd(stats + ptrepack::PT_REPACK_STAT_REPACKS, 1ull); atomicAdd(stats + ptrepack::PT_REPACK_STAT_MOVED, (unsigned long long)L); }
+        }
+    }
+}
+
+struct RpLayout { float4* f4; size_t stride; uint32_t *flags, *rng, *pixelOf; };
+PT_DEV RpLayout rp_set_layout(const PTWfBuffers& B) { return RpLayout{B.f4base, B.f4stride, B.flags, B.rng, B.pixelOf}; }
+PT_DEV RpLayout rp_temp_layout(const PTWfBuffers& B) { return RpLayout{(float4*)B.rpTemp, B.rpCapacity, rp_u32(B, 0u), rp_u32(B, 1u), rp_u32(B, 2u)}; }
+PT_DEV void rp_copy(const RpLayout& s, size_t si, const RpLayout& d, size_t di, uint32_t flagsWord)
+{
+    const float4* s0 = s.f4 + PT_F4_RAY0 * s.stride + 2u * si;
+    const float4* s1 = s.f4 + PT_F4_RAY1 * s.stride + 2u * si;
+    const float4* s2 = s.f4 + PT_F4_RAY2 * s.stride + 2u * si;
+    const float4 a0 = s0[0], a1 = s0[1], b0 = s1[0], b1 = s1[1], c0 = s2[0], c1 = s2[1];
+    const float4 rad = s.f4[PT_F4_RAD * s.stride + si], thr = s.f4[PT_F4_THR * s.stride + si], col = s.f4[PT_F4_COLOR * s.stride + si];
+    const float4 envC = s.f4[PT_F4_ENVC * s.stride + si], lightC = s.f4[PT_F4_LIGHTC * s.stride + si], pthr = s.f4[PT_F4_PTHR * s.stride + si];
+    const uint32_t rng = s.rng[si], pix = s.pixelOf[si];
+    float4* d0 = d.f4 + PT_F4_RAY0 * d.stride + 2u * di;
+    float4* d1 = d.f4 + PT_F4_RAY1 * d.stride + 2u * di;
+    float4* d2 = d.f4 + PT_F4_RAY2 * d.stride + 2u * di;
+    d0[0] = a0; d0[1] = a1; d1[0] = b0; d1[1] = b1; d2[0] = c0; d2[1] = c1;
+    d.f4[PT_F4_RAD * d.stride + di] = rad; d.f4[PT_F4_THR * d.stride + di] = thr; d.f4[PT_F4_COLOR * d.stride + di] = col;
+    d.f4[PT_F4_ENVC * d.stride + di] = envC; d.f4[PT_F4_LIGHTC * d.stride + di] = lightC; d.f4[PT_F4_PTHR * d.stride + di] = pthr;
+    d.flags[di] = flagsWord; d.rng[di] = rng; d.pixelOf[di] = pix;
+}
+
+__global__ __launch_bounds__(256) void pt_wf_repack_out(PTWfBuffers B)
+{
+    __shared__ uint32_t s_wave[4];
+    if (B.rpCtl[ptrepack::PT_REPACK_GO] == 0u) return;
+    const uint32_t slot = blockIdx.x * 256u + threadIdx.x;
+    if (slot >= B.rpCtl[ptrepack::PT_REPACK_EXTENT]) return;
+    const uint32_t f = B.flags[slot];
+    const bool live = ptrepack::slot_live(f);
+    uint32_t blockLive;
+    const uint32_t rank = rp_rank_in_block(live, s_wave, blockLive);
+    if (!live) return;
+    const uint32_t d = ptrepack::destination(B.rpPrefix[blockIdx.x], rank);
+    if (d >= B.rpCapacity) return;
+    rp_copy(rp_set_layout(B), slot, rp_temp_layout(B), d, f);
+}
+
+__global__ __launch_bounds__(256) void pt_wf_repack_back(PTWfBuffers B)
+{
+    if (B.rpCtl[ptrepack::PT_REPACK_GO] == 0u) return;
+    const uint32_t slot = blockIdx.x * 256u + threadIdx.x;
+    const ptrepack::After w = ptrepack::after_move(slot, B.rpCtl[ptrepack::PT_REPACK_LIVE], B.rpCtl[ptrepack::PT_REPACK_EXTENT]);
+    if (w == ptrepack::After::Done) B.flags[slot] = PS_DONE;
+    if (w != ptrepack::After::Live) return;
+    const RpLayout T = rp_temp_layout(B);
+    rp_copy(T, slot, rp_set_layout(B), slot, T.flags[slot]);
+}
+
+template <bool STATS>
+__global__ __launch_bounds__(PT_WF_SHADE_BLOCK, PT_WF_SHADE_MIN_WAVES) void pt_wf_shade_repack(DScene S, PTFrameParams P, PTTileMap tm, PTWfBuffers B,
+                                                                                uint32_t iteration)
+{
+    const uint32_t vb = blockIdx.x;
+    const uint32_t slot = vb * PT_WF_SHADE_BLOCK + threadIdx.x;
+    if (vb == 0u && threadIdx.x < PT_WF_SHARDS) B.chunkHeads[threadIdx.x * 32u] = 0u;
+    const uint32_t f = B.flags[slot];
+    Counters cn = {};
+    if (fl_state(f) != PS_DONE) shade_slot<STATS, true, PTTileMap>(S, P, tm, B, slot, B.pixelOf[slot], f, cn, vb * PT_WF_SHADE_BLOCK);
+    flush_counters<STATS>(cn, B.statRows, vb * (PT_WF_SHADE_BLOCK / 64u) + (threadIdx.x >> 6), threadIdx.x & 63u);
+}
+
+template <bool STATS, bool TLAS>
+__global__ __launch_bounds__(256, 2) void pt_wf_cleanup_repack(DScene S, PTFrameParams P, PTTileMap tm, PTWfBuffers B)
+{
+    __shared__ uint2 s_stack[PT_LDS_STACK][256];
+    cleanup_slots<STATS, TLAS, true, PTTileMap>(S, P, tm, B, s_stack);
+}
+
+}
+
+hipError_t pt_launch_repack(const PTWfBuffers& B, uint32_t fillNum, uint32_t fillDen, bool firstOfSequence, unsigned long long* stats, hipStream_t stream)
+{
+    const uint32_t nb = B.numSlots >> 8;
+    hipLaunchKernelGGL(pt_wf_repack_count, dim3(nb), dim3(256), 0, stream, B);
+    hipLaunchKernelGGL(pt_wf_repack_scan, dim3(1), dim3(1024), 0, stream, B, fillNum, fillDen, firstOfSequence ? 1u : 0u, stats);
+    hipLaunchKernelGGL(pt_wf_repack_out, dim3(nb), dim3(256), 0, stream, B);
+    hipLaunchKernelGGL(pt_wf_repack_back, dim3(nb), dim3(256), 0, stream, B);
+    return hipGetLastError();
+}
+
+hipError_t pt_launch_repack_shade(const DScene& S, const PTFrameParams& P, const PTTileMap& tm, const PTWfBuffers& B, bool fullStats, uint32_t iteration,
+                                  hipStream_t stream)
+{
+    const dim3 grid(B.numSlots / PT_WF_SHADE_BLOCK), block(PT_WF_SHADE_BLOCK);
+    if (fullStats) hipLaunchKernelGGL(pt_wf_shade_repack<true>, grid, block, 0, stream, S, P, tm, B, iteration);
+    else hipLaunchKernelGGL(pt_wf_shade_repack<false>, grid, block, 0, stream, S, P, tm, B, iteration);
+    return hipGetLastError();
+}
+
+hipError_t pt_launch_repack_cleanup(const DScene& S, const PTFrameParams& P, const PTTileMap& tm, const PTWfBuffers& B, bool fullStats, uint32_t blocks,
+                                    hipStream_t stream)
+{
+    const bool tlas = S.hasTlas != 0u;
+    if (fullStats) {
+        if (tlas) hipLaunchKernelGGL((pt_wf_cleanup_repack<true, true>), dim3(blocks), dim3(256), 0, stream, S, P, tm, B);
+        else hipLaunchKernelGGL((pt_wf_cleanup_repack<true, false>), dim3(blocks), dim3(256), 0, stream, S, P, tm, B);
+    } else {
+        if (tlas) hipLaunchKernelGGL((pt_wf_cleanup_repack<false, true>), dim3(blocks), dim3(256), 0, stream, S, P, tm, B);
+        else hipLaunchKernelGGL((pt_wf_cleanup_repack<false, false>), dim3(blocks), dim3(256), 0, stream, S, P, tm, B);
+    }
+    return hipGetLastError();
+}
diff --git a/unity_webgpu_pathtracer_amd/csrc/pt_wavefront.hip b/unity_webgpu_pathtracer_amd/csrc/pt_wavefront.hip
--- a/unity_webgpu_pathtracer_amd/csrc/pt_wavefront.hip
+++ b/unity_webgpu_pathtracer_amd/csrc/pt_wavefront.hip
@@ -1,76 +1,13 @@
 #include "pt_device.h"
 #include "pt_launch.h"
 #include "pt_wf_state.h"
+#include "pt_wf_shade.h"
+#include "repack_rule.h"
 #include <type_traits>
 
 namespace {
 
 #define PT_WF_CHUNK 64u
-
-PT_DEV float4* f4_array(const PTWfBuffers& B, uint32_t k) { return B.f4base + (size_t)k * B.f4stride; }
-PT_DEV void fetch_ray(const PTWfBuffers& B, uint32_t slot, uint32_t kind, v3& o, v3& d)
-{
-    const float4* rec = f4_array(B, 2u * kind) + 2u * (size_t)slot;
-    o = xyz(rec[0]);
-    d = xyz(rec[1]);
-}
-
-
-PT_DEV uint32_t pixel_slot_of(const PTWfBuffers& B, uint32_t slot, uint32_t& pass)
-{
-    pass = 0u;
-    if (slot >= B.slotsPerPass) { pass = slot / B.slotsPerPass; slot -= pass * B.slotsPerPass; }
-    return slot;
-}
-
-PT_DEV bool wf_pixel(const PTTileMap& tm, const PTWfBuffers& B, uint32_t slot, uint32_t wgSlot, uint32_t& px, uint32_t& py, uint32_t& pass, uint32_t& base)
-{
-    base = 0u;
-    return pt_slot_to_pixel(tm, pixel_slot_of(B, slot, pass), px, py);
-}
-PT_DEV bool wf_pixel(const PTListMap& lm, const PTWfBuffers& B, uint32_t slot, uint32_t wgSlot, uint32_t& px, uint32_t& py, uint32_t& pass, uint32_t& base)
-{
-    pass = wgSlot / B.slotsPerPass;
-    const uint2 entry = lm.table[(wgSlot - pass * B.slotsPerPass) >> 8];
-    base = entry.y;
-    return pt_list_slot_to_pixel(lm.frameBlocksX, lm.coverW, lm.coverH, entry.x, slot & 255u, px, py);
-}
-template <class MAP> constexpr bool kListMap = std::is_same<MAP, PTListMap>::value;
-
-PT_DEV bool wf_pixel(const PTRayMap& rm, const PTWfBuffers& B, uint32_t slot, uint32_t wgSlot, uint32_t& px, uint32_t& py, uint32_t& pass, uint32_t& base)
-{
-    px = 0u; py = 0u; pass = 0u; base = 0u;
-    return slot < rm.count;
-}
-template <class MAP> constexpr bool kRayMap = std::is_same<MAP, PTRayMap>::value;
-struct RaySample {
-    const PTRadianceRay* rays; uint32_t slot;
-    PT_DEV void operator()(const PTFrameParams&, uint32_t, uint32_t, PathRegs& r, Counters& cn) const { start_ray(r, cn); }
-    PT_DEV void start_ray(PathRegs& r, Counters& cn) const
-    {
-        const float4* e = (const float4*)(rays + slot);
-        const float4 a = e[0], b = e[1];
-        cn.paths++;
-        r.scatterPdf = 0.0f;
-        r.maxRoughness = 0.0f;
-        r.ro = mk3(a.x, a.y, a.z);
-        r.rd = mk3(a.w, b.x, b.y);
-        r.state = PS_TRACE;
-    }
-};
-PT_DEV void ray_path_init(const PTRayMap& rm, uint32_t slot, PathRegs& r, Counters& cn)
-{
-    r.rng = rm.rays[slot].rng;
-    r.sampleIdx = 0u;
-    r.color = mk3(0.0f);
-    r.env.valid = 0u; r.light.valid = 0u;
-    r.env.dir = mk3(0.0f); r.light.dir = mk3(0.0f);
-    r.env.contribution = mk3(0.0f); r.light.contribution = mk3(0.0f);
-    r.neeOrigin = mk3(0.0f); r.pendThroughput = mk3(0.0f);
-    r.hasPending = false; r.green = false;
-    path_reset_sample(r);
-    RaySample{rm.rays, slot}.start_ray(r, cn);
-}
 
 template <class MAP = PTTileMap>
 __global__ __launch_bounds__(256) void pt_wf_init(PTFrameParams P, PTBatch batch, MAP tm, PTWfBuffers B)
@@ -78,6 +15,7 @@
     const uint32_t slot = blockIdx.x * 256u + threadIdx.x;
     if (blockIdx.x == 0u && threadIdx.x < PT_WF_SHARDS) B.chunkHeads[threadIdx.x * 32u] = 0u;
     if (slot >= B.numSlots) return;
+    if constexpr (!kListMap<MAP> && !kRayMap<MAP>) B.pixelOf[slot] = slot;
     uint32_t px, py, pass, base;
     Counters cn = {};
     if (!wf_pixel(tm, B, slot, blockIdx.x * 256u, px, py, pass, base)) B.flags[slot] = PS_DONE;
@@ -672,107 +610,6 @@
     flush_counters<STATS>(cn, B.statRows, (B.numSlots >> 6) + blockIdx.x, lane);
 }
 
-#ifndef PT_WF_SHADE_MIN_WAVES
-#define PT_WF_SHADE_MIN_WAVES 3
-#endif
-
-PT_DEV void load_path(const PTWfBuffers& B, uint32_t slot, uint32_t f, PathRegs& r)
-{
-    r.state = fl_state(f);
-    r.hasPending = fl_pending(f);
-    r.env.valid = fl_env(f);
-    r.light.valid = fl_light(f);
-    r.green = (f >> 6) & 1u;
-    r.sampleIdx = (f >> 7) & 0xFFFu;
-    r.depth = f >> 19;
-    r.rng = B.rng[slot];
-    float4 q;
-    q = B.ray[0][2u * slot]; r.ro = xyz(q); r.scatterPdf = q.w;
-    q = B.ray[0][2u * slot + 1u]; r.rd = xyz(q); r.maxRoughness = q.w;
-    r.radiance = xyz(B.rad[slot]);
-    r.throughput = xyz(B.thr[slot]);
-    r.color = xyz(B.color[slot]);
-    r.env.dir = mk3(0.0f); r.light.dir = mk3(0.0f); r.neeOrigin = mk3(0.0f);
-    r.env.contribution = mk3(0.0f); r.light.contribution = mk3(0.0f); r.pendThroughput = mk3(0.0f);
-    if (r.hasPending) {
-        r.env.contribution = xyz(B.envC[slot]);
-        r.light.contribution = xyz(B.lightC[slot]);
-        r.pendThroughput = xyz(B.pthr[slot]);
-    }
-}
-
-template <bool STATS, bool PIXSUM = false, class MAP = PTTileMap>
-PT_DEV bool shade_slot(const DScene& S, const PTFrameParams& P, const MAP& tm, const PTWfBuffers& B, uint32_t slot, uint32_t pixelSlot,
-                       uint32_t f, Counters& cn, uint32_t wgSlot = 0u)
-{
-    uint32_t px, py, pass, base;
-    wf_pixel(tm, B, pixelSlot, wgSlot, px, py, pass, base);
-    uint32_t rng = B.rng[slot];
-    float4 qro = B.ray[0][2u * slot], qrd = B.ray[0][2u * slot + 1u], qrad = B.rad[slot], qthr = B.thr[slot], qcol = B.color[slot];
-    float4 qenvC = B.envC[slot], qlightC = B.lightC[slot], qpthr = B.pthr[slot], qhit = B.hit[slot];
-    uint32_t o0 = B.occl[slot], o1 = B.occl[(size_t)B.numSlots + slot];
-    float4 qhit2 = make_float4(0.0f, 0.0f, 0.0f, 0.0f);
-    if (S.hasTlas) qhit2 = B.hit2[slot];
-    asm volatile("" : "+v"(rng), "+v"(qro.x), "+v"(qrd.x), "+v"(qrad.x), "+v"(qthr.x), "+v"(qcol.x), "+v"(qenvC.x), "+v"(qlightC.x), "+v"(qpthr.x),
-                      "+v"(qhit.x), "+v"(o0), "+v"(o1), "+v"(qhit2.x));
-    PathRegs r;
-    r.state = fl_state(f);
-    r.hasPending = fl_pending(f);
-    r.env.valid = fl_env(f);
-    r.light.valid = fl_light(f);
-    r.green = (f >> 6) & 1u;
-    r.sampleIdx = (f >> 7) & 0xFFFu;
-    r.depth = f >> 19;
-    r.rng = rng;
-    r.ro = xyz(qro); r.scatterPdf = qro.w;
-    r.rd = xyz(qrd); r.maxRoughness = qrd.w;
-    r.radiance = xyz(qrad);
-    r.throughput = xyz(qthr);
-    r.color = xyz(qcol);
-    r.env.dir = mk3(0.0f); r.light.dir = mk3(0.0f); r.neeOrigin = mk3(0.0f);
-    r.env.contribution = r.hasPending ? xyz(qenvC) : mk3(0.0f);
-    r.light.contribution = r.hasPending ? xyz(qlightC) : mk3(0.0f);
-    r.pendThroughput = r.hasPending ? xyz(qpthr) : mk3(0.0f);
-    const bool occEnv = r.hasPending && o0 != 0u, occLight = r.hasPending && o1 != 0u;
-    HitRecord ch;
-    ch.h.t = PT_FAR_PLANE; ch.h.u = 0.0f; ch.h.v = 0.0f; ch.h.triIndex = 0u;
-    ch.pos = mk3(0.0f); ch.inst = 0u;
-    if (r.state == PS_TRACE) {
-        ch.h.t = qhit.x; ch.h.u = qhit.y; ch.h.v = qhit.z; ch.h.triIndex = pt_asuint(qhit.w);
-        if (S.hasTlas) { ch.pos = xyz(qhit2); ch.inst = pt_asuint(qhit2.w); }
-    }
-    struct Sink {
-        const PTWfBuffers& B; uint32_t slot;
-        PT_DEV void operator()(PathRegs& q) const {
-            uint32_t s2 = slot;
-            asm volatile("" : "+v"(s2));
-            B.ray[1][2u * s2] = f4(q.neeOrigin, 0.0f);
-            B.ray[1][2u * s2 + 1u] = f4(q.env.dir, 0.0f);
-            B.ray[2][2u * s2] = f4(q.neeOrigin, 0.0f);
-            B.ray[2][2u * s2 + 1u] = f4(q.light.dir, 0.0f);
-            B.envC[s2] = f4(q.env.contribution, 0.0f);
-            B.lightC[s2] = f4(q.light.contribution, 0.0f);
-            B.pthr[s2] = f4(q.pendThroughput, 0.0f);
-        }
-    };
-    if constexpr (kRayMap<MAP>)
-        path_step<STATS, false, Sink, RaySample, true>(S, P, r, ch, occEnv, occLight, 0u, 0u, 0u, nullptr, nullptr, cn, Sink{B, slot}, RaySample{tm.rays, pixelSlot});
-    else
-        path_step<STATS, false, Sink, CameraSample, true>(S, P, r, ch, occEnv, occLight, px, py, py * P.OutputWidth + px, nullptr, nullptr, cn, Sink{B, slot});
-    uint32_t storeSlot = slot;
-    asm volatile("" : "+v"(storeSlot));
-    store_path(B, storeSlot, r, false);
-    if (PIXSUM && r.state == PS_DONE) {
-        uint32_t ps = pixelSlot;
-        asm volatile("" : "+v"(ps));
-        B.pixsum[ps] = f4(r.color, 0.0f);
-    }
-    return r.state != PS_DONE;
-}
-
-#ifndef PT_WF_SHADE_BLOCK
-#define PT_WF_SHADE_BLOCK 64u
-#endif
 template <bool STATS, class MAP = PTTileMap>
 __global__ __launch_bounds__(PT_WF_SHADE_BLOCK, PT_WF_SHADE_MIN_WAVES) void pt_wf_shade(DScene S, PTFrameParams P, MAP tm, PTWfBuffers B,
                                                                          uint32_t iteration)
@@ -988,58 +825,7 @@
 __global__ __launch_bounds__(256, 2) void pt_wf_cleanup(DScene S, PTFrameParams P, MAP tm, PTWfBuffers B)
 {
     __shared__ uint2 s_stack[PT_LDS_STACK][256];
-    Counters cn = {};
-    for (uint32_t blk = blockIdx.x; blk < (B.numSlots >> 8); blk += gridDim.x) {
-    const uint32_t slot = blk * 256u + threadIdx.x;
-    const uint32_t f = B.flags[slot];
-    if (__any(fl_state(f) != PS_DONE)) {
-        if (fl_state(f) != PS_DONE) {
-            uint32_t px, py, pass, base;
-            wf_pixel(tm, B, slot, blk * 256u, px, py, pass, base);
-            PathRegs r;
-            load_path(B, slot, f, r);
-            if (r.hasPending) {
-                r.neeOrigin = xyz(B.ray[1][2u * slot]);
-                r.env.dir = xyz(B.ray[1][2u * slot + 1u]);
-                r.light.dir = xyz(B.ray[2][2u * slot + 1u]);
-            }
-            TravStack st;
-            st.lds = PT_LDS_U2(&s_stack[0][threadIdx.x]);
-            st.stride = 256u;
-            while (r.state != PS_DONE) {
-                HitRecord ch;
-                ch.h.t = PT_FAR_PLANE; ch.h.u = 0.0f; ch.h.v = 0.0f; ch.h.triIndex = 0u;
-                ch.pos = mk3(0.0f); ch.inst = 0u;
-                bool occEnv = false, occLight = false;
-                if (r.hasPending && r.env.valid != 0u) {
-                    HitRecord h = ch;
-                    if (TLAS) occEnv = traverse_tlas<STATS>(S, r.neeOrigin, r.env.dir, true, h, st, cn);
-                    else { traverse_cwbvh<STATS>(S, r.neeOrigin, r.env.dir, true, h.h, st, cn); occEnv = h.h.t < PT_FAR_PLANE; }
-                    cn.shadowRays++;
-                }
-                if (r.hasPending && r.light.valid != 0u) {
-                    HitRecord h = ch;
-                    if (TLAS) occLight = traverse_tlas<STATS>(S, r.neeOrigin, r.light.dir, true, h, st, cn);
-                    else { traverse_cwbvh<STATS>(S, r.neeOrigin, r.light.dir, true, h.h, st, cn); occLight = h.h.t < PT_FAR_PLANE; }
-                    cn.shadowRays++;
-                }
-                if (r.state == PS_TRACE) {
-                    if (TLAS) traverse_tlas<STATS>(S, r.ro, r.rd, false, ch, st, cn);
-                    else traverse_cwbvh<STATS>(S, r.ro, r.rd, false, ch.h, st, cn);
-                    cn.closestRays++;
-                }
-                if constexpr (kRayMap<MAP>)
-                    path_step<STATS, false, NoNeeSink, RaySample, true>(S, P, r, ch, occEnv, occLight, 0u, 0u, 0u, nullptr, nullptr, cn, NoNeeSink(), RaySample{tm.rays, slot});
-                else
-                    path_step<STATS, false, NoNeeSink, CameraSample, true>(S, P, r, ch, occEnv, occLight, px, py, py * P.OutputWidth + px, nullptr, nullptr, cn);
-            }
-            B.flags[slot] = pack_flags(r);
-            B.color[slot] = f4(r.color, 0.0f);
-            if constexpr (kRayMap<MAP>) B.rng[slot] = r.rng;
-        }
-    }
-    }
-    flush_counters<STATS>(cn, B.statRows, blockIdx.x * 4u + (threadIdx.x >> 6), threadIdx.x & 63u);
+    cleanup_slots<STATS, TLAS, false, MAP>(S, P, tm, B, s_stack);
 }
 
 template <class MAP = PTTileMap>
@@ -1136,6 +922,13 @@
     B.susp = (uint4*)carve(suspBytes);
     B.suspCount = (uint32_t*)carve(traceWaves * 4);
     B.tlasSpill = needTlas ? (uint32_t*)carve(tlasSpillBytes) : nullptr;
+    B.pixelOf = (uint32_t*)carve(n * 4);
+    B.rpPrefix = (uint32_t*)carve((n >> 8) * 4 + 4);
+    B.rpCtl = (uint32_t*)carve(ptrepack::PT_REPACK_CTL_WORDS * 4);
+    B.rpCapacity = numSlots / 2u;
+    const size_t tempBytes = (size_t)B.rpCapacity * PT_WF_REPACK_SLOT_BYTES;
+    const bool aliased = base ? (char*)B.susp + suspBytes >= (char*)B.stackSpill + tempBytes : align(spillBytes) + suspBytes >= tempBytes;
+    B.rpTemp = aliased ? (char*)B.stackSpill : carve(tempBytes);
     B.residentWaves = residentWaves;
     B.numSlots = numSlots;
     B.numStatRows = numRows;
@@ -1206,6 +999,9 @@
     const uint32_t bounces = P.MaxRayBounces > 1u ? P.MaxRayBounces : 1u;
     uint32_t iterations = L.iterationsOverride ? L.iterationsOverride : spp * (bounces + 2u) + 4u;
     if (iterations > B.maxIterations) iterations = B.maxIterations;
+    const bool repack = !kList && !kRays && (trace == Trace::Refill || trace == Trace::RefillTlas) && B.rpTemp != nullptr &&
+                        pt_wf_repack_slots(B.numSlots, B.residentWaves) && iterations >= PT_WF_REPACK_MIN_ITERATIONS;
+    bool firstCandidate = true;
     for (uint32_t it = 0; it < iterations; ++it) {
         if constexpr (UNIT_A) {
             const bool wide = PT_WF_RANGE >= 128u && pt_wf_wide_ranges(B.numSlots, B.residentWaves);
@@ -1240,13 +1036,24 @@
             }
             launches++;
         }
-        with_flag(fullStats, [&](auto stats) {
+        if constexpr (!kList && !kRays) {
+            if (repack) { if ((e = pt_launch_repack_shade(S, P, tm, B, fullStats, it, stream)) != hipSuccess) return e; }
+        }
+        if (!repack) with_flag(fullStats, [&](auto stats) {
             hipLaunchKernelGGL((pt_wf_shade<PT_FLAG(stats), MAP>), dim3(B.numSlots / PT_WF_SHADE_BLOCK), dim3(PT_WF_SHADE_BLOCK), 0, stream, S, P, tm, B, it);
         });
         launches++;
+        if (repack && pt_wf_repack_candidate(it, iterations, spp)) {
+            if ((e = pt_launch_repack(B, PT_WF_REPACK_FILL_NUM, PT_WF_REPACK_FILL_DEN, firstCandidate, L.repackStats, stream)) != hipSuccess) return e;
+            firstCandidate = false;
+            launches += 4;
+        }
     }
     const uint32_t cleanupBlocks = nb < 1024u ? nb : 1024u;
-    with_flag(fullStats, [&](auto stats) { with_flag(!UNIT_A && tlas, [&](auto tl) {
+    if constexpr (!kList && !kRays) {
+        if (repack) { if ((e = pt_launch_repack_cleanup(S, P, tm, B, fullStats, cleanupBlocks, stream)) != hipSuccess) return e; }
+    }
+    if (!repack) with_flag(fullStats, [&](auto stats) { with_flag(!UNIT_A && tlas, [&](auto tl) {
         constexpr bool TLAS = !UNIT_A && PT_FLAG(tl);
         hipLaunchKernelGGL((pt_wf_cleanup<PT_FLAG(stats), TLAS, MAP>), dim3(cleanupBlocks), dim3(256), 0, stream, S, P, tm, B);
     }); });
@@ -1262,7 +1069,7 @@
             (e = hipMemcpyAsync(output, L.accumulated, (size_t)P.OutputWidth * P.OutputHeight * sizeof(float4), hipMemcpyDeviceToDevice, stream)) != hipSuccess) return e;
     }
     if constexpr (!kRays)
-        hipLaunchKernelGGL(pt_wf_resolve<MAP>, dim3(nbPass), dim3(256), 0, stream, P, batch, tm, B, (const float4*)B.color, L.accumulated, output);
+        hipLaunchKernelGGL(pt_wf_resolve<MAP>, dim3(nbPass), dim3(256), 0, stream, P, batch, tm, B, (const float4*)(repack ? B.pixsum : B.color), L.accumulated, output);
     hipLaunchKernelGGL(pt_wf_fold_rows, dim3(256), dim3(256), 0, stream, B.statRows, B.numStatRows, L.counters);
     launches += 3;
     if (launchesOut) *launchesOut = launches;
diff --git a/unity_webgpu_pathtracer_amd/csrc/pt_wf_shade.h b/unity_webgpu_pathtracer_amd/csrc/pt_wf_shade.h
--- /dev/null
+++ b/unity_webgpu_pathtracer_amd/csrc/pt_wf_shade.h
@@ -0,0 +1,234 @@
+#pragma once
+#include "pt_device.h"
+#include "pt_launch.h"
+#include "pt_wf_state.h"
+#include <type_traits>
+
+namespace {
+
+PT_DEV float4* f4_array(const PTWfBuffers& B, uint32_t k) { return B.f4base + (size_t)k * B.f4stride; }
+PT_DEV void fetch_ray(const PTWfBuffers& B, uint32_t slot, uint32_t kind, v3& o, v3& d)
+{
+    const float4* rec = f4_array(B, 2u * kind) + 2u * (size_t)slot;
+    o = xyz(rec[0]);
+    d = xyz(rec[1]);
+}
+
+
+PT_DEV uint32_t pixel_slot_of(const PTWfBuffers& B, uint32_t slot, uint32_t& pass)
+{
+    pass = 0u;
+    if (slot >= B.slotsPerPass) { pass = slot / B.slotsPerPass; slot -= pass * B.slotsPerPass; }
+    return slot;
+}
+
+PT_DEV bool wf_pixel(const PTTileMap& tm, const PTWfBuffers& B, uint32_t slot, uint32_t wgSlot, uint32_t& px, uint32_t& py, uint32_t& pass, uint32_t& base)
+{
+    base = 0u;
+    return pt_slot_to_pixel(tm, pixel_slot_of(B, slot, pass), px, py);
+}
+PT_DEV bool wf_pixel(const PTListMap& lm, const PTWfBuffers& B, uint32_t slot, uint32_t wgSlot, uint32_t& px, uint32_t& py, uint32_t& pass, uint32_t& base)
+{
+    pass = wgSlot / B.slotsPerPass;
+    const uint2 entry = lm.table[(wgSlot - pass * B.slotsPerPass) >> 8];
+    base = entry.y;
+    return pt_list_slot_to_pixel(lm.frameBlocksX, lm.coverW, lm.coverH, entry.x, slot & 255u, px, py);
+}
+template <class MAP> constexpr bool kListMap = std::is_same<MAP, PTListMap>::value;
+
+PT_DEV bool wf_pixel(const PTRayMap& rm, const PTWfBuffers& B, uint32_t slot, uint32_t wgSlot, uint32_t& px, uint32_t& py, uint32_t& pass, uint32_t& base)
+{
+    px = 0u; py = 0u; pass = 0u; base = 0u;
+    return slot < rm.count;
+}
+template <class MAP> constexpr bool kRayMap = std::is_same<MAP, PTRayMap>::value;
+struct RaySample {
+    const PTRadianceRay* rays; uint32_t slot;
+    PT_DEV void operator()(const PTFrameParams&, uint32_t, uint32_t, PathRegs& r, Counters& cn) const { start_ray(r, cn); }
+    PT_DEV void start_ray(PathRegs& r, Counters& cn) const
+    {
+        const float4* e = (const float4*)(rays + slot);
+        const float4 a = e[0], b = e[1];
+        cn.paths++;
+        r.scatterPdf = 0.0f;
+        r.maxRoughness = 0.0f;
+        r.ro = mk3(a.x, a.y, a.z);
+        r.rd = mk3(a.w, b.x, b.y);
+        r.state = PS_TRACE;
+    }
+};
+PT_DEV void ray_path_init(const PTRayMap& rm, uint32_t slot, PathRegs& r, Counters& cn)
+{
+    r.rng = rm.rays[slot].rng;
+    r.sampleIdx = 0u;
+    r.color = mk3(0.0f);
+    r.env.valid = 0u; r.light.valid = 0u;
+    r.env.dir = mk3(0.0f); r.light.dir = mk3(0.0f);
+    r.env.contribution = mk3(0.0f); r.light.contribution = mk3(0.0f);
+    r.neeOrigin = mk3(0.0f); r.pendThroughput = mk3(0.0f);
+    r.hasPending = false; r.green = false;
+    path_reset_sample(r);
+    RaySample{rm.rays, slot}.start_ray(r, cn);
+}
+
+#ifndef PT_WF_SHADE_MIN_WAVES
+#define PT_WF_SHADE_MIN_WAVES 3
+#endif
+
+PT_DEV void load_path(const PTWfBuffers& B, uint32_t slot, uint32_t f, PathRegs& r)
+{
+    r.state = fl_state(f);
+    r.hasPending = fl_pending(f);
+    r.env.valid = fl_env(f);
+    r.light.valid = fl_light(f);
+    r.green = (f >> 6) & 1u;
+    r.sampleIdx = (f >> 7) & 0xFFFu;
+    r.depth = f >> 19;
+    r.rng = B.rng[slot];
+    float4 q;
+    q = B.ray[0][2u * slot]; r.ro = xyz(q); r.scatterPdf = q.w;
+    q = B.ray[0][2u * slot + 1u]; r.rd = xyz(q); r.maxRoughness = q.w;
+    r.radiance = xyz(B.rad[slot]);
+    r.throughput = xyz(B.thr[slot]);
+    r.color = xyz(B.color[slot]);
+    r.env.dir = mk3(0.0f); r.light.dir = mk3(0.0f); r.neeOrigin = mk3(0.0f);
+    r.env.contribution = mk3(0.0f); r.light.contribution = mk3(0.0f); r.pendThroughput = mk3(0.0f);
+    if (r.hasPending) {
+        r.env.contribution = xyz(B.envC[slot]);
+        r.light.contribution = xyz(B.lightC[slot]);
+        r.pendThroughput = xyz(B.pthr[slot]);
+    }
+}
+
+template <bool STATS, bool PIXSUM = false, class MAP = PTTileMap>
+PT_DEV bool shade_slot(const DScene& S, const PTFrameParams& P, const MAP& tm, const PTWfBuffers& B, uint32_t slot, uint32_t pixelSlot,
+                       uint32_t f, Counters& cn, uint32_t wgSlot = 0u)
+{
+    uint32_t px, py, pass, base;
+    wf_pixel(tm, B, pixelSlot, wgSlot, px, py, pass, base);
+    uint32_t rng = B.rng[slot];
+    float4 qro = B.ray[0][2u * slot], qrd = B.ray[0][2u * slot + 1u], qrad = B.rad[slot], qthr = B.thr[slot], qcol = B.color[slot];
+    float4 qenvC = B.envC[slot], qlightC = B.lightC[slot], qpthr = B.pthr[slot], qhit = B.hit[slot];
+    uint32_t o0 = B.occl[slot], o1 = B.occl[(size_t)B.numSlots + slot];
+    float4 qhit2 = make_float4(0.0f, 0.0f, 0.0f, 0.0f);
+    if (S.hasTlas) qhit2 = B.hit2[slot];
+    asm volatile("" : "+v"(rng), "+v"(qro.x), "+v"(qrd.x), "+v"(qrad.x), "+v"(qthr.x), "+v"(qcol.x), "+v"(qenvC.x), "+v"(qlightC.x), "+v"(qpthr.x),
+                      "+v"(qhit.x), "+v"(o0), "+v"(o1), "+v"(qhit2.x));
+    PathRegs r;
+    r.state = fl_state(f);
+    r.hasPending = fl_pending(f);
+    r.env.valid = fl_env(f);
+    r.light.valid = fl_light(f);
+    r.green = (f >> 6) & 1u;
+    r.sampleIdx = (f >> 7) & 0xFFFu;
+    r.depth = f >> 19;
+    r.rng = rng;
+    r.ro = xyz(qro); r.scatterPdf = qro.w;
+    r.rd = xyz(qrd); r.maxRoughness = qrd.w;
+    r.radiance = xyz(qrad);
+    r.throughput = xyz(qthr);
+    r.color = xyz(qcol);
+    r.env.dir = mk3(0.0f); r.light.dir = mk3(0.0f); r.neeOrigin = mk3(0.0f);
+    r.env.contribution = r.hasPending ? xyz(qenvC) : mk3(0.0f);
+    r.light.contribution = r.hasPending ? xyz(qlightC) : mk3(0.0f);
+    r.pendThroughput = r.hasPending ? xyz(qpthr) : mk3(0.0f);
+    const bool occEnv = r.hasPending && o0 != 0u, occLight = r.hasPending && o1 != 0u;
+    HitRecord ch;
+    ch.h.t = PT_FAR_PLANE; ch.h.u = 0.0f; ch.h.v = 0.0f; ch.h.triIndex = 0u;
+    ch.pos = mk3(0.0f); ch.inst = 0u;
+    if (r.state == PS_TRACE) {
+        ch.h.t = qhit.x; ch.h.u = qhit.y; ch.h.v = qhit.z; ch.h.triIndex = pt_asuint(qhit.w);
+        if (S.hasTlas) { ch.pos = xyz(qhit2); ch.inst = pt_asuint(qhit2.w); }
+    }
+    struct Sink {
+        const PTWfBuffers& B; uint32_t slot;
+        PT_DEV void operator()(PathRegs& q) const {
+            uint32_t s2 = slot;
+            asm volatile("" : "+v"(s2));
+            B.ray[1][2u * s2] = f4(q.neeOrigin, 0.0f);
+            B.ray[1][2u * s2 + 1u] = f4(q.env.dir, 0.0f);
+            B.ray[2][2u * s2] = f4(q.neeOrigin, 0.0f);
+            B.ray[2][2u * s2 + 1u] = f4(q.light.dir, 0.0f);
+            B.envC[s2] = f4(q.env.contribution, 0.0f);
+            B.lightC[s2] = f4(q.light.contribution, 0.0f);
+            B.pthr[s2] = f4(q.pendThroughput, 0.0f);
+        }
+    };
+    if constexpr (kRayMap<MAP>)
+        path_step<STATS, false, Sink, RaySample, true>(S, P, r, ch, occEnv, occLight, 0u, 0u, 0u, nullptr, nullptr, cn, Sink{B, slot}, RaySample{tm.rays, pixelSlot});
+    else
+        path_step<STATS, false, Sink, CameraSample, true>(S, P, r, ch, occEnv, occLight, px, py, py * P.OutputWidth + px, nullptr, nullptr, cn, Sink{B, slot});
+    uint32_t storeSlot = slot;
+    asm volatile("" : "+v"(storeSlot));
+    store_path(B, storeSlot, r, false);
+    if (PIXSUM && r.state == PS_DONE) {
+        uint32_t ps = pixelSlot;
+        asm volatile("" : "+v"(ps));
+        B.pixsum[ps] = f4(r.color, 0.0f);
+    }
+    return r.state != PS_DONE;
+}
+
+#ifndef PT_WF_SHADE_BLOCK
+#define PT_WF_SHADE_BLOCK 64u
+#endif
+template <bool STATS, bool TLAS, bool REPACK, class MAP>
+PT_DEV void cleanup_slots(const DScene& S, const PTFrameParams& P, const MAP& tm, const PTWfBuffers& B, uint2 (&s_stack)[PT_LDS_STACK][256])
+{
+    Counters cn = {};
+    for (uint32_t blk = blockIdx.x; blk < (B.numSlots >> 8); blk += gridDim.x) {
+    const uint32_t slot = blk * 256u + threadIdx.x;
+    const uint32_t f = B.flags[slot];
+    if (__any(fl_state(f) != PS_DONE)) {
+        if (fl_state(f) != PS_DONE) {
+            uint32_t px, py, pass, base;
+            const uint32_t pixelSlot = REPACK ? B.pixelOf[slot] : slot;
+            wf_pixel(tm, B, pixelSlot, blk * 256u, px, py, pass, base);
+            PathRegs r;
+            load_path(B, slot, f, r);
+            if (r.hasPending) {
+                r.neeOrigin = xyz(B.ray[1][2u * slot]);
+                r.env.dir = xyz(B.ray[1][2u * slot + 1u]);
+                r.light.dir = xyz(B.ray[2][2u * slot + 1u]);
+            }
+            TravStack st;
+            st.lds = PT_LDS_U2(&s_stack[0][threadIdx.x]);
+            st.stride = 256u;
+            while (r.state != PS_DONE) {
+                HitRecord ch;
+                ch.h.t = PT_FAR_PLANE; ch.h.u = 0.0f; ch.h.v = 0.0f; ch.h.triIndex = 0u;
+                ch.pos = mk3(0.0f); ch.inst = 0u;
+                bool occEnv = false, occLight = false;
+                if (r.hasPending && r.env.valid != 0u) {
+                    HitRecord h = ch;
+                    if (TLAS) occEnv = traverse_tlas<STATS>(S, r.neeOrigin, r.env.dir, true, h, st, cn);
+                    else { traverse_cwbvh<STATS>(S, r.neeOrigin, r.env.dir, true, h.h, st, cn); occEnv = h.h.t < PT_FAR_PLANE; }
+                    cn.shadowRays++;
+                }
+                if (r.hasPending && r.light.valid != 0u) {
+                    HitRecord h = ch;
+                    if (TLAS) occLight = traverse_tlas<STATS>(S, r.neeOrigin, r.light.dir, true, h, st, cn);
+                    else { traverse_cwbvh<STATS>(S, r.neeOrigin, r.light.dir, true, h.h, st, cn); occLight = h.h.t < PT_FAR_PLANE; }
+                    cn.shadowRays++;
+                }
+                if (r.state == PS_TRACE) {
+                    if (TLAS) traverse_tlas<STATS>(S, r.ro, r.rd, false, ch, st, cn);
+                    else traverse_cwbvh<STATS>(S, r.ro, r.rd, false, ch.h, st, cn);
+                    cn.closestRays++;
+                }
+                if constexpr (kRayMap<MAP>)
+                    path_step<STATS, false, NoNeeSink, RaySample, true>(S, P, r, ch, occEnv, occLight, 0u, 0u, 0u, nullptr, nullptr, cn, NoNeeSink(), RaySample{tm.rays, slot});
+                else
+                    path_step<STATS, false, NoNeeSink, CameraSample, true>(S, P, r, ch, occEnv, occLight, px, py, py * P.OutputWidth + px, nullptr, nullptr, cn);
+            }
+            B.flags[slot] = pack_flags(r);
+            if (REPACK) B.pixsum[pixelSlot] = f4(r.color, 0.0f); else
+            B.color[slot] = f4(r.color, 0.0f);
+            if constexpr (kRayMap<MAP>) B.rng[slot] = r.rng;
+        }
+    }
+    }
+    flush_counters<STATS>(cn, B.statRows, blockIdx.x * 4u + (threadIdx.x >> 6), threadIdx.x & 63u);
+}
+
+}
diff --git a/unity_webgpu_pathtracer_amd/csrc/repack_host.cpp b/unity_webgpu_pathtracer_amd/csrc/repack_host.cpp
--- /dev/null
+++ b/unity_webgpu_pathtracer_amd/csrc/repack_host.cpp
@@ -0,0 +1,58 @@
+#include <cstring>
+#include <vector>
+#include "repack_rule.h"
+
+namespace ptrepack {
+
+bool plan_host(const uint32_t* flags, uint32_t numSlots, uint32_t capacity, uint32_t fillNum, uint32_t fillDen, Plan& plan, uint32_t* dest,
+               uint32_t* blockPrefix)
+{
+    plan = Plan{0u, 0u, 0u};
+    if (numSlots % PT_REPACK_BLOCK != 0u || fillDen == 0u || (numSlots != 0u && !flags)) return false;
+    const uint32_t blocks = numSlots / PT_REPACK_BLOCK;
+    std::vector<uint32_t> count(blocks, 0u);
+    for (uint32_t b = 0; b < blocks; ++b)
+        for (uint32_t t = 0; t < PT_REPACK_BLOCK; ++t) count[b] += slot_live(flags[b * PT_REPACK_BLOCK + t]) ? 1u : 0u;
+    std::vector<uint32_t> prefix(blocks, 0u);
+    uint32_t L = 0u, highest = 0u;
+    bool any = false;
+    for (uint32_t b = 0; b < blocks; ++b) {
+        prefix[b] = L;
+        L += count[b];
+        if (count[b] != 0u) { any = true; highest = b; }
+    }
+    plan.live = L;
+    plan.extent = extent_of(any, highest);
+    plan.go = decide(L, plan.extent, capacity, fillNum, fillDen) ? 1u : 0u;
+    if (blockPrefix) std::memcpy(blockPrefix, prefix.data(), (size_t)blocks * sizeof(uint32_t));
+    if (dest) {
+        for (uint32_t b = 0; b < blocks; ++b) {
+            uint32_t rank = 0u;
+            for (uint32_t t = 0; t < PT_REPACK_BLOCK; ++t) {
+                const uint32_t s = b * PT_REPACK_BLOCK + t;
+                if (slot_live(flags[s])) dest[s] = destination(prefix[b], rank++);
+                else dest[s] = 0xFFFFFFFFu;
+            }
+        }
+    }
+    return true;
+}
+
+void move_host(const Plan& plan, const uint32_t* dest, uint32_t numSlots, void* array, uint32_t stride, bool isFlags)
+{
+    if (!plan.go) return;
+    std::vector<unsigned char> tmp((size_t)plan.live * stride);
+    unsigned char* a = (unsigned char*)array;
+    for (uint32_t s = 0; s < plan.extent && s < numSlots; ++s)
+        if (dest[s] != 0xFFFFFFFFu) std::memcpy(&tmp[(size_t)dest[s] * stride], a + (size_t)s * stride, stride);
+    for (uint32_t s = 0; s < plan.extent && s < numSlots; ++s) {
+        const After w = after_move(s, plan.live, plan.extent);
+        if (w == After::Live) std::memcpy(a + (size_t)s * stride, &tmp[(size_t)s * stride], stride);
+        else if (w == After::Done && isFlags) {
+            const uint32_t done = PT_REPACK_STATE_DONE;
+            std::memcpy(a + (size_t)s * stride, &done, sizeof(done) < stride ? sizeof(done) : stride);
+        }
+    }
+}
+
+}
diff --git a/unity_webgpu_pathtracer_amd/csrc/repack_rule.h b/unity_webgpu_pathtracer_amd/csrc/repack_rule.h
--- /dev/null
+++ b/unity_webgpu_pathtracer_amd/csrc/repack_rule.h
@@ -0,0 +1,40 @@
+#pragma once
+#include <stdint.h>
+
+#if defined(__HIPCC__)
+#define PT_REPACK_HD __host__ __device__ __forceinline__
+#else
+#define PT_REPACK_HD inline
+#endif
+
+#define PT_REPACK_BLOCK 256u
+#define PT_REPACK_STATE_DONE 2u
+
+namespace ptrepack {
+
+enum : uint32_t { PT_REPACK_GO = 0, PT_REPACK_LIVE, PT_REPACK_EXTENT, PT_REPACK_CTL_WORDS };
+enum : uint32_t { PT_REPACK_STAT_SEQUENCES = 0, PT_REPACK_STAT_CANDIDATES, PT_REPACK_STAT_REPACKS, PT_REPACK_STAT_MOVED, PT_REPACK_STAT_WORDS };
+
+PT_REPACK_HD bool slot_live(uint32_t flagsWord) { return (flagsWord & 3u) != PT_REPACK_STATE_DONE; }
+
+PT_REPACK_HD uint32_t extent_of(bool anyLive, uint32_t highestLiveBlock) { return anyLive ? (highestLiveBlock + 1u) * PT_REPACK_BLOCK : 0u; }
+
+PT_REPACK_HD bool decide(uint32_t L, uint32_t E, uint32_t capacity, uint32_t fillNum, uint32_t fillDen)
+{
+    return L > 0u && L <= capacity && (uint64_t)L * fillDen <= (uint64_t)E * fillNum;
+}
+
+PT_REPACK_HD uint32_t destination(uint32_t blockPrefix, uint32_t rankInBlock) { return blockPrefix + rankInBlock; }
+
+enum class After : uint32_t { Live, Done, Untouched };
+PT_REPACK_HD After after_move(uint32_t slot, uint32_t L, uint32_t E) { return slot < L ? After::Live : slot < E ? After::Done : After::Untouched; }
+
+struct Plan {
+    uint32_t go;
+    uint32_t live, extent;
+};
+bool plan_host(const uint32_t* flags, uint32_t numSlots, uint32_t capacity, uint32_t fillNum, uint32_t fillDen, Plan& plan, uint32_t* dest,
+               uint32_t* blockPrefix);
+void move_host(const Plan& plan, const uint32_t* dest, uint32_t numSlots, void* array, uint32_t stride, bool isFlags);
+
+}
diff --git a/unity_webgpu_pathtracer_amd/csrc/repack_sanitize_main.cpp b/unity_webgpu_pathtracer_amd/csrc/repack_sanitize_main.cpp
--- /dev/null
+++ b/unity_webgpu_pathtracer_amd/csrc/repack_sanitize_main.cpp
@@ -0,0 +1,97 @@
+#include <cstdio>
+#include <cstring>
+#include <vector>
+#include "repack_rule.h"
+
+namespace {
+
+uint32_t g_state = 2463534242u;
+uint32_t rnd() { g_state ^= g_state << 13; g_state ^= g_state >> 17; g_state ^= g_state << 5; return g_state; }
+
+int bad(const char* what) { std::printf("repack-sanitize: %s\n", what); return 1; }
+
+int run(const std::vector<uint32_t>& flags, uint32_t capacity, uint32_t num, uint32_t den, int expectGo)
+{
+    using namespace ptrepack;
+    const uint32_t n = (uint32_t)flags.size();
+    std::vector<uint32_t> liveSlots;
+    for (uint32_t s = 0; s < n; ++s) if ((flags[s] & 3u) != 2u) liveSlots.push_back(s);
+    const uint32_t L = (uint32_t)liveSlots.size();
+    const uint32_t E = L ? (liveSlots.back() / PT_REPACK_BLOCK + 1u) * PT_REPACK_BLOCK : 0u;
+    const bool go = L > 0u && L <= capacity && (unsigned long long)L * den <= (unsigned long long)E * num;
+
+    Plan plan;
+    std::vector<uint32_t> dest(n), prefix(n / PT_REPACK_BLOCK);
+    if (!plan_host(flags.data(), n, capacity, num, den, plan, dest.data(), prefix.data())) return bad("plan_host refused a well-formed array");
+    if (plan.live != L || plan.extent != E) return bad("live count or extent differ from the plain loop");
+    if ((plan.go != 0u) != go) return bad("the decision differs from the plain loop");
+    if (expectGo >= 0 && (int)plan.go != expectGo) return bad("an edge of the decision fell on the wrong side");
+    for (uint32_t k = 0; k < L; ++k) if (dest[liveSlots[k]] != k) return bad("a live slot's destination is not its rank among the live slots");
+    for (uint32_t s = 0; s < n; ++s) if ((flags[s] & 3u) == 2u && dest[s] != 0xFFFFFFFFu) return bad("a finished slot has a destination");
+
+    std::vector<uint32_t> f(flags);
+    std::vector<uint32_t> rec((size_t)n * 8u);
+    for (uint32_t s = 0; s < n; ++s) for (uint32_t k = 0; k < 8u; ++k) rec[(size_t)s * 8u + k] = s * 8u + k;
+    move_host(plan, dest.data(), n, rec.data(), 32u, false);
+    move_host(plan, dest.data(), n, f.data(), 4u, true);
+    if (!plan.go) {
+        if (std::memcmp(f.data(), flags.data(), (size_t)n * 4u) != 0) return bad("a refused plan changed the flags");
+        return 0;
+    }
+    for (uint32_t s = 0; s < n; ++s) {
+        if (s < L) {
+            if (f[s] != flags[liveSlots[s]]) return bad("slot order is not stable");
+            for (uint32_t k = 0; k < 8u; ++k) if (rec[(size_t)s * 8u + k] != liveSlots[s] * 8u + k) return bad("a record did not follow its slot");
+        } else if (s < E) {
+            if (f[s] != 2u) return bad("a slot between the live ones and the extent is not DONE");
+        } else if (f[s] != flags[s]) return bad("a slot beyond the extent was touched");
+    }
+    return 0;
+}
+
+std::vector<uint32_t> make(uint32_t n, uint32_t livePerMille)
+{
+    std::vector<uint32_t> f(n);
+    for (uint32_t s = 0; s < n; ++s) {
+        const uint32_t hi = rnd() & ~3u;
+        f[s] = hi | ((rnd() % 1000u) < livePerMille ? (rnd() & 1u) : 2u);
+    }
+    return f;
+}
+
+}
+
+int main()
+{
+    const uint32_t B = PT_REPACK_BLOCK;
+    for (uint32_t trial = 0; trial < 200u; ++trial) {
+        const uint32_t n = (1u + rnd() % 40u) * B;
+        const std::vector<uint32_t> f = make(n, rnd() % 1001u);
+        if (run(f, n / 2u, 3u, 4u, -1) || run(f, n / 2u, 1u, 1u, -1)) return 1;
+    }
+    const uint32_t n = 8u * B, cap = n / 2u;
+    std::vector<uint32_t> f(n, 2u);
+    if (run(f, cap, 1u, 1u, 0)) return 1;
+    std::fill(f.begin(), f.end(), 0u);
+    if (run(f, cap, 1u, 1u, 0)) return 1;
+    if (run(f, n, 1u, 1u, 1)) return 1;
+    if (run(f, n, 3u, 4u, 0)) return 1;
+    std::fill(f.begin(), f.end(), 2u);
+    for (uint32_t k = 0; k < cap; ++k) f[2u * k + 1u] = 1u;
+    if (run(f, cap, 1u, 1u, 1)) return 1;
+    f[0] = 0u;
+    if (run(f, cap, 1u, 1u, 0)) return 1;
+    std::fill(f.begin(), f.end(), 2u);
+    f[n - 1u] = 0u; f[n - B] = 1u; f[n - 7u] = 0u;
+    if (run(f, cap, 3u, 4u, 1)) return 1;
+    std::vector<uint32_t> one(B, 2u);
+    one[5] = 0u; one[200] = 1u;
+    if (run(one, B / 2u, 3u, 4u, 1)) return 1;
+    std::fill(one.begin(), one.end(), 0u);
+    if (run(one, B, 1u, 1u, 1)) return 1;
+    ptrepack::Plan plan;
+    if (ptrepack::plan_host(f.data(), n - 1u, cap, 3u, 4u, plan, nullptr, nullptr)) return bad("a slot count that is no multiple of the block was accepted");
+    if (ptrepack::plan_host(f.data(), n, cap, 3u, 0u, plan, nullptr, nullptr)) return bad("a fill of x / 0 was accepted");
+    std::printf("repack ok\n");
+    return 0;
+}
diff --git a/unity_webgpu_pathtracer_amd/pathtracer.py b/unity_webgpu_pathtracer_amd/pathtracer.py
--- a/unity_webgpu_pathtracer_amd/pathtracer.py
+++ b/unity_webgpu_pathtracer_amd/pathtracer.py
@@ -247,6 +247,11 @@
     def reset_stats(self):
         plugin.check(self.lib.PTResetStats(self.ctx))
 
+    def repack_stats(self) -> abi.PTRepackStats:
+        st = abi.PTRepackStats()
+        plugin.check(self.lib.PTGetRepackStats(self.ctx, C.byref(st)))
+        return st
+
     def set_profiling(self, on: bool):
         plugin.check(self.lib.PTSetProfiling(self.ctx, 1 if on else 0))
 
diff --git a/unity_webgpu_pathtracer_amd/plugin.py b/unity_webgpu_pathtracer_amd/plugin.py
--- a/unity_webgpu_pathtracer_amd/plugin.py
+++ b/unity_webgpu_pathtracer_amd/plugin.py
@@ -32,6 +32,8 @@
     "PTSynchronize": (i32, [vp]), "PTReadback": (i32, [vp, vp, C.c_uint64]),
     "PTGetFramePointer": (vp, [vp, i32]), "PTGetStream": (vp, [vp]),
     "PTSetStatsLevel": (i32, [vp, i32]), "PTGetStats": (i32, [vp, C.POINTER(abi.PTStats)]), "PTResetStats": (i32, [vp]),
+    "PTGetRepackStats": (i32, [vp, C.POINTER(abi.PTRepackStats)]),
+    "PTRepackPlanHost": (i32, [vp, C.c_uint32, C.c_uint32, C.c_uint32, C.c_uint32, vp, vp]),
     "PTSetProfiling": (i32, [vp, i32]), "PTGetTimings": (i32, [vp, C.POINTER(abi.PTTimings)]), "PTResetTimings": (i32, [vp]),
     "PTProcessMeshes": (i32, [vp, C.POINTER(abi.PTMeshDesc), C.c_uint32, C.c_uint32, vp, vp]),
     "PTCopyTextureData": (i32, [vp, C.POINTER(abi.PTTextureDesc), C.c_uint32, vp, C.c_uint64]),
```

Measured after the change: 5940 Mrays/s, median of 6. +4.4%, better.
